# shichaoy/pop_up_slam

Hardware: AMD Instinct MI355X
Metric: graph-solve iters/sec + final chi2, 1k-pose/5k-edge plane graph (higher is better)
Workload: dtype f64; 1 GPU; C2 synthetic corridor: 1000 SE3 poses, 200 planes, 5000 plane edges, 999 odometry edges (BASELINE.json configs[1], seed 42); jacobian_mode=numeric, total_lm_solves=812

## Files before the change

### include/pps.h

```cpp
#ifndef PPS_H
#define PPS_H

#include <stddef.h>
#include <stdint.h>

#ifdef __cplusplus
extern "C" {
#endif

#define PPS_VERSION 304

typedef struct pps_graph pps_graph;

enum pps_status {
  PPS_OK = 0,
  PPS_EINVAL = 1,
  PPS_ENOTPD = 2,
  PPS_EHIP = 3,
  PPS_ENOMEM = 4,
  PPS_ESTATE = 5
};

enum pps_jacobian_mode {
  PPS_JAC_NUMERIC = 0,
// ... 26 lines not shown

int pps_add_pose_prior(pps_graph* g, int pose, const double meas6[6], const double sqrtinf_ut[21], int* fid);
int pps_add_odometry(pps_graph* g, int pose1, int pose2, const double meas6[6], const double sqrtinf_ut[21], int* fid);
int pps_add_plane_obs(pps_graph* g, int pose, int plane, const double meas4[4], const double sqrtinf_ut[6], int* fid);
int pps_add_plane_obs2(pps_graph* g, int pose_id, int plane_id, const double meas4[4], const double ray6[6],
                       const double sqrtinf_ut[6], int* fid);
int pps_edge_ray(const float invK[9], const float seg2d[4], double ray6[6]);
int pps_add_plane_prior(pps_graph* g, int plane, const double meas4[4], const double sqrtinf_ut[6], int* fid);

int pps_set_measurement(pps_graph* g, int fid, const double meas4[4]);
int pps_set_measurements(pps_graph* g, int n, const int* fids, const double* meas4 );

int pps_remove_factor(pps_graph* g, int fid);
int pps_remove_node(pps_graph* g, int nid);

int pps_update(pps_graph* g);
int pps_batch_optimize(pps_graph* g, int* iterations);
int pps_chi2(pps_graph* g, double* chi2);

int pps_cov_recover(pps_graph* g);
int pps_cov_marginals(pps_graph* g, int n, const int* ids, double* out, int64_t* offsets);
int pps_cov_access(pps_graph* g, int n, const int* rows, const int* cols, double* out, int64_t* offsets, int* in_pattern);
int pps_cov_joint(pps_graph* g, int n, const int* ids, double* out);
int pps_cov_last_times(const pps_graph* g, double sec[2]);
int pps_cov_block(pps_graph* g, int nr, const int* rows, int nc, const int* cols, double* out);
int pps_cov_block_last(const pps_graph* g, double* kernel_sec, int* launches);

typedef struct pps_multi pps_multi;
int pps_multi_create(int n, pps_graph* const* graphs, pps_multi** out);
int pps_multi_destroy(pps_multi* m);
const char* pps_multi_last_error(const pps_multi* m);
int pps_multi_optimize(pps_multi* m, int* iterations, int* status);
int pps_multi_rounds(const pps_multi* m, int* rounds);
int pps_multi_save_state(pps_multi* m);
int pps_multi_restore_state(pps_multi* m);
int pps_multi_set_profiling(pps_multi* m, int level);
int pps_multi_phase_times(const pps_multi* m, double sec[5], long long counts[4]);

int pps_num_nodes(const pps_graph* g, int* n);
int pps_num_factors(const pps_graph* g, int* n);
int pps_get_pose(pps_graph* g, int id, double tq[7]);
int pps_get_plane(pps_graph* g, int id, double abcd[4]);
int pps_set_pose(pps_graph* g, int id, const double tq[7]);
int pps_set_plane(pps_graph* g, int id, const double abcd[4]);
int pps_get_poses(pps_graph* g, int n, const int* ids, double* out);
int pps_get_planes(pps_graph* g, int n, const int* ids, double* out);
int pps_save_state(pps_graph* g);
int pps_restore_state(pps_graph* g);

typedef struct pps_stats {
  int    n_poses, n_planes, n_factors;
  int    dim_nodes, dim_measure;
  int    n_fronts, n_levels, max_front;
  int64_t nnz_L;
  int    lm_iterations;
  int    lm_trials_accepted, lm_trials_rejected;
  double chi2_initial, chi2_final, lambda_final;
  double last_delta_norm;
  double t_total, t_analysis, t_upload;
  double t_linearize, t_assemble, t_factor, t_backsolve, t_retract_chi2;
  int    n_linearize, n_factorize;
  int    lm_trials_notpd;
  int    n_launches;
} pps_stats;
int pps_get_stats(const pps_graph* g, pps_stats* out);
int pps_get_trace(const pps_graph* g, int cap, double* lambda, double* chi2, int* accepted, int* n);
int pps_set_profiling(pps_graph* g, int level);

int pps_factor_shape(const pps_graph* g, int fid, int* dim, int* cols);
int pps_eval_factor(pps_graph* g, int fid, int mode , double* J, double* r);

int pps_analyze(pps_graph* g);
int pps_analysis_reuse(const pps_graph* g, int* fronts_kept, int* fronts_total);
int pps_analysis_kept(const pps_graph* g, int kept[6]);
int pps_analysis_dump(pps_graph* g, int64_t cap, int32_t* out, int64_t* needed);

int pps_time_linearize(pps_graph* g, int mode, int iters, double* sec_per_launch);
int pps_bench_sweep(pps_graph* g, int mode, int replicas, int iters, double sec_per_sweep[3],
                    int64_t* n_plane_edges, int64_t* n_odo_edges);

int pps_debug_front_factor(int tiles, int strip, int p, int b, const double* A, double* L, double* U, double* not_pd);

int pps_debug_exmap(int kind, int n, const double* x, const double* delta, double* out);

int pps_popup_planes(int device, const float* seg2d, int n, const float invK[9], const float T_wc[16],
                     float* planes_out);

typedef struct pps_point { float x, y, z; uint32_t rgba; } pps_point;

typedef struct pps_popup pps_popup;
int pps_popup_create(int device, int width, int height, const float invK[9], pps_popup** out);
int pps_popup_destroy(pps_popup* p);
const char* pps_popup_last_error(const pps_popup* p);
int pps_popup_set_image(pps_popup* p, const unsigned char* bgr);
int pps_popup_run(pps_popup* p, const float* seg2d, int n, const float T_wc[16], const float* polys,
                  const int* poly_off, int nplanes, int step, float depth_thre, float ceiling_thre, int* n_valid);
int pps_popup_run_async(pps_popup* p, const float* seg2d, int n, const float T_wc[16], const float* polys,
                        const int* poly_off, int nplanes, int step, float depth_thre, float ceiling_thre);
int pps_popup_planes_wait(pps_popup* p, float* planes);
int pps_popup_wait(pps_popup* p, int* n_valid);
int pps_popup_download(pps_popup* p, float* planes, pps_point* cloud, float* depth, int32_t* plane_id);
int pps_popup_set_outputs(pps_popup* p, int want_depth, int want_plane_id);
int pps_popup_plane_info(pps_popup* p, float plane_cam_dist_thre, const int* actual_plane_indices, int n_actual,
                         float* dist_to_cam, int32_t* good);
int pps_popup_fill_depth(pps_popup* p);
int pps_popup_download_segments3d(pps_popup* p, float* seg3d_world);
int pps_popup_last_kernel_time(const pps_popup* p, double* sec);
int pps_popup_polygons_simple(const float K[9], const float invK[9], const float T_wc[16], int width, int height, const float* seg2d, int n,
                              float* verts, int cap_verts, int* poly_off, int* n_verts);
int pps_popup_mask_host(const float* polys, const int* poly_off, int nplanes, int width, int height, int step, int32_t* plane_id);

int pps_frames_set_calibration(pps_graph* g, const float invK[9]);
int pps_frames_add(pps_graph* g, int pose_id, int n_seg, const float* seg2d, const int* fids, int* frame_id);
int pps_refresh_measurements(pps_graph* g);
int pps_get_measurement(pps_graph* g, int fid, double meas4[4]);

typedef struct pps_assoc_params {
  double edge_asso_2ddist;
  double edge_asso_planedist;
  double edge_asso_proj;
  double edge_asso_angle;
  int assoc_near_frames;
} pps_assoc_params;
void pps_assoc_default_params(pps_assoc_params* p);
int pps_landmark_update(pps_graph* g, int plane_id, int frame_plane_indice, int frame_seq_id, const float seg2d[4],
                        const float seg3d_xy[4]);
int pps_landmark_set_merged(pps_graph* g, int plane_id);
int pps_find_closest_planes(pps_graph* g, const double est_pose[7], int frame_seq_id, int n, const double* planes_local,
                            const int* frame_plane_indice, const float* seg2d, const float* seg3d_xy,
                            const pps_assoc_params* prm, int* best_plane_id, double* best_err);

int pps_graph_save(pps_graph* g, const char* path, int precision);
int pps_graph_load(const char* path, const pps_props* props, pps_graph** out);

int pps_reproject_points(pps_graph* g, int n, const int* plane_ids, const float* pts_xyz, float* out_xyz);

typedef struct pps_edge_params {
  int downsample_contour;
  int dilation_distance, erosion_distance;
  double pre_vertical_thre, pre_minium_len, pre_contour_close_thre, interval_overlap_thre, post_short_thre,
         post_bind_dist_thre, post_merge_dist_thre, post_merge_angle_thre, post_extend_thre;
  double pre_boundary_thre, pre_merge_angle_thre, pre_merge_dist_thre, pre_proj_angle_thre, pre_proj_cover_thre,
         pre_proj_cover_large_thre, pre_proj_dist_thre;
} pps_edge_params;
void pps_edge_default_params(pps_edge_params* p);

typedef struct pps_edges pps_edges;
int pps_edges_create(int device, int width, int height, pps_edges** out);
int pps_edges_destroy(pps_edges* e);
const char* pps_edges_last_error(const pps_edges* e);
int pps_edges_select(pps_edges* e, const unsigned char* label_map, int label_on_device, const float* lsd_lines,
                     int n_lines, const pps_edge_params* prm, float* open_segs, int* n_open, float* closed_segs,
                     int* n_closed, float* open_in_closed);
int pps_edges_download_label(pps_edges* e, unsigned char* out, int* w, int* h);
int pps_edges_contour(pps_edges* e, float* xy, int cap, int* n, int* n_contours, int* n_points);
int pps_edges_last_kernel_time(const pps_edges* e, double* sec);
int pps_edges_host_contour(const int16_t* cell_segs, int n, float scale, float* xy, int cap, int* n_xy, int* n_contours,
                           int* n_points);
int pps_edges_host_select(const float* contour_xy, int n_contour, int width, int height, const float* lsd_lines, int n_lines,
                          const pps_edge_params* prm, float* open_segs, int* n_open, float* closed_segs, int* n_closed,
                          float* open_in_closed);

#ifdef __cplusplus
}
#endif
#endif
// ... 1 lines not shown
```

### pop_up_slam_amd/__init__.py

```python
from __future__ import annotations

import ctypes as C
import os

import numpy as np

_HERE = os.path.dirname(os.path.abspath(__file__))
LIB_PATH = os.environ.get("PPS_LIB") or os.path.join(_HERE, "libpps.so")

PPS_OK, PPS_EINVAL, PPS_ENOTPD, PPS_EHIP, PPS_ENOMEM, PPS_ESTATE = range(6)
JAC_NUMERIC, JAC_ANALYTIC = 0, 1

_dp = C.POINTER(C.c_double)
_fp = C.POINTER(C.c_float)
_ip = C.POINTER(C.c_int)


PPS_VERSION = 304


class PpsProps(C.Structure):
    _fields_ = [
        ("epsilon2", C.c_double), ("epsilon_abs", C.c_double), ("epsilon_rel", C.c_double),
        ("max_iterations", C.c_int), ("lm_lambda0", C.c_double), ("lm_lambda_factor", C.c_double),
        ("jacobian_mode", C.c_int), ("device", C.c_int), ("verbose", C.c_int),
    ]


class PpsStats(C.Structure):
    _fields_ = [
        ("n_poses", C.c_int), ("n_planes", C.c_int), ("n_factors", C.c_int),
        ("dim_nodes", C.c_int), ("dim_measure", C.c_int),
        ("n_fronts", C.c_int), ("n_levels", C.c_int), ("max_front", C.c_int),
        ("nnz_L", C.c_int64),
        ("lm_iterations", C.c_int), ("lm_trials_accepted", C.c_int), ("lm_trials_rejected", C.c_int),
        ("chi2_initial", C.c_double), ("chi2_final", C.c_double), ("lambda_final", C.c_double),
        ("last_delta_norm", C.c_double),
        ("t_total", C.c_double), ("t_analysis", C.c_double), ("t_upload", C.c_double),
        ("t_linearize", C.c_double), ("t_assemble", C.c_double), ("t_factor", C.c_double),
        ("t_backsolve", C.c_double), ("t_retract_chi2", C.c_double),
        ("n_linearize", C.c_int), ("n_factorize", C.c_int), ("lm_trials_notpd", C.c_int), ("n_launches", C.c_int),
    ]

    def asdict(self):
        return {k: getattr(self, k) for k, _ in self._fields_}


class PpsError(RuntimeError):
    def __init__(self, code, msg):
        super().__init__(f"pps error {code}: {msg}")
        self.code = code


_LIB = None

def edge_ray(invK, seg2d):
    k = np.ascontiguousarray(invK, dtype=np.float32).reshape(9); sg = np.ascontiguousarray(seg2d, dtype=np.float32).reshape(4)
    out = np.zeros(6)
    rc = lib().pps_edge_ray(k.ctypes.data_as(_fp), sg.ctypes.data_as(_fp), out.ctypes.data_as(_dp))
    if rc != PPS_OK:
        raise PpsError(rc, "pps_edge_ray")
    return out


class PpsEdgeParams(C.Structure):
    _fields_ = [("downsample_contour", C.c_int), ("dilation_distance", C.c_int), ("erosion_distance", C.c_int)] + [
        (k, C.c_double) for k in ("pre_vertical_thre", "pre_minium_len", "pre_contour_close_thre", "interval_overlap_thre",
                                  "post_short_thre", "post_bind_dist_thre", "post_merge_dist_thre", "post_merge_angle_thre",
                                  "post_extend_thre", "pre_boundary_thre", "pre_merge_angle_thre", "pre_merge_dist_thre",
                                  "pre_proj_angle_thre", "pre_proj_cover_thre", "pre_proj_cover_large_thre",
                                  "pre_proj_dist_thre")]


class PpsAssocParams(C.Structure):
    _fields_ = [("edge_asso_2ddist", C.c_double), ("edge_asso_planedist", C.c_double), ("edge_asso_proj", C.c_double),
                ("edge_asso_angle", C.c_double), ("assoc_near_frames", C.c_int)]


SYMBOLS = [
    "pps_default_props", "pps_version", "pps_last_error", "pps_graph_create", "pps_graph_destroy",
    "pps_get_props", "pps_set_props", "pps_add_pose", "pps_add_plane", "pps_add_pose_prior",
    "pps_add_odometry", "pps_add_plane_obs", "pps_add_plane_prior", "pps_set_measurement",
    "pps_set_measurements", "pps_remove_factor", "pps_remove_node", "pps_update", "pps_batch_optimize",
    "pps_chi2", "pps_num_nodes", "pps_num_factors", "pps_get_pose", "pps_get_plane", "pps_set_pose",
    "pps_set_plane", "pps_get_poses", "pps_get_planes", "pps_get_stats", "pps_get_trace",
    "pps_set_profiling", "pps_factor_shape", "pps_eval_factor", "pps_analyze", "pps_analysis_dump",
    "pps_bench_sweep", "pps_save_state", "pps_restore_state",
    "pps_popup_planes", "pps_popup_create", "pps_popup_destroy", "pps_popup_last_error", "pps_popup_set_image",
    "pps_popup_run", "pps_popup_run_async", "pps_popup_planes_wait", "pps_popup_wait", "pps_popup_download", "pps_popup_last_kernel_time",
    "pps_frames_set_calibration", "pps_frames_add", "pps_refresh_measurements", "pps_get_measurement",
    "pps_popup_download_segments3d", "pps_assoc_default_params", "pps_landmark_update", "pps_landmark_set_merged",
    "pps_find_closest_planes", "pps_graph_save", "pps_graph_load", "pps_add_plane_obs2", "pps_edge_ray",
    "pps_time_linearize", "pps_debug_front_factor", "pps_debug_exmap", "pps_reproject_points", "pps_popup_set_outputs",
    "pps_edge_default_params", "pps_edges_create", "pps_edges_destroy", "pps_edges_last_error", "pps_edges_select",
    "pps_edges_download_label", "pps_edges_contour", "pps_edges_last_kernel_time", "pps_edges_host_contour",
    "pps_edges_host_select", "pps_popup_fill_depth", "pps_popup_plane_info", "pps_popup_mask_host",
    "pps_multi_create", "pps_multi_destroy", "pps_multi_last_error", "pps_multi_optimize", "pps_multi_rounds", "pps_multi_save_state", "pps_multi_restore_state", "pps_multi_set_profiling", "pps_multi_phase_times", "pps_popup_polygons_simple", "pps_analysis_reuse", "pps_analysis_kept",
    "pps_cov_recover", "pps_cov_marginals", "pps_cov_access", "pps_cov_joint", "pps_cov_last_times",
    "pps_cov_block", "pps_cov_block_last",
]


def lib():
    global _LIB
    if _LIB is None:
        if not os.path.exists(LIB_PATH):
            raise ImportError(
                f"{LIB_PATH} not found: build it with `python -c 'import __graft_entry__ as g; g.build()'` "
                "(or make -C pop_up_slam_amd/csrc).  There is no CPU fallback.")
        L = C.CDLL(LIB_PATH)
        L.pps_version.restype = C.c_int
        if L.pps_version() != PPS_VERSION:
            raise ImportError(f"{LIB_PATH} reports PPS_VERSION {L.pps_version()}, this binding mirrors {PPS_VERSION}: rebuild the library")
        L.pps_last_error.restype = C.c_char_p
        L.pps_last_error.argtypes = [C.c_void_p]
        L.pps_default_props.argtypes = [C.POINTER(PpsProps)]
        L.pps_default_props.restype = None
        L.pps_graph_create.argtypes = [C.POINTER(PpsProps), C.POINTER(C.c_void_p)]
        L.pps_graph_destroy.argtypes = [C.c_void_p]
        L.pps_get_props.argtypes = [C.c_void_p, C.POINTER(PpsProps)]
        L.pps_set_props.argtypes = [C.c_void_p, C.POINTER(PpsProps)]
        L.pps_add_pose.argtypes = [C.c_void_p, _dp, _ip]
        L.pps_add_plane.argtypes = [C.c_void_p, _dp, _ip]
        L.pps_add_pose_prior.argtypes = [C.c_void_p, C.c_int, _dp, _dp, _ip]
        L.pps_add_odometry.argtypes = [C.c_void_p, C.c_int, C.c_int, _dp, _dp, _ip]
        L.pps_add_plane_obs.argtypes = [C.c_void_p, C.c_int, C.c_int, _dp, _dp, _ip]
        L.pps_add_plane_prior.argtypes = [C.c_void_p, C.c_int, _dp, _dp, _ip]
        L.pps_set_measurement.argtypes = [C.c_void_p, C.c_int, _dp]
        L.pps_set_measurements.argtypes = [C.c_void_p, C.c_int, _ip, _dp]
        L.pps_remove_factor.argtypes = [C.c_void_p, C.c_int]
        L.pps_remove_node.argtypes = [C.c_void_p, C.c_int]
        L.pps_update.argtypes = [C.c_void_p]
        L.pps_batch_optimize.argtypes = [C.c_void_p, _ip]
        L.pps_chi2.argtypes = [C.c_void_p, _dp]
        L.pps_num_nodes.argtypes = [C.c_void_p, _ip]
        L.pps_num_factors.argtypes = [C.c_void_p, _ip]
        L.pps_get_pose.argtypes = [C.c_void_p, C.c_int, _dp]
        L.pps_get_plane.argtypes = [C.c_void_p, C.c_int, _dp]
        L.pps_set_pose.argtypes = [C.c_void_p, C.c_int, _dp]
        L.pps_set_plane.argtypes = [C.c_void_p, C.c_int, _dp]
        L.pps_get_poses.argtypes = [C.c_void_p, C.c_int, _ip, _dp]
        L.pps_get_planes.argtypes = [C.c_void_p, C.c_int, _ip, _dp]
        L.pps_save_state.argtypes = [C.c_void_p]
        L.pps_restore_state.argtypes = [C.c_void_p]
        L.pps_get_stats.argtypes = [C.c_void_p, C.POINTER(PpsStats)]
        L.pps_get_trace.argtypes = [C.c_void_p, C.c_int, _dp, _dp, _ip, _ip]
        L.pps_set_profiling.argtypes = [C.c_void_p, C.c_int]
        L.pps_factor_shape.argtypes = [C.c_void_p, C.c_int, _ip, _ip]
        L.pps_eval_factor.argtypes = [C.c_void_p, C.c_int, C.c_int, _dp, _dp]
        L.pps_analyze.argtypes = [C.c_void_p]
        L.pps_analysis_dump.argtypes = [C.c_void_p, C.c_int64, C.POINTER(C.c_int32), C.POINTER(C.c_int64)]
        L.pps_bench_sweep.argtypes = [C.c_void_p, C.c_int, C.c_int, C.c_int, _dp, C.POINTER(C.c_int64),
                                      C.POINTER(C.c_int64)]
        _u8 = C.POINTER(C.c_ubyte)
        L.pps_popup_planes.argtypes = [C.c_int, _fp, C.c_int, _fp, _fp, _fp]
        L.pps_popup_create.argtypes = [C.c_int, C.c_int, C.c_int, _fp, C.POINTER(C.c_void_p)]
        L.pps_popup_destroy.argtypes = [C.c_void_p]
        L.pps_popup_last_error.argtypes = [C.c_void_p]
        L.pps_popup_last_error.restype = C.c_char_p
        L.pps_popup_set_image.argtypes = [C.c_void_p, _u8]
        L.pps_popup_run.argtypes = [C.c_void_p, _fp, C.c_int, _fp, _fp, _ip, C.c_int, C.c_int, C.c_float, C.c_float, _ip]
        L.pps_popup_run_async.argtypes = L.pps_popup_run.argtypes[:-1]
        L.pps_popup_planes_wait.argtypes = [C.c_void_p, _fp]
        L.pps_popup_wait.argtypes = [C.c_void_p, C.POINTER(C.c_int)]
        L.pps_popup_download.argtypes = [C.c_void_p, _fp, C.c_void_p, _fp, C.POINTER(C.c_int32)]
        L.pps_popup_last_kernel_time.argtypes = [C.c_void_p, _dp]
        L.pps_popup_mask_host.argtypes = [_fp, _ip, C.c_int, C.c_int, C.c_int, C.c_int, C.POINTER(C.c_int32)]
        L.pps_popup_polygons_simple.argtypes = [_fp, _fp, _fp, C.c_int, C.c_int, _fp, C.c_int, _fp, C.c_int, _ip, _ip]
        L.pps_multi_create.argtypes = [C.c_int, C.POINTER(C.c_void_p), C.POINTER(C.c_void_p)]
        L.pps_multi_destroy.argtypes = [C.c_void_p]
        L.pps_multi_last_error.argtypes = [C.c_void_p]
        L.pps_multi_last_error.restype = C.c_char_p
        L.pps_multi_optimize.argtypes = [C.c_void_p, _ip, _ip]
        L.pps_multi_rounds.argtypes = [C.c_void_p, _ip]
        L.pps_multi_save_state.argtypes = [C.c_void_p]; L.pps_multi_restore_state.argtypes = [C.c_void_p]
        L.pps_multi_set_profiling.argtypes = [C.c_void_p, C.c_int]
        L.pps_multi_phase_times.argtypes = [C.c_void_p, _dp, C.POINTER(C.c_longlong)]
        L.pps_popup_fill_depth.argtypes = [C.c_void_p]
        L.pps_popup_plane_info.argtypes = [C.c_void_p, C.c_float, _ip, C.c_int, _fp, _ip]
        L.pps_frames_set_calibration.argtypes = [C.c_void_p, _fp]
        L.pps_frames_add.argtypes = [C.c_void_p, C.c_int, C.c_int, _fp, _ip, _ip]
        L.pps_refresh_measurements.argtypes = [C.c_void_p]
# ... 237 lines not shown
        out = np.zeros((n, 7)); self._ck(self.L.pps_get_poses(self.h, n, ptr, out.ctypes.data_as(_dp))); return out

    def get_planes(self, ids=None, n=None):
        if ids is not None:
            i = np.ascontiguousarray(ids, dtype=np.int32); n = len(i); ptr = i.ctypes.data_as(_ip)
        else:
            ptr = None
            if n is None:
                n = self.stats()["n_planes"]
        out = np.zeros((n, 4)); self._ck(self.L.pps_get_planes(self.h, n, ptr, out.ctypes.data_as(_dp))); return out

    def frames_set_calibration(self, invK):
        k = np.ascontiguousarray(invK, dtype=np.float32).reshape(9)
        self._ck(self.L.pps_frames_set_calibration(self.h, k.ctypes.data_as(_fp)))

    def frames_add(self, pose_id, seg2d, fids):
        seg = np.ascontiguousarray(seg2d, dtype=np.float32).reshape(-1, 4)
        f = np.ascontiguousarray(fids, dtype=np.int32)
        assert len(f) == len(seg) + 1
        out = C.c_int()
        self._ck(self.L.pps_frames_add(self.h, pose_id, len(seg), seg.ctypes.data_as(_fp), f.ctypes.data_as(_ip), C.byref(out)))
        return out.value

    def refresh_measurements(self):
        self._ck(self.L.pps_refresh_measurements(self.h))

    def get_measurement(self, fid):
        out = np.zeros(4); self._ck(self.L.pps_get_measurement(self.h, fid, out.ctypes.data_as(_dp))); return out

    def landmark_update(self, plane_id, frame_plane_indice, frame_seq_id, seg2d=None, seg3d_xy=None):
        s2 = None if seg2d is None else np.ascontiguousarray(seg2d, dtype=np.float32).reshape(4)
        s3 = None if seg3d_xy is None else np.ascontiguousarray(seg3d_xy, dtype=np.float32).reshape(4)
        self._ck(self.L.pps_landmark_update(self.h, int(plane_id), int(frame_plane_indice), int(frame_seq_id),
                                            None if s2 is None else s2.ctypes.data_as(_fp),
                                            None if s3 is None else s3.ctypes.data_as(_fp)))

    def landmark_set_merged(self, plane_id):
        self._ck(self.L.pps_landmark_set_merged(self.h, int(plane_id)))

    def find_closest_planes(self, est_pose, frame_seq_id, planes_local, frame_plane_indice, seg2d, seg3d_xy, **params):
        prm = PpsAssocParams(); self.L.pps_assoc_default_params(C.byref(prm))
        for k, v in params.items():
            setattr(prm, k, v)
        pl = np.ascontiguousarray(planes_local, dtype=np.float64).reshape(-1, 4); n = len(pl)
        fpi = np.ascontiguousarray(frame_plane_indice, dtype=np.int32).reshape(n)
        s2 = np.ascontiguousarray(seg2d, dtype=np.float32).reshape(n, 4)
        s3 = np.ascontiguousarray(seg3d_xy, dtype=np.float32).reshape(n, 4)
        pose = np.ascontiguousarray(est_pose, dtype=np.float64).reshape(7)
        best = np.full(n, -1, dtype=np.int32); err = np.full(n, -1.0)
        self._ck(self.L.pps_find_closest_planes(self.h, pose.ctypes.data_as(_dp), int(frame_seq_id), n, pl.ctypes.data_as(_dp),
                                                fpi.ctypes.data_as(_ip), s2.ctypes.data_as(_fp), s3.ctypes.data_as(_fp),
                                                C.byref(prm), best.ctypes.data_as(_ip), err.ctypes.data_as(_dp)))
        return best, err

    def time_linearize(self, mode=JAC_NUMERIC, iters=200):
        s = C.c_double(); self._ck(self.L.pps_time_linearize(self.h, int(mode), int(iters), C.byref(s))); return s.value

    def reproject_points(self, plane_ids, pts):
        ids = np.ascontiguousarray(plane_ids, dtype=np.int32); p = np.ascontiguousarray(pts, dtype=np.float32).reshape(-1, 3)
        assert len(ids) == len(p)
        out = np.zeros_like(p)
        self._ck(self.L.pps_reproject_points(self.h, len(ids), ids.ctypes.data_as(_ip), p.ctypes.data_as(_fp), out.ctypes.data_as(_fp)))
        return out

    def save_state(self):
        self._ck(self.L.pps_save_state(self.h))

    def restore_state(self):
        self._ck(self.L.pps_restore_state(self.h))

    def stats(self):
        s = PpsStats(); self._ck(self.L.pps_get_stats(self.h, C.byref(s))); return s.asdict()

    def trace(self):
        n = C.c_int(); self._ck(self.L.pps_get_trace(self.h, 0, None, None, None, C.byref(n)))
        lam = np.zeros(n.value); chi = np.zeros(n.value); acc = np.zeros(n.value, dtype=np.int32)
        self._ck(self.L.pps_get_trace(self.h, n.value, lam.ctypes.data_as(_dp), chi.ctypes.data_as(_dp),
                                      acc.ctypes.data_as(_ip), C.byref(n)))
        return [(float(l), float(c), bool(a)) for l, c, a in zip(lam, chi, acc)]

    def set_profiling(self, level=2):
        self._ck(self.L.pps_set_profiling(self.h, int(level)))

    def eval_factor(self, fid, mode=JAC_NUMERIC):
        m, c = C.c_int(), C.c_int(); self._ck(self.L.pps_factor_shape(self.h, fid, C.byref(m), C.byref(c)))
        J = np.zeros((m.value, c.value)); r = np.zeros(m.value)
        self._ck(self.L.pps_eval_factor(self.h, fid, mode, J.ctypes.data_as(_dp), r.ctypes.data_as(_dp)))
        return J, r

    def analysis_reuse(self):
        a, b = C.c_int(), C.c_int()
        self._ck(self.L.pps_analysis_reuse(self.h, C.byref(a), C.byref(b)))
        return a.value, b.value

    def analysis_kept(self):
        k = (C.c_int * 6)()
        self._ck(self.L.pps_analysis_kept(self.h, k))
        return dict(zip(("fronts", "fronts_lists", "blocks", "segs", "contribs", "nd_segs"), [int(x) for x in k]))

    def analyze(self):
        self._ck(self.L.pps_analyze(self.h))

    def analysis_dump(self):
        need = C.c_int64(); self._ck(self.L.pps_analysis_dump(self.h, 0, None, C.byref(need)))
        buf = np.zeros(need.value, dtype=np.int32)
        self._ck(self.L.pps_analysis_dump(self.h, need.value, buf.ctypes.data_as(C.POINTER(C.c_int32)), C.byref(need)))
        return parse_analysis_dump(buf)

    def bench_sweep(self, mode=JAC_NUMERIC, replicas=1, iters=10):
        sec = (C.c_double * 3)(); npl = C.c_int64(); nod = C.c_int64()
        self._ck(self.L.pps_bench_sweep(self.h, mode, replicas, iters, sec, C.byref(npl), C.byref(nod)))
        return tuple(sec), npl.value, nod.value


_DUMP_SCALARS = ["n_nodes", "n_scalars", "n_fronts", "n_levels", "max_front", "n_blocks", "n_segs", "L_size",
                 "U_size", "H_size", "J_size"]
_DUMP_VECTORS = ["node_pos", "node_voff", "order", "f_p", "f_b", "f_poff", "f_parent", "f_level", "f_Loff", "f_Uoff",
                 "f_bidx_off", "bidx", "f_child_off", "child", "f_cmap_off", "cmap", "level_off", "level_fronts",
                 "f_asm_off", "asm_blk", "asm_lrow", "asm_lcol", "blk_rows", "blk_cols", "blk_size", "blk_nseg",
                 "blk_hoff", "seg_blk", "seg_c0", "seg_cnt", "seg_hoff", "contrib", "node_compact", "factor_joff"]


def parse_analysis_dump(buf):
    out = {}
    k = 0
    for name in _DUMP_SCALARS:
        out[name] = int(buf[k]); k += 1
    def vec():
        nonlocal k
        n = int(buf[k]); k += 1
        v = np.array(buf[k:k + n], dtype=np.int64); k += n
        return v
    for name in _DUMP_VECTORS[:-2]:
        out[name] = vec()
    for name in ("n_stages", "n_groups", "n_glevels"):
        out[name] = int(buf[k]); k += 1
    for name in ("stage_grp_off", "grp_lvl_off", "glvl_front_off", "glvl_fronts", "stage_max_front", "stage_max_width",
                 "f_el_off", "el_src", "el_tgt", "f_ea_off", "ea_tgt", "blk_doff", "blk_dst", "frec", "crec", "srec",
                 "pidx", "obs_dir", "nd_segs"):
        out[name] = vec()
    for name in _DUMP_VECTORS[-2:]:
        out[name] = vec()
    out["factor_poff"] = vec()
    out["P_size"] = int(buf[k]); k += 1
    assert k == len(buf), (k, len(buf))
    return out


POINT_DTYPE = np.dtype([("x", "<f4"), ("y", "<f4"), ("z", "<f4"), ("rgba", "<u4")])


def popup_planes(seg2d, invK, T_wc, device=0):
    seg = np.ascontiguousarray(seg2d, dtype=np.float32).reshape(-1, 4)
    k = np.ascontiguousarray(invK, dtype=np.float32).reshape(9)
    t = np.ascontiguousarray(T_wc, dtype=np.float32).reshape(16)
    out = np.zeros((len(seg) + 1, 4), dtype=np.float32)
    rc = lib().pps_popup_planes(device, seg.ctypes.data_as(_fp), len(seg), k.ctypes.data_as(_fp), t.ctypes.data_as(_fp),
                                out.ctypes.data_as(_fp))
    if rc != PPS_OK:
        raise PpsError(rc, "pps_popup_planes failed")
    return out


class Popup:

    def __init__(self, width, height, invK, device=0):
# ... 300 lines not shown
```

### pop_up_slam_amd/csrc/pps_api.cpp

```cpp
#include "pps_graph.h"

using namespace pps;
using namespace pps_impl;

namespace pps {
Switches read_switches() {
  auto on = [](const char* k) { return getenv(k) != nullptr; };
  auto num = [](const char* k, long long dflt) { const char* e = getenv(k); return e && *e ? atoll(e) : dflt; };
  Switches s;
  s.k1_thread_form = on("PPS_K1_THREAD_FORM");
  {
    long long plain = num("PPS_PLAIN_SCHEDULE", 0);
    if (on("PPS_PLAIN_SCHEDULE") && plain <= 0) plain = 15;
    s.no_preassemble = (plain & 1) != 0; s.no_solve_flow = (plain & 2) != 0; s.no_root_fuse = (plain & 4) != 0; s.split_expand = (plain & 8) != 0;
  }
  s.no_spec_lin = on("PPS_NO_SPEC_LIN");
  s.no_dual = on("PPS_NO_DUAL");
  s.no_strip = on("PPS_NO_STRIP");
  s.no_incremental = on("PPS_NO_INCREMENTAL");
  s.no_incr_compact = on("PPS_NO_INCR_COMPACT");
  s.verify_upload = on("PPS_DEBUG_VERIFY_UPLOAD");
  s.multi_levels = on("PPS_MULTI_LEVELS");
  s.multi_thread_form = on("PPS_MULTI_THREAD_FORM");
  s.debug_drop_flag = (int)num("PPS_DEBUG_DROP_FLAG", 0);
  if (on("PPS_DEBUG_DROP_FLAG") && s.debug_drop_flag < 1) s.debug_drop_flag = 1;
  s.trace = (int)num("PPS_TRACE", 0);
  if (on("PPS_TRACE") && s.trace < 1) s.trace = 1;
  {
    long long tm = num("PPS_TIMING", 0);
    if (on("PPS_TIMING") && tm <= 0) tm = 7;
    s.analysis_timing = (tm & 1) != 0; s.upload_timing = (tm & 2) != 0; s.multi_timing = (tm & 8) ? 2 : ((tm & 4) ? 1 : 0);
  }
  s.multi_split = (int)num("PPS_MULTI_SPLIT", 0);
  s.multi_thread_factors = num("PPS_MULTI_THREAD_FACTORS", 120000);
  return s;
}
}

namespace pps_impl {
void report_front_trace(pps_graph* g) {
  const Analysis& A = g->an;
  std::vector<long long> tr((size_t)A.n_fronts * 8);
  (void)hipMemcpy(tr.data(), g->dev.trace, tr.size() * 8, hipMemcpyDeviceToHost);
  if (g->dev.trace_solve) {
    for (int l = A.n_levels - 1; l >= 0; l--) {
      double ph[5] = {0, 0, 0, 0, 0}, gap = 0; int n = 0, ng = 0;
      for (int s2 = 0; s2 < A.n_fronts; s2++) {
        if (A.f_level[s2] != l) continue;
        n++;
        for (int k = 0; k < 5; k++) ph[k] += (double)(tr[(size_t)s2 * 8 + k + 1] - tr[(size_t)s2 * 8 + k]);
        const int par = A.f_parent[s2];
        if (par >= 0) { gap += (double)(tr[(size_t)s2 * 8] - tr[(size_t)par * 8 + 5]); ng++; }
      }
      if (!n) continue;
      fprintf(stderr, "  solve level %d (%d fronts): panel load %.0f boundary values %.0f y - L_B^T x_b %.0f back-substitution %.0f store %.0f | start after parent's end %.0f\n",
              l, n, ph[0] / n, ph[1] / n, ph[2] / n, ph[3] / n, ph[4] / n, ng ? gap / ng : 0.0);
    }
  } else {
    double acc[5] = {0, 0, 0, 0, 0};
    std::vector<double> lvl_tot(A.n_levels, 0.0); std::vector<int> lvl_n(A.n_levels, 0);
    for (int s2 = 0; s2 < A.n_fronts; s2++) {
      for (int k = 0; k < 5; k++) acc[k] += (double)(tr[(size_t)s2 * 8 + k + 1] - tr[(size_t)s2 * 8 + k]);
      lvl_tot[A.f_level[s2]] += (double)(tr[(size_t)s2 * 8 + 5] - tr[(size_t)s2 * 8]); lvl_n[A.f_level[s2]]++;
    }
    { double pn = 0, tr2 = 0; for (int s2 = 0; s2 < A.n_fronts; s2++) { pn += (double)tr[(size_t)s2 * 8 + 6]; tr2 += (double)tr[(size_t)s2 * 8 + 7]; }
      fprintf(stderr, "PPS_TRACE elimination split: panel %.0f trailing %.0f cycles per front\n", pn / A.n_fronts, tr2 / A.n_fronts); }
    fprintf(stderr, "PPS_TRACE mean cycles per front: zero %.0f gather %.0f extend-add %.0f eliminate %.0f store %.0f\n",
            acc[0] / A.n_fronts, acc[1] / A.n_fronts, acc[2] / A.n_fronts, acc[3] / A.n_fronts, acc[4] / A.n_fronts);
    for (int l = 0; l < A.n_levels; l++) fprintf(stderr, "  level %d: %d fronts, mean total %.0f cycles\n", l, lvl_n[l], lvl_tot[l] / std::max(1, lvl_n[l]));
    {
      std::vector<long long> last_child_end(A.n_fronts, 0);
      for (int s2 = 0; s2 < A.n_fronts; s2++) if (A.f_parent[s2] >= 0) last_child_end[A.f_parent[s2]] = std::max(last_child_end[A.f_parent[s2]], tr[(size_t)s2 * 8 + 5]);
      for (int l = 0; l < A.n_levels; l++) {
        double ph[7] = {0, 0, 0, 0, 0, 0, 0}, gap = 0; int n = 0, ng = 0;
        for (int s2 = 0; s2 < A.n_fronts; s2++) {
          if (A.f_level[s2] != l) continue;
          n++;
          for (int k = 0; k < 5; k++) ph[k] += (double)(tr[(size_t)s2 * 8 + k + 1] - tr[(size_t)s2 * 8 + k]);
          ph[5] += (double)tr[(size_t)s2 * 8 + 6]; ph[6] += (double)tr[(size_t)s2 * 8 + 7];
          if (last_child_end[s2] > 0) { gap += (double)(tr[(size_t)s2 * 8] - last_child_end[s2]); ng++; }
        }
        if (!n) continue;
        fprintf(stderr, "  level %d: zero %.0f gather %.0f extend-add %.0f eliminate %.0f (panel %.0f trailing %.0f) store %.0f | start after last child's end %.0f\n", l,
                ph[0] / n, ph[1] / n, ph[2] / n, ph[3] / n, ph[5] / n, ph[6] / n, ph[4] / n, ng ? gap / ng : 0.0);
      }
    }
    {
      double w[8] = {0, 0, 0, 0, 0, 0, 0, 0}; int nw2 = 0;
      for (int s2 = 0; s2 < A.n_fronts; s2++) {
        if (A.f_p[s2] + A.f_b[s2] + 1 <= 64) continue;
        nw2++;
        for (int k = 0; k < 5; k++) w[k] += (double)(tr[(size_t)s2 * 8 + k + 1] - tr[(size_t)s2 * 8 + k]);
        w[5] += (double)tr[(size_t)s2 * 8 + 6]; w[6] += (double)tr[(size_t)s2 * 8 + 7];
      }
      if (nw2) fprintf(stderr, "  fronts beyond 64 rows (%d): zero %.0f gather %.0f extend-add %.0f eliminate %.0f (panel %.0f trailing %.0f) store %.0f cycles\n", nw2,
                       w[0] / nw2, w[1] / nw2, w[2] / nw2, w[3] / nw2, w[5] / nw2, w[6] / nw2, w[4] / nw2);
    }
    long long tmin = tr[0], tmax = tr[5];
    for (int s2 = 0; s2 < A.n_fronts; s2++) { tmin = std::min(tmin, tr[(size_t)s2 * 8]); tmax = std::max(tmax, tr[(size_t)s2 * 8 + 5]); }
    fprintf(stderr, "  first start -> last end: %lld cycles\n", tmax - tmin);
// ... 315 lines not shown
int pps_set_profiling(pps_graph* g, int level) { if (!g) return PPS_EINVAL; g->profiling = level < 0 ? 0 : level; return PPS_OK; }

int pps_factor_shape(const pps_graph* g, int fid, int* dim, int* cols) {
  if (!g) return PPS_EINVAL;
  if (fid < 0 || fid >= (int)g->factors.size() || g->factors[fid].deleted) return PPS_EINVAL;
  const HostFactor& f = g->factors[fid];
  if (dim) *dim = kFDim[f.type];
  if (cols) *cols = (g->nodes[f.a].type == NODE_POSE ? 6 : 3) + (f.b >= 0 ? (g->nodes[f.b].type == NODE_POSE ? 6 : 3) : 0);
  return PPS_OK;
}

int pps_eval_factor(pps_graph* g, int fid, int mode, double* J, double* r) {
  if (!g || !J || !r) return PPS_EINVAL;
  if (fid < 0 || fid >= (int)g->factors.size() || g->factors[fid].deleted) return fail(g, PPS_EINVAL, "eval_factor: unknown id");
  int rc = prepare_solve(g);
  if (rc != PPS_OK) return rc;
  rc = linpoint_from_estimate(g); if (rc != PPS_OK) return rc;
  HIP_TRY(g, launch_linearize(g->dev, mode, true, g->stream));
  const HostFactor& f = g->factors[fid];
  const int m = kFDim[f.type];
  const int da = g->nodes[f.a].type == NODE_POSE ? 6 : 3;
  const int db = f.b >= 0 ? (g->nodes[f.b].type == NODE_POSE ? 6 : 3) : 0;
  const int64_t base[4] = {g->dev.joff_pp, g->dev.joff_odo, g->dev.joff_obs, g->dev.joff_lp};
  std::vector<double> buf(kJSize[f.type]);
  HIP_TRY(g, hipMemcpyAsync(buf.data(), g->dev.J + base[f.type] + (int64_t)f.slot * kJSize[f.type], buf.size() * 8,
                            hipMemcpyDeviceToHost, g->stream));
  HIP_TRY(g, hipStreamSynchronize(g->stream));
  const int cols = da + db;
  for (int i = 0; i < m; i++) {
    for (int j = 0; j < da; j++) J[i * cols + j] = buf[i * da + j];
    for (int j = 0; j < db; j++) J[i * cols + da + j] = buf[m * da + i * db + j];
    r[i] = buf[m * (da + db) + i];
  }
  return PPS_OK;
}

int pps_analyze(pps_graph* g) {
  if (!g) return PPS_EINVAL;
  if (g->n_live_nodes == 0) return fail(g, PPS_ESTATE, "empty graph");
  if (g->dev_ready) {
    int rc = download_state(g); if (rc != PPS_OK) return rc;
    rc = download_measurements(g); if (rc != PPS_OK) return rc;
    g->topo_dirty = true;
  }
  return run_analysis(g);
}

int pps_analysis_reuse(const pps_graph* g, int* fronts_kept, int* fronts_total) {
  if (!g) return PPS_EINVAL;
  analysis_cache_stats(g->acache, fronts_kept, fronts_total);
  return PPS_OK;
}

int pps_analysis_kept(const pps_graph* g, int kept[6]) {
  if (!g || !kept) return PPS_EINVAL;
  const Analysis::Kept& k = g->an.kept;
  kept[0] = k.fronts; kept[1] = k.fronts_lists; kept[2] = k.blocks; kept[3] = k.segs; kept[4] = k.contribs; kept[5] = k.nd_segs;
  return PPS_OK;
}

int pps_analysis_dump(pps_graph* g, int64_t cap, int32_t* out, int64_t* needed) {
  if (!g || !needed) return PPS_EINVAL;
  if (!g->analyzed || g->analysis_stale) { int rc = pps_analyze(g); if (rc != PPS_OK) return rc; }
  std::vector<int32_t> v;
  dump_analysis(g->an, v);
  v.push_back((int32_t)g->nodes.size());
  for (const auto& n : g->nodes) v.push_back(n.deleted ? -1 : n.compact);
  int64_t base[4]; j_bases(g, base, nullptr);
  v.push_back((int32_t)g->factors.size());
  for (const auto& f : g->factors) v.push_back(f.deleted ? -1 : (int32_t)(base[f.type] + (int64_t)f.slot * kJSize[f.type]));
  int64_t pbase[4]; p_bases(g, pbase, nullptr);
  v.push_back((int32_t)g->factors.size());
  for (const auto& f : g->factors) v.push_back(f.deleted ? -1 : (int32_t)(pbase[f.type] + (int64_t)f.slot * kPSize[f.type]));
  v.push_back((int32_t)g->an.P_size);
  *needed = (int64_t)v.size();
  if (out && cap >= (int64_t)v.size()) memcpy(out, v.data(), v.size() * sizeof(int32_t));
  return PPS_OK;
}

int pps_debug_front_factor(int tiles, int strip, int p, int b, const double* A, double* L, double* U, double* not_pd) {
  if (!A || !L || !U) return PPS_EINVAL;
  const int rc = pps::debug_front_factor(tiles, strip, p, b, A, L, U, not_pd);
  return rc == 0 ? PPS_OK : (rc < 0 ? PPS_EINVAL : PPS_EHIP);
}

int pps_debug_exmap(int kind, int n, const double* x, const double* delta, double* out) {
  if (!x || !delta || !out) return PPS_EINVAL;
  const int rc = pps::debug_exmap(kind, n, x, delta, out);
  return rc == 0 ? PPS_OK : (rc < 0 ? PPS_EINVAL : PPS_EHIP);
}

int pps_time_linearize(pps_graph* g, int mode, int iters, double* sec_per_launch) {
  if (!g || iters < 1 || !sec_per_launch) return PPS_EINVAL;
  int rc = prepare_solve(g);
  if (rc != PPS_OK) return rc;
  rc = linpoint_from_estimate(g); if (rc != PPS_OK) return rc;
  for (int k = 0; k < 3; k++) HIP_TRY(g, launch_linearize(g->dev, mode, false, g->stream));
  HIP_TRY(g, hipEventRecord(g->ev[0], g->stream));
  for (int k = 0; k < iters; k++) HIP_TRY(g, launch_linearize(g->dev, mode, false, g->stream));
  HIP_TRY(g, hipEventRecord(g->ev[1], g->stream));
  HIP_TRY(g, hipEventSynchronize(g->ev[1]));
  float ms = 0;
  HIP_TRY(g, hipEventElapsedTime(&ms, g->ev[0], g->ev[1]));
  *sec_per_launch = 1e-3 * ms / iters;
  return PPS_OK;
}

int pps_bench_sweep(pps_graph* g, int mode, int replicas, int iters, double* sec_per_sweep, int64_t* n_plane_edges,
                    int64_t* n_odo_edges) {
  if (!g || replicas < 1 || iters < 1 || !sec_per_sweep) return PPS_EINVAL;
  int rc = prepare_solve(g);
  if (rc != PPS_OK) return rc;
  rc = linpoint_from_estimate(g); if (rc != PPS_OK) return rc;
  if (g->dev.n_obs_fixed != g->dev.n_obs) return fail(g, PPS_ESTATE, "bench_sweep: graph holds re-popping plane edges (Factor2)");
  DevGraph d = g->dev;
  std::vector<void*> tmp;
  auto rep = [&](auto** ptr, size_t count_per) -> int {
    using T = std::remove_pointer_t<std::remove_pointer_t<decltype(ptr)>>;
    if (count_per == 0) return PPS_OK;
    void* p = nullptr;
    hipError_t e = hipMalloc(&p, count_per * sizeof(T) * (size_t)replicas);
    if (e != hipSuccess) return hip_fail(g, e, "hipMalloc(bench)");
    tmp.push_back(p);
    for (int r = 0; r < replicas; r++) {
      e = hipMemcpyAsync(static_cast<char*>(p) + (size_t)r * count_per * sizeof(T), *ptr, count_per * sizeof(T),
                         hipMemcpyDeviceToDevice, g->stream);
      if (e != hipSuccess) return hip_fail(g, e, "hipMemcpyAsync(bench)");
    }
    *ptr = static_cast<T*>(p);
    return PPS_OK;
  };
  auto cleanup = [&]() { (void)hipStreamSynchronize(g->stream); for (void* p : tmp) (void)hipFree(p); };
#define BT(x) do { rc = (x); if (rc != PPS_OK) { cleanup(); return rc; } } while (0)
  BT(rep(&d.obs_pose, (size_t)d.n_obs)); BT(rep(&d.obs_plane, (size_t)d.n_obs));
  BT(rep(&d.obs_meas, (size_t)4 * d.obs_ld)); BT(rep(&d.obs_w, (size_t)6 * d.obs_ld));
  BT(rep(&d.odo_a, (size_t)d.n_odo)); BT(rep(&d.odo_b, (size_t)d.n_odo));
  BT(rep(&d.odo_meas, (size_t)6 * d.odo_ld)); BT(rep(&d.odo_w, (size_t)21 * d.odo_ld));
#undef BT
  const size_t slab = (size_t)d.n_obs * 30 + (size_t)d.n_odo * 78;
  double* Jbig = nullptr;
  hipError_t e = hipMalloc(reinterpret_cast<void**>(&Jbig), slab * sizeof(double) * (size_t)replicas);
  if (e != hipSuccess) { cleanup(); return hip_fail(g, e, "hipMalloc(Jbig)"); }
  tmp.push_back(Jbig);
  e = launch_sweep_bench(d, mode, replicas, Jbig, -1, g->stream);
  if (e == hipSuccess) e = hipStreamSynchronize(g->stream);
  float total_ms = 0, part_ms[2] = {0, 0};
  for (int it = 0; it < iters && e == hipSuccess; it++) {
    (void)hipEventRecord(g->ev[0], g->stream);
    e = launch_sweep_bench(d, mode, replicas, Jbig, -1, g->stream);
    (void)hipEventRecord(g->ev[1], g->stream);
    if (e == hipSuccess) e = hipEventSynchronize(g->ev[1]);
    float ms = 0;
    (void)hipEventElapsedTime(&ms, g->ev[0], g->ev[1]);
    total_ms += ms;
    for (int part = 0; part < 2 && e == hipSuccess; part++) {
      (void)hipEventRecord(g->ev[0], g->stream);
      e = launch_sweep_bench(d, mode, replicas, Jbig, part, g->stream);
      (void)hipEventRecord(g->ev[1], g->stream);
      if (e == hipSuccess) e = hipEventSynchronize(g->ev[1]);
      (void)hipEventElapsedTime(&ms, g->ev[0], g->ev[1]);
      part_ms[part] += ms;
    }
  }
  cleanup();
  if (e != hipSuccess) return hip_fail(g, e, "sweep bench");
  sec_per_sweep[1] = 1e-3 * part_ms[0] / iters;
// ... 9 lines not shown
```

### pop_up_slam_amd/csrc/pps_device.h

```cpp
#pragma once

#include <hip/hip_runtime.h>

#include <cstdint>

namespace pps {

struct DevGraph {
  int n_pose = 0, n_plane = 0, pose_ld = 0, plane_ld = 0;
  double *pose_est = nullptr, *pose_lin = nullptr;
  double *plane_est = nullptr, *plane_lin = nullptr;
  int *pose_voff = nullptr, *plane_voff = nullptr;
  int n_obs = 0, n_odo = 0, n_pp = 0, n_lp = 0;
  int obs_ld = 0, odo_ld = 0, pp_ld = 0, lp_ld = 0;
  int *obs_pose = nullptr, *obs_plane = nullptr; double *obs_meas = nullptr, *obs_w = nullptr;
  int n_obs_fixed = 0; double* obs_ray = nullptr;
  int *odo_a = nullptr, *odo_b = nullptr;         double *odo_meas = nullptr, *odo_w = nullptr;
  int *pp_pose = nullptr;                          double *pp_meas = nullptr, *pp_w = nullptr;
  int *lp_plane = nullptr;                         double *lp_meas = nullptr, *lp_w = nullptr;
  double* J = nullptr;
  int64_t joff_obs = 0, joff_odo = 0, joff_pp = 0, joff_lp = 0;
  double* P = nullptr;
  int64_t poff_obs = 0;
  double* H = nullptr;
  double* L = nullptr;
  double* U = nullptr;
  double* delta = nullptr;
  int n_scalars = 0;
  int n_fronts = 0, n_levels = 0, max_front = 0, n_segs = 0, n_blocks = 0;
  int *f_p = nullptr, *f_b = nullptr, *f_poff = nullptr;
  int* pidx = nullptr;
  int64_t *f_Loff = nullptr, *f_Uoff = nullptr;
  int *f_bidx_off = nullptr, *bidx = nullptr;
  int *f_child_off = nullptr, *child = nullptr;
  int *f_cmap_off = nullptr, *cmap = nullptr;
  int *level_fronts = nullptr;
  int *f_asm_off = nullptr, *asm_blk = nullptr, *asm_lrow = nullptr, *asm_lcol = nullptr;
  int *asm_el0 = nullptr, *asm_fsz = nullptr;
  int *blk_rows = nullptr, *blk_cols = nullptr, *blk_size = nullptr, *blk_nseg = nullptr;
  int64_t* blk_hoff = nullptr;
  int *seg_blk = nullptr, *seg_c0 = nullptr, *seg_cnt = nullptr;
  int64_t* seg_hoff = nullptr;
  int* contrib = nullptr;
  int n_mseg = 0; int* mseg_blk = nullptr;
  int *f_el_off = nullptr, *el_src = nullptr, *el_tgt = nullptr;
  int *blk_doff = nullptr, *blk_dst = nullptr;
  double* Hf = nullptr;
  int64_t* f_ea_off = nullptr; int* ea_tgt = nullptr;
  int *grp_lvl_off = nullptr, *glvl_front_off = nullptr, *glvl_fronts = nullptr;
  int* grp_span = nullptr;
  int *frec = nullptr, *crec = nullptr, *srec = nullptr;
  int* obs_dir = nullptr;
  int* k3_flag = nullptr;
  int* nd_segs = nullptr; int n_nd_segs = 0;
  int* k2_single = nullptr; int n_k2_single = 0;
  int* k2_multi = nullptr; int n_k2_multi = 0;
  int* k2_finish = nullptr; int n_k2_finish = 0;
  int* k2t = nullptr; int n_k2t_big = 0, n_k2t_small = 0, n_k2t_spec = 0;
  int *cls_off = nullptr, *cls_fronts = nullptr;
  double* chi2_partials = nullptr;
  int chi2_blocks = 0;
  double* dn_partials = nullptr;
  unsigned int* ticket = nullptr;
  double* result_dev = nullptr;
  long long* trace = nullptr;
  int trace_solve = 0;
  int no_strip = 0;
  unsigned sw = 0;
  double step_ac[4] = {0, 0, 0, 0};
  double* gwork = nullptr;
  int64_t gwork_stride = 0;
};

constexpr double kStatusInternal = 64.0;
enum : unsigned { SW_K1_THREAD_FORM = 1u, SW_NO_SOLVE_FLOW = 2u, SW_NO_ROOT_FUSE = 4u, SW_DEBUG_DROP_FLAG = 8u, SW_DEBUG_DROP_XFLAG = 16u };
struct Switches {
  bool k1_thread_form = false;
  bool no_preassemble = false;
  bool no_solve_flow = false;
  bool no_root_fuse = false;
  bool split_expand = false;
  bool no_spec_lin = false;
  bool no_dual = false;
  bool no_strip = false;
  bool no_incremental = false;
  bool no_incr_compact = false;
  bool verify_upload = false;
  bool multi_levels = false, multi_thread_form = false;
  int debug_drop_flag = 0;
  int trace = 0;
  bool analysis_timing = false, upload_timing = false;
  int multi_timing = 0;
  int multi_split = 0;
  long long multi_thread_factors = 120000;
  unsigned dev_bits() const {
    return (k1_thread_form ? SW_K1_THREAD_FORM : 0u) | (no_solve_flow ? SW_NO_SOLVE_FLOW : 0u) | (no_root_fuse ? SW_NO_ROOT_FUSE : 0u) |
           (debug_drop_flag == 1 ? SW_DEBUG_DROP_FLAG : 0u) | (debug_drop_flag == 2 ? SW_DEBUG_DROP_XFLAG : 0u);
  }
};
Switches read_switches();

struct LinGuard {
  const double* chi[2];
  const double* pose[2];
  const double* plane[2];
  double error;
  int on, single;
  int want = -1;
};

struct SpecLin {
  double *J, *P, *H, *Hf;
  int which;
};

unsigned long long launch_count();
void count_launch();
#define PPS_LAUNCH(...) do { ::pps::count_launch(); hipLaunchKernelGGL(__VA_ARGS__); } while (0)
#define PPS_LAUNCH_EV(ev0, ev1, kernel, grid, block, lds, st, ...)                                                     \
  do {                                                                                                                 \
    ::pps::count_launch();                                                                                             \
    if (ev0) hipExtLaunchKernelGGL(kernel, grid, block, lds, st, ev0, ev1, 0, __VA_ARGS__);                            \
    else hipLaunchKernelGGL(kernel, grid, block, lds, st, __VA_ARGS__);                                                \
  } while (0)

hipError_t step_constants(double ac[4]);
hipError_t launch_linearize(const DevGraph& d, int mode, bool at_estimate, hipStream_t st, const LinGuard* guard = nullptr, hipEvent_t ev0 = nullptr,
                            hipEvent_t ev1 = nullptr);
hipError_t launch_hblocks(const DevGraph& d, hipStream_t st, const LinGuard* guard = nullptr, bool products = true);
bool k1_lane_form(const DevGraph& d, int mode);
bool k1_products(const DevGraph& d, int mode);
hipError_t launch_factor_level(const DevGraph& d, int level_begin, int level_count, int level_max_front, double lambda,
                               hipStream_t st);
hipError_t launch_backsolve_level(const DevGraph& d, int level_begin, int level_count, hipStream_t st);
struct DualAlt {
  double *L, *U, *delta, *result_dev, *chi2_partials, *dn_partials;
  unsigned int* ticket;
  double lambda;
};
hipError_t launch_band_all(const DevGraph& d, const DualAlt* alt, int n_groups, int nwaves_factor, int nwaves_solve, int max_front, int max_panel,
                           int max_group_fronts, double lambda, int epoch, hipStream_t st, hipEvent_t ev0 = nullptr, hipEvent_t ev1 = nullptr);
int band_all_solve_waves(int max_panel, int max_group_fronts);
hipError_t launch_band_factor(const DevGraph& d, int grp_begin, int grp_count, int nwaves, int max_front, double lambda, hipStream_t st,
                              hipEvent_t ev0 = nullptr, hipEvent_t ev1 = nullptr, bool pre = false);
hipError_t launch_band_solve(const DevGraph& d, int grp_begin, int grp_count, int nwaves, int max_panel, int max_group_fronts, hipStream_t st,
                             const DualAlt* alt = nullptr);
hipError_t launch_band_factor_dual(const DevGraph& d, const DualAlt& alt, int grp_begin, int grp_count, int nwaves, int max_front, double lambda,
                                   hipStream_t st, hipEvent_t ev0 = nullptr, hipEvent_t ev1 = nullptr, bool pre = false);
bool band_root_fusable(const DevGraph& d, int grp_count, int max_front);
hipError_t launch_band_root(const DevGraph& d, const DualAlt* alt, int grp, int nwaves_factor, int nwaves_solve, int max_front, int max_panel,
                            int max_group_fronts, double lambda, hipStream_t st, hipEvent_t ev0 = nullptr, hipEvent_t ev1 = nullptr,
                            bool pre = false);
hipError_t launch_trial_dual(const DevGraph& d, const DualAlt& alt, const double* base_pose, const double* base_plane, double* out_pose0,
                             double* out_plane0, double* out_pose1, double* out_plane1, double* host_result0, double seq0, double* host_result1,
                             double seq1, hipStream_t st, int n_trials = 2);
hipError_t launch_trial_lin(const DevGraph& d, const DualAlt& alt, const SpecLin& sl, const double* base_pose, const double* base_plane, double* out_pose0,
                            double* out_plane0, double* out_pose1, double* out_plane1, double* host_result0, double seq0, double* host_result1,
                            double seq1, hipStream_t st, hipEvent_t ev0 = nullptr, hipEvent_t ev1 = nullptr);
int trial_lin_waves(const DevGraph& d);
bool trial_lin_ok(const DevGraph& d, int mode);
hipError_t launch_hblocks_spec(const DevGraph& d, const SpecLin& sl, hipStream_t st, const LinGuard* guard = nullptr);
hipError_t launch_expand_ea(const DevGraph& d, int n_fronts, double* zero, size_t n_zero, int* ones, size_t n_ones, hipStream_t st);
hipError_t launch_expand_el(const DevGraph& d, int n_asm, hipStream_t st);
hipError_t launch_expand_lists(const DevGraph& d, int n_fronts, int n_asm, double* zero, size_t n_zero, hipStream_t st);
int band_max_rows();
bool band_level_solve_direct_ok(int p, int b);
size_t band_solve_lds_bytes(int max_panel);
int band_front_limit();
int debug_front_factor(int tiles, int strip, int p, int b, const double* A_host, double* L_host, double* U_host, double* not_pd);
int debug_exmap(int kind, int n, const double* x_host, const double* delta_host, double* out_host);
int band_reg_rows();
size_t band_lds_bytes(int max_front, bool reg_only_kernel = false);
hipError_t launch_retract_trial(const DevGraph& d, hipStream_t st);
hipError_t launch_retract_apply(const DevGraph& d, hipStream_t st);
hipError_t launch_chi2(const DevGraph& d, bool at_estimate, double* host_result, double seq, hipStream_t st);
hipError_t launch_clear_status(const DevGraph& d, hipStream_t st);
hipError_t launch_chi2_trial(const DevGraph& d, double* host_result, double seq, hipStream_t st);

int dense_front_max_pivots();
hipError_t launch_dense_hpush(const DevGraph& d, int max_el_per_front, double lambda, hipStream_t st);
hipError_t launch_dense_factor_level(const DevGraph& d, int level_begin, int level_count, const int* off_asm, int n_asm,
                                     const int* off_pan, int n_pan, const int* off_trl, int n_trl, hipStream_t st);
hipError_t launch_dense_solve_level(const DevGraph& d, int level_begin, int level_count, int level_max_b, hipStream_t st);

constexpr int kBatchMax = 128;
enum { BF_ACTIVE = 1,
       BF_RELIN = 2 };
struct BatchStage { int grp_begin, grp_count; };
struct BatchAlt {
  double *L, *U, *delta, *result_dev, *chi2_partials, *dn_partials;
  unsigned int* ticket;
  double* pose[3];
  double* plane[3];
};
struct BatchArgs {
  const DevGraph* gs;
  const BatchStage* stage_tab;
  double* results;
  int n_total, b0, n;
  int no_products;
  double seq;
  double lambda[kBatchMax];
  unsigned char flags[kBatchMax];
  const BatchAlt* alt;
  int rstride, lin_apply;
  double lambda2[kBatchMax];
  unsigned char xsel[kBatchMax];
};
struct BatchGeom {
  int lin_blocks = 0, lin_obs_blocks = 0, lin_rest_blocks = 0, repop_blocks = 0;
  int hblocks = 0, k2t_blocks = 0, k2tg_blocks = 0, hreduce = 0, retract = 0, chi2 = 0;
  int k2_blocks = 0, k2_finish = 0;
  long long n_factors_total = 0;
  bool lin_thread_form = false;
  int n_stages = 0;
  int stage_groups[32] = {0}, stage_nw_factor[32] = {0}, stage_nw_solve[32] = {0};
  int stage_per_wave_factor[32] = {0}, stage_per_wave_solve[32] = {0}, stage_grp_fronts[32] = {0};
  bool stage_reg_only[32] = {false};
  bool stage_pre[32] = {false};
  int stage_nw_flow[32] = {0};
  bool level_form = false;
  int n_levels = 0;
  int lvl_cls_blocks[64][3] = {{0}};
  int lvl_blocks[64] = {0};
  int lvl_direct_pp[64] = {0};
  int lvl_max_panel[64] = {0};
  int solve_per_wave_all = 0;
  int stage_max_front[32] = {0};
};
hipError_t launch_batch_linearize(const BatchArgs& a, const BatchGeom& g, int mode, hipStream_t st);
hipError_t launch_batch_hblocks(const BatchArgs& a, const BatchGeom& g, hipStream_t st, bool products);
hipError_t launch_batch_chi2(const BatchArgs& a, const BatchGeom& g, int slot, hipStream_t st);
hipError_t launch_batch_solve(const BatchArgs& a, const BatchGeom& g, hipStream_t st, hipEvent_t after_factor = nullptr);
struct RestoreRec { double* dst; const double* src; long long n; };
hipError_t launch_batch_restore(const RestoreRec* tab, int n, hipStream_t st);
hipError_t launch_batch_begin_dual(const BatchArgs& a, const BatchGeom& g, hipStream_t st);
hipError_t launch_batch_trial_dual(const BatchArgs& a, const BatchGeom& g, hipStream_t st);

hipError_t launch_scatter_patches(const char* table, const char* src_base, int n_patches, char* arena, hipStream_t st);

int lds_front_limit();
// ... 5 lines not shown
```

### pop_up_slam_amd/csrc/pps_graph.h

```cpp
#pragma once
#include <hip/hip_runtime.h>

#include <algorithm>
#include <charconv>
#include <chrono>
#include <cmath>
#include <cstdio>
#include <cstdlib>
#include <cstring>
#include <mutex>
#include <new>
#include <string>
#include <unordered_map>
#include <vector>

#include "../../include/pps.h"
#include "pps_device.h"
#include "pps_geom.h"
#include "pps_lm.h"
#include "pps_popup_dev.h"
#include "pps_symbolic.h"

namespace pps_impl {

// ... 11 lines not shown
  double w[21];
  bool deleted;
  int slot;
  int repop;
  double ray[6];
};

inline double now_s() {
  using namespace std::chrono;
  return duration_cast<duration<double>>(steady_clock::now().time_since_epoch()).count();
}

}

struct pps_graph {
  pps_props props;
  std::string err;
  std::vector<pps_impl::HostNode> nodes;
  std::vector<pps_impl::HostFactor> factors;
  int n_live_nodes = 0, n_live_factors = 0, dim_nodes = 0, dim_measure = 0;
  int n_live_type[4] = {0, 0, 0, 0}, n_live_repop = 0;
  bool topo_dirty = true;
  bool analysis_stale = true;
  bool host_values_newer = true;
  bool dev_values_newer = false;
  bool meas_dirty = false;
  bool analyzed = false;
  int n_analyses = 0;
  std::vector<pps::SymNode> sym_nodes; std::vector<pps::SymFactor> sym_factors;
  size_t cmp_nodes = 0, cmp_factors = 0; int64_t cmp_base[4] = {0, 0, 0, 0}; bool cmp_valid = false, cmp_has_repop = false;
  bool grown_only = true;
  bool grown_only_upload = false;
  pps::Analysis an;
  pps::AnalysisParams aprm;
  pps::Switches sw;
  pps::AnalysisCache* acache = nullptr;
  std::vector<int> pose_ids, plane_ids;
  std::vector<int> fslot_ids[4];
  std::vector<int> level_max_front;
  bool use_band = false;
  bool use_dense = false;
  std::vector<int> level_max_b;
  int max_el_per_front = 0;
  std::vector<int> dw_asm, dw_pan, dw_trl;
  int *d_dw_asm = nullptr, *d_dw_pan = nullptr, *d_dw_trl = nullptr;
  std::vector<int> stage_max_piv, stage_nw_factor, stage_nw_solve, stage_max_grp_fronts, stage_max_panel;
  std::vector<char> stage_pre;
  bool dev_ready = false;
  hipStream_t stream = nullptr;
  pps::DevGraph dev;
  std::vector<void*> allocs;
  struct Arena { char* base = nullptr; size_t cap = 0, off = 0, spill = 0; };
  Arena up, scr;
  char* stage = nullptr;
  size_t stage_cap = 0;
  size_t stage_lo = 0, stage_hi = 0;
  struct UpSlot { size_t off, cap; };
  std::vector<UpSlot> up_slots;
  size_t up_cursor = 0, up_high = 0;
  bool up_unknown = true;
  long an_seq = 0, an_base_seq = -1, up_an_seq = -1;
  bool hint_violation = false;
  bool verify_hints = false;
  bool up_unknown_meas = false;
  size_t slot_obs_meas = (size_t)-1;
  size_t slot_lp_meas = (size_t)-1;
  std::vector<int> pk_obs_a, pk_obs_b, pk_odo_a, pk_odo_b, pk_obs_ids, pk_odo_ids;
  std::vector<double> pk_obs_m, pk_obs_w, pk_odo_m, pk_odo_w;
  size_t pk_n_obs = 0, pk_n_odo = 0, pk_ld_obs = 0, pk_ld_odo = 0;
  bool pk_meas_ok = false;
  bool status_clean = false;
  bool up_inflight = false;
  double* state_pin = nullptr; size_t state_pin_cap = 0;
  bool pin_holds_est = false;
  std::unordered_map<std::string, double> up_laps;
  struct UpPatch { size_t off, len; bool exact8 = false; };
  std::vector<UpPatch> up_patches;
  char* patch_host = nullptr; size_t patch_cap = 0;
  size_t up_bytes_sent = 0, up_bytes_total = 0;
  double* host_result = nullptr;
  double seq = 0.0;
  double *spec_pose = nullptr, *spec_plane = nullptr, *spec_chi2_partials = nullptr, *spec_dn_partials = nullptr;
  unsigned int* spec_ticket = nullptr;
  double seq2 = 0.0;
  double *spec_L = nullptr, *spec_U = nullptr, *spec_delta = nullptr;
  double* spec_result = nullptr;
  double *spec_J = nullptr, *spec_P = nullptr, *spec_H = nullptr, *spec_Hf = nullptr;
  bool k3_all = false;
  int k3_nw_factor = 0, k3_nw_solve = 0, k3_max_front = 0, k3_max_panel = 0, k3_max_grp = 0, k3_epoch = 0;
  double *snap_pose = nullptr, *snap_plane = nullptr;
  int snap_version = -1, upload_version = 0;
  int k2t_version = -1;
  int profiling = 0;
  hipEvent_t ev[2] = {nullptr, nullptr};
  unsigned long long launches0 = 0;
  std::vector<char> k1_skip;
  std::vector<hipEvent_t> k1_events;
  std::vector<hipEvent_t> fk_events;
  int fk_used = 0;
  int k1_used = 0;
  float frames_invK[9] = {1, 0, 0, 0, 1, 0, 0, 0, 1};
  std::vector<int> fr_pose;
  std::vector<int> fr_seg_off{0};
  std::vector<float> fr_seg;
  std::vector<int> fr_item_frame, fr_item_plane, fr_item_fid;
  bool frames_dirty = true;
  std::vector<int> fr_slot, fr_pslot;
  long n_removals = 0, fr_cache_removals = -1;
  int fr_hint_version = -2; size_t fr_hint_cursor = 0, fr_hint_items = 0, fr_hint_frames = 0;
  int frames_version = -1;
  int *d_item_frame = nullptr, *d_item_plane = nullptr, *d_item_slot = nullptr, *d_frame_pose_slot = nullptr, *d_frame_seg_off = nullptr;
  float* d_fr_seg = nullptr;
  bool dev_meas_newer = false;
  int n_obs_fixed = 0;
  struct Landmark { int plane_id, fpi, seq, deleted; float seg2d[4], seg3d[4]; };
  std::vector<Landmark> lms;
  std::unordered_map<int, int> lm_of_plane;
  bool lms_dirty = true;
  int lms_upload_version = -1;
  pps::AssocLandmark* d_lms = nullptr; size_t d_lms_cap = 0;
  pps::AssocLandmark* h_lms = nullptr;
  pps::AssocQuery* d_queries = nullptr; pps::AssocResult* d_results = nullptr; size_t d_q_cap = 0;
  double* d_lm_planes = nullptr; size_t d_lm_planes_cap = 0;
  char* rp_pin = nullptr; size_t rp_cap = 0;
  bool cov_valid = false;
  int cov_version = -1;
  double* cov_S = nullptr; size_t cov_S_cap = 0;
  int* cov_parent = nullptr; size_t cov_parent_cap = 0; int cov_parent_version = -1;
  char* cov_req = nullptr; size_t cov_req_cap = 0;
  double* cov_out = nullptr; size_t cov_out_cap = 0;
  std::vector<int> cov_epos, cov_front_of;
  hipEvent_t cov_ev[3] = {nullptr, nullptr, nullptr};
  double cov_sec[2] = {0, 0};
  std::vector<int> cov_rootlen; int cov_max_p = 0, cov_max_rows = 0;
  char* cov_breq = nullptr; size_t cov_breq_cap = 0;
  double* cov_strip = nullptr; size_t cov_strip_cap = 0;
  double* cov_bout = nullptr; size_t cov_bout_cap = 0; bool cov_bout_clean = false;
  hipEvent_t cov_bev[2] = {nullptr, nullptr};
  double cov_block_sec = 0; int cov_block_launches = 0;
  pps_stats stats{};
  std::vector<double> tr_lambda, tr_chi2;
  std::vector<int> tr_acc;
};

namespace pps_impl {
using namespace pps;

inline int fail(pps_graph* g, int code, const std::string& msg) {
  if (g) g->err = msg;
  return code;
}
inline int hip_fail(pps_graph* g, hipError_t e, const char* what) {
  return fail(g, PPS_EHIP, std::string(what) + ": " + hipGetErrorString(e));
}
#define HIP_TRY(g, expr)                                   \
  do {                                                     \
    hipError_t _e = (expr);                                \
    if (_e != hipSuccess) return hip_fail(g, _e, #expr);   \
  } while (0)


inline bool live_node(const pps_graph* g, int id, int type) {
  return id >= 0 && id < (int)g->nodes.size() && !g->nodes[id].deleted && g->nodes[id].type == type;
}

void free_device(pps_graph* g);
// ... 119 lines not shown
```

### pop_up_slam_amd/csrc/pps_k1.hip

```cpp
#include <atomic>
#include <cstdlib>
#include <mutex>

#include <hip/hip_ext.h>

#include "pps_k1_body.h"

namespace pps {

hipError_t launch_linearize_lanes(const DevGraph& d, const double* pose, const double* plane, const LinGuard& gd, hipStream_t st, hipEvent_t ev0, hipEvent_t ev1);
hipError_t launch_sweep_bench_lanes(const DevGraph& d, int replicas, double* Jbig, int part, hipStream_t st);
hipError_t launch_batch_linearize_lanes(const BatchArgs& a, const BatchGeom& g, hipStream_t st);

constexpr int kObsNumericWaves = 2;

template <int MODE, int PART>
__global__ __launch_bounds__(kLinBlock) void k_linearize(DevGraph d, const double* __restrict__ pose,
                                                          const double* __restrict__ plane, int nb_obs, int nb_odo,
                                                          int nb_pp, LinGuard gd) {
  extern __shared__ double lin_lds[];
  if (!lin_guard(gd, pose, plane)) return;
  body_linearize<MODE, PART, PART == 0>(d, pose, plane, nb_obs, nb_odo, nb_pp, blockIdx.x, lin_lds);
}

__global__ __launch_bounds__(kLinBlock) __attribute__((amdgpu_waves_per_eu(kObsNumericWaves, kObsNumericWaves)))
void k_linearize_obs_numeric(DevGraph d, const double* __restrict__ pose, const double* __restrict__ plane, int nb_obs, int nb_odo, int nb_pp, LinGuard gd) {
  extern __shared__ double lin_lds[];
  if (!lin_guard(gd, pose, plane)) return;
  body_linearize<0, 0, true>(d, pose, plane, nb_obs, nb_odo, nb_pp, blockIdx.x, lin_lds);
}

__global__ void k_step_constants(double* out, double eps) {
  double ac[2];
  rot_step_quat(ac, eps); out[0] = ac[0]; out[1] = ac[1];
  plane_step_quat(ac, eps); out[2] = ac[0]; out[3] = ac[1];
}
static std::atomic<int> g_step_state[64];
static double g_step_ac[64][4];
static std::mutex g_step_mutex;
hipError_t step_constants(double ac[4]) {
  int dev = 0;
  (void)hipGetDevice(&dev);
  dev &= 63;
  if (g_step_state[dev].load(std::memory_order_acquire) != 2) {
    std::lock_guard<std::mutex> lk(g_step_mutex);
    if (g_step_state[dev].load(std::memory_order_acquire) != 2) {
      double* o = nullptr;
      hipError_t e = hipMalloc(&o, 4 * sizeof(double));
      if (e != hipSuccess) return e;
      hipLaunchKernelGGL(k_step_constants, dim3(1), dim3(1), 0, 0, o, kNumDiffEps);
      e = hipGetLastError();
      if (e == hipSuccess) e = hipMemcpy(g_step_ac[dev], o, 4 * sizeof(double), hipMemcpyDeviceToHost);
      (void)hipFree(o);
      if (e != hipSuccess) return e;
      g_step_state[dev].store(2, std::memory_order_release);
    }
  }
  for (int k = 0; k < 4; k++) ac[k] = g_step_ac[dev][k];
  return hipSuccess;
}

static thread_local unsigned long long t_launches = 0;
unsigned long long launch_count() { return t_launches; }
void count_launch() { ++t_launches; }

__global__ __launch_bounds__(64) void k_linearize_repop(DevGraph d, const double* __restrict__ pose,
                                                        const double* __restrict__ plane, LinGuard gd) {
  __shared__ double repop_lds[64 * 31];
  if (!lin_guard(gd, pose, plane)) return;
  body_linearize_repop(d, pose, plane, blockIdx.x, repop_lds);
}

bool k1_lane_form(const DevGraph& d, int mode) {
  return mode == 0 && d.n_obs + d.n_odo + d.n_pp + d.n_lp <= kLaneParallelMaxFactors && !(d.sw & SW_K1_THREAD_FORM);
}

bool k1_products(const DevGraph& d, int mode) { (void)mode; return !(d.sw & SW_K1_THREAD_FORM); }

hipError_t launch_linearize(const DevGraph& d, int mode, bool at_estimate, hipStream_t st, const LinGuard* guard, hipEvent_t ev0, hipEvent_t ev1) {
  const LinGuard gd = guard ? *guard : LinGuard{};
  if (d.n_obs > d.n_obs_fixed) {
    PPS_LAUNCH(k_linearize_repop, dim3(cdiv(d.n_obs - d.n_obs_fixed, 64)), dim3(64), 0, st, d,
                       at_estimate ? d.pose_est : d.pose_lin, at_estimate ? d.plane_est : d.plane_lin, gd);
  }
  const int nb_obs = cdiv(d.n_obs_fixed, kLinBlock), nb_odo = cdiv(d.n_odo, kLinBlock), nb_pp = cdiv(d.n_pp, kLinBlock),
            nb_lp = cdiv(d.n_lp, kLinBlock);
  const int nb = nb_obs + nb_odo + nb_pp + nb_lp;
  if (nb == 0) return hipSuccess;
  const double* pose = at_estimate ? d.pose_est : d.pose_lin;
  const double* plane = at_estimate ? d.plane_est : d.plane_lin;
  if (k1_lane_form(d, mode)) return launch_linearize_lanes(d, pose, plane, gd, st, ev0, ev1);
  if (ev0) { const hipError_t e = hipEventRecord(ev0, st); if (e != hipSuccess) return e; }
  const size_t lds0 = (size_t)(kLinBlock / 64) * 64 * 31 * sizeof(double), lds1 = (size_t)(kLinBlock / 64) * 64 * 79 * sizeof(double);
  const int nb_rest = nb - nb_obs;
  DevGraph dn = d;
  if (!k1_products(d, mode)) dn.P = nullptr;
  if (mode == 1) {
    if (nb_obs) PPS_LAUNCH((k_linearize<1, 0>), dim3(nb_obs), dim3(kLinBlock), lds0, st, dn, pose, plane, nb_obs, nb_odo, nb_pp, gd);
    if (nb_rest) PPS_LAUNCH((k_linearize<1, 1>), dim3(nb_rest), dim3(kLinBlock), lds1, st, dn, pose, plane, nb_obs, nb_odo, nb_pp, gd);
  } else {
    if (nb_obs) PPS_LAUNCH(k_linearize_obs_numeric, dim3(nb_obs), dim3(kLinBlock), lds0, st, dn, pose, plane, nb_obs, nb_odo, nb_pp, gd);
    if (nb_rest) PPS_LAUNCH((k_linearize<0, 1>), dim3(nb_rest), dim3(kLinBlock), lds1, st, dn, pose, plane, nb_obs, nb_odo, nb_pp, gd);
  }
  if (ev1) { const hipError_t e = hipEventRecord(ev1, st); if (e != hipSuccess) return e; }
  return hipGetLastError();
}

template <int MODE, int PART>
__device__ __forceinline__ void body_sweep_bench(const DevGraph& d, double* __restrict__ Jbig, int nb_obs_per, int nb_odo_per, int replicas) {
  const int per = PART == 0 ? nb_obs_per : nb_odo_per;
  const int rep = blockIdx.x / per;
  int b = blockIdx.x % per + (PART == 0 ? 0 : nb_obs_per);
  const size_t slab = (size_t)d.n_obs * 30 + (size_t)d.n_odo * 78;
  double* Jr = Jbig + (size_t)rep * slab;
  const double* obs_meas = d.obs_meas + (size_t)rep * 4 * d.obs_ld;
  const double* obs_w = d.obs_w + (size_t)rep * 6 * d.obs_ld;
  const int* obs_pose = d.obs_pose + (size_t)rep * d.n_obs;
  const int* obs_plane = d.obs_plane + (size_t)rep * d.n_obs;
  const double* odo_meas = d.odo_meas + (size_t)rep * 6 * d.odo_ld;
  const double* odo_w = d.odo_w + (size_t)rep * 21 * d.odo_ld;
  const int* odo_a = d.odo_a + (size_t)rep * d.n_odo;
  const int* odo_b = d.odo_b + (size_t)rep * d.n_odo;
  extern __shared__ double lin_lds[];
  double* lds_wave = lin_lds + (size_t)(threadIdx.x >> 6) * 64 * (PART == 0 ? 31 : 79);
  if (b < nb_obs_per) {
    const int i0 = b * kLinBlock + (threadIdx.x & ~63);
    const int i = min(b * kLinBlock + (int)threadIdx.x, d.n_obs - 1);
    double pz[7], pl[4], ms[4], w[6], out[30];
    load_pose(d.pose_lin, d.pose_ld, obs_pose[i], pz);
    load_plane(d.plane_lin, d.plane_ld, obs_plane[i], pl);
    load_soa<4>(obs_meas, d.obs_ld, i, ms);
    load_soa<6>(obs_w, d.obs_ld, i, w);
    lin_plane_obs<MODE>(pz, pl, ms, w, out);
    if (i0 < d.n_obs) store_records_coalesced<30>(out, Jr + (size_t)i0 * 30, min(64, d.n_obs - i0), lds_wave);
    return;
  }
  if (PART == 0) return;
  b -= nb_obs_per;
  const int i0 = b * kLinBlock + (threadIdx.x & ~63);
  const int i = min(b * kLinBlock + (int)threadIdx.x, d.n_odo - 1);
  double p1[7], p2[7], ms[6], w[21];
  load_pose(d.pose_lin, d.pose_ld, odo_a[i], p1);
  load_pose(d.pose_lin, d.pose_ld, odo_b[i], p2);
  load_soa<6>(odo_meas, d.odo_ld, i, ms);
  load_soa<21>(odo_w, d.odo_ld, i, w);
  if (MODE == 1) {
    double out[78];
    lin_odometry<MODE>(p1, p2, ms, w, out);
    if (i0 < d.n_odo) store_records_coalesced<78>(out, Jr + (size_t)d.n_obs * 30 + (size_t)i0 * 78, min(64, d.n_odo - i0), lds_wave);
  } else {
    lin_odometry<MODE>(p1, p2, ms, w, lds_wave + (threadIdx.x & 63) * 79);
    if (i0 < d.n_odo) flush_records_coalesced<78>(Jr + (size_t)d.n_obs * 30 + (size_t)i0 * 78, min(64, d.n_odo - i0), lds_wave);
  }
}

template <int MODE, int PART>
__global__ __launch_bounds__(kLinBlock) void k_sweep_bench(DevGraph d, double* __restrict__ Jbig, int nb_obs_per, int nb_odo_per, int replicas) {
  body_sweep_bench<MODE, PART>(d, Jbig, nb_obs_per, nb_odo_per, replicas);
}
__global__ __launch_bounds__(kLinBlock) __attribute__((amdgpu_waves_per_eu(kObsNumericWaves, kObsNumericWaves)))
void k_sweep_bench_obs_numeric(DevGraph d, double* __restrict__ Jbig, int nb_obs_per, int nb_odo_per, int replicas) {
  body_sweep_bench<0, 0>(d, Jbig, nb_obs_per, nb_odo_per, replicas);
}

hipError_t launch_sweep_bench(const DevGraph& d, int mode, int replicas, double* Jbig, int part, hipStream_t st) {
  if (mode == 2) return launch_sweep_bench_lanes(d, replicas, Jbig, part, st);
  const int nb_obs = cdiv(d.n_obs, kLinBlock), nb_odo = cdiv(d.n_odo, kLinBlock);
  const size_t lds0 = (size_t)(kLinBlock / 64) * 64 * 31 * sizeof(double), lds1 = (size_t)(kLinBlock / 64) * 64 * 79 * sizeof(double);
  if (nb_obs + nb_odo == 0) return hipSuccess;
  if (mode == 1) {
    if (nb_obs && part != 1) PPS_LAUNCH((k_sweep_bench<1, 0>), dim3(nb_obs * replicas), dim3(kLinBlock), lds0, st, d, Jbig, nb_obs, nb_odo, replicas);
    if (nb_odo && part != 0) PPS_LAUNCH((k_sweep_bench<1, 1>), dim3(nb_odo * replicas), dim3(kLinBlock), lds1, st, d, Jbig, nb_obs, nb_odo, replicas);
  } else {
    if (nb_obs && part != 1) PPS_LAUNCH(k_sweep_bench_obs_numeric, dim3(nb_obs * replicas), dim3(kLinBlock), lds0, st, d, Jbig, nb_obs, nb_odo, replicas);
// ... 45 lines not shown
```

### pop_up_slam_amd/csrc/pps_k1_lanes.hip

```cpp
#include <hip/hip_ext.h>

#include "pps_k1_body.h"

namespace pps {

__global__ __launch_bounds__(kLanesPerBlock) void k_linearize_lanes(DevGraph d, const double* __restrict__ pose,
                                                                    const double* __restrict__ plane, int nb_obs, int nb_odo,
                                                                    int nb_pp, LinGuard gd, int apply) {
  if (!lin_guard(gd, pose, plane)) return;
  body_linearize_lanes(d, pose, plane, nb_obs, nb_odo, nb_pp, blockIdx.x, apply != 0);
}


hipError_t launch_linearize_lanes(const DevGraph& d, const double* pose, const double* plane, const LinGuard& gd, hipStream_t st, hipEvent_t ev0, hipEvent_t ev1) {
  const int lb_obs = cdiv(d.n_obs_fixed, kObsPerBlock), lb_odo = cdiv(d.n_odo, kFactorsPerBlock), lb_pp = cdiv(d.n_pp, kFactorsPerBlock),
            lb_lp = cdiv(d.n_lp, kFactorsPerBlock);
  PPS_LAUNCH_EV(ev0, ev1, k_linearize_lanes, dim3(lb_obs + lb_odo + lb_pp + lb_lp), dim3(kLanesPerBlock), 0, st, d, pose, plane, lb_obs, lb_odo, lb_pp, gd, 0);
  return hipGetLastError();
}

template <int PART>
__global__ __launch_bounds__(kLanesPerBlock) void k_sweep_bench_lanes(DevGraph d, double* __restrict__ Jbig, int lb_obs_per, int lb_odo_per, int apply) {
  const int per = PART == 0 ? lb_obs_per : lb_odo_per;
  const int rep = blockIdx.x / per;
  const int b = blockIdx.x % per + (PART == 0 ? 0 : lb_obs_per);
  const size_t slab = (size_t)d.n_obs * 30 + (size_t)d.n_odo * 78;
  DevGraph r = d;
  r.J = Jbig + (size_t)rep * slab; r.joff_obs = 0; r.joff_odo = (int64_t)d.n_obs * 30;
  r.obs_meas = d.obs_meas + (size_t)rep * 4 * d.obs_ld; r.obs_w = d.obs_w + (size_t)rep * 6 * d.obs_ld;
  r.obs_pose = d.obs_pose + (size_t)rep * d.n_obs; r.obs_plane = d.obs_plane + (size_t)rep * d.n_obs;
  r.odo_meas = d.odo_meas + (size_t)rep * 6 * d.odo_ld; r.odo_w = d.odo_w + (size_t)rep * 21 * d.odo_ld;
  r.odo_a = d.odo_a + (size_t)rep * d.n_odo; r.odo_b = d.odo_b + (size_t)rep * d.n_odo;
  r.n_obs_fixed = d.n_obs;
  r.obs_dir = nullptr; r.P = nullptr;
  body_linearize_lanes(r, d.pose_lin, d.plane_lin, lb_obs_per, lb_odo_per, 0, b, apply != 0);
}


hipError_t launch_sweep_bench_lanes(const DevGraph& d, int replicas, double* Jbig, int part, hipStream_t st) {
  const int lb_obs = cdiv(d.n_obs, kObsPerBlock), lb_odo = cdiv(d.n_odo, kFactorsPerBlock);
  if (lb_obs && part != 1) PPS_LAUNCH(k_sweep_bench_lanes<0>, dim3(lb_obs * replicas), dim3(kLanesPerBlock), 0, st, d, Jbig, lb_obs, lb_odo, 0);
  if (lb_odo && part != 0) PPS_LAUNCH(k_sweep_bench_lanes<1>, dim3(lb_odo * replicas), dim3(kLanesPerBlock), 0, st, d, Jbig, lb_obs, lb_odo, 0);
  return hipGetLastError();
}

__global__ __launch_bounds__(kLanesPerBlock) void kb_linearize_lanes(BatchArgs a) {
  PPS_BATCH_PROLOGUE(BF_ACTIVE | BF_RELIN)
  const int nb_obs = dcdiv(d.n_obs_fixed, kObsPerBlock), nb_odo = dcdiv(d.n_odo, kFactorsPerBlock),
            nb_pp = dcdiv(d.n_pp, kFactorsPerBlock), nb_lp = dcdiv(d.n_lp, kFactorsPerBlock);
  if ((int)blockIdx.x >= nb_obs + nb_odo + nb_pp + nb_lp) return;
  body_linearize_lanes(d, pose_lin, plane_lin, nb_obs, nb_odo, nb_pp, blockIdx.x, a.lin_apply != 0);
}


hipError_t launch_batch_linearize_lanes(const BatchArgs& a, const BatchGeom& g, hipStream_t st) {
  PPS_LAUNCH(kb_linearize_lanes, dim3(g.lin_blocks, a.n), dim3(kLanesPerBlock), 0, st, a);
  return hipGetLastError();
}

}
```

### pop_up_slam_amd/csrc/pps_k2.hip

```cpp
#include <cstdlib>

#include "pps_kcommon.h"
#include "pps_symbolic.h"

namespace pps {

constexpr int kK2Waves = 16;

__device__ __forceinline__ double wave_segment_sum(const DevGraph& d, int rec, int4 mine, int lane, int* __restrict__ plist) {
  const int rows = __builtin_amdgcn_readlane(rec, 0), cols = __builtin_amdgcn_readlane(rec, 1), size = __builtin_amdgcn_readlane(rec, 2);
  const int cnt = __builtin_amdgcn_readlane(rec, 4);
  const int rc = rows * cols;
  const bool act = lane < size;
  const bool is_g = lane >= rc;
  const int cdiv_ = cols > 0 ? cols : 1;
  const int i = is_g ? lane - rc : lane / cdiv_;
  const int j = is_g ? 0 : lane - (lane / cdiv_) * cdiv_;
  const bool isp = lane < cnt && mine.w >= kProductFlag;
  const unsigned long long pmask = __ballot(isp);
  unsigned long long jmask = __ballot(lane < cnt && !isp);
  const double* __restrict__ J = d.J;
  const double* __restrict__ P = d.P;
  double acc = 0.0;
  const int np = __builtin_popcountll(pmask);
  const int S = size <= 12 ? 5 : (size <= 21 ? 3 : (size <= 32 ? 2 : 1));
  const int sl = lane / (size > 0 ? size : 1), en = lane - sl * size;
  const bool live = sl < S && size > 0;
  const int enc = live ? en : 0;
  double v0[16];
  if (np > 0) {
    const int rank = __builtin_popcountll(pmask & ((1ull << lane) - 1ull));
    if (isp) plist[rank] = mine.y;
    __builtin_amdgcn_wave_barrier();
#pragma unroll
    for (int u = 0; u < 16; u++) { const int k = sl + S * u; v0[u] = P[plist[k < np ? k : np - 1] + enc]; }
  }
  while (jmask) {
    const int c0 = __builtin_ctzll(jmask);
    jmask &= jmask - 1;
    const bool two = jmask != 0;
    const int c1 = two ? __builtin_ctzll(jmask) : c0;
    jmask &= jmask - 1;
    double a[2][6], bb[2][6];
#pragma unroll
    for (int u = 0; u < 2; u++) {
      const int cc = u ? c1 : c0;
      const int jv = __builtin_amdgcn_readlane(mine.x, cc), ju = __builtin_amdgcn_readlane(mine.y, cc);
      const int ro = __builtin_amdgcn_readlane(mine.z, cc), mm = __builtin_amdgcn_readlane(mine.w, cc);
      const double* pa = J + jv + i;
      const double* pb = is_g ? J + ro : J + ju + j;
      const int sb = is_g ? 1 : cols;
#pragma unroll
      for (int k = 0; k < 6; k++) {
        const bool ok = act && k < mm && (u == 0 || two);
        a[u][k] = ok ? pa[k * rows] : 0.0;
        bb[u][k] = ok ? pb[k * sb] : 0.0;
      }
    }
#pragma unroll
    for (int u = 0; u < 2; u++)
#pragma unroll
      for (int k = 0; k < 6; k++) acc = PPS_MAC(acc, a[u][k], bb[u][k]);
  }
  if (is_g) acc = -acc;
  if (!act) acc = 0.0;
  if (np > 0) {
    double pacc = 0.0;
#pragma unroll
    for (int u = 0; u < 16; u++) pacc += (live && sl + S * u < np) ? v0[u] : 0.0;
    for (int k0 = 16 * S; k0 < np; k0 += 16 * S) {
      double v[16];
#pragma unroll
      for (int u = 0; u < 16; u++) { const int k = k0 + sl + S * u; v[u] = P[plist[k < np ? k : np - 1] + enc]; }
#pragma unroll
      for (int u = 0; u < 16; u++) pacc += (live && k0 + sl + S * u < np) ? v[u] : 0.0;
    }
    __builtin_amdgcn_wave_barrier();
    double tot = pacc;
    for (int sg = 1; sg < S; sg++) tot += __shfl(pacc, lane + sg * size, 64);
    acc += act ? tot : 0.0;
  }
  return acc;
}

__device__ __forceinline__ void seg_header(const DevGraph& d, int seg, int lane, int& rec, int4& mine) {
  rec = d.srec[(size_t)seg * 8 + (lane & 7)];
  const int c0 = __builtin_amdgcn_readlane(rec, 3), cnt = __builtin_amdgcn_readlane(rec, 4);
  mine = make_int4(0, 0, 0, 0);
  if (lane < cnt) mine = reinterpret_cast<const int4*>(d.contrib)[c0 + lane];
  if (!d.P && mine.w >= kProductFlag) { mine.w -= kProductFlag; mine.y = mine.x; }
}

__device__ __forceinline__ void body_hblocks2(const DevGraph& d, int bx) {
  __shared__ double part[kK2Waves][64];
  __shared__ int plist_lds[kK2Waves][64];
  const int wave = uni(threadIdx.x >> 6), lane = threadIdx.x & 63;
  int* const plist = plist_lds[wave];
  const int nbs = (d.n_k2_single + kK2Waves - 1) / kK2Waves;
  if (bx < nbs) {
    const int slot = bx * kK2Waves + wave;
    if (slot >= d.n_k2_single) return;
    int rec; int4 mine;
    seg_header(d, uni(d.k2_single[slot]), lane, rec, mine);
    const int size = __builtin_amdgcn_readlane(rec, 2), hoff = __builtin_amdgcn_readlane(rec, 5), doff = __builtin_amdgcn_readlane(rec, 6);
    const int dst = lane < size ? d.blk_dst[doff + lane] : -1;
    const double acc = wave_segment_sum(d, rec, mine, lane, plist);
    if (lane >= size) return;
    d.H[hoff + lane] = acc;
    if (dst >= 0) d.Hf[dst] = acc;
    return;
  }
  const int b = bx - nbs;
  if (b >= d.n_k2_multi) return;
  const int seg0 = uni(d.k2_multi[2 * b]), info = uni(d.k2_multi[2 * b + 1]);
  const int nsc = info & 0xffff;
  const bool fin = (info >> 16) != 0;
  int rec0; int4 mine0;
  seg_header(d, seg0, lane, rec0, mine0);
  const int size = __builtin_amdgcn_readlane(rec0, 2), hoff = __builtin_amdgcn_readlane(rec0, 5), doff = __builtin_amdgcn_readlane(rec0, 6);
  const int dst = (fin && wave == 0 && lane < size) ? d.blk_dst[doff + lane] : -1;
  double acc = 0.0;
  for (int sgi = wave; sgi < nsc; sgi += kK2Waves) {
    int rec; int4 mine;
    if (sgi == 0) { rec = rec0; mine = mine0; } else seg_header(d, seg0 + sgi, lane, rec, mine);
    acc += wave_segment_sum(d, rec, mine, lane, plist);
  }
  part[wave][lane] = acc;
  __syncthreads();
  if (wave != 0 || lane >= size) return;
  const int nw = nsc < kK2Waves ? nsc : kK2Waves;
  double q[4] = {0.0, 0.0, 0.0, 0.0};
#pragma unroll
  for (int w = 0; w < 4; w++)
    for (int v = w; v < nw; v += 4) q[w] += part[v][lane];
  const double tot = (q[0] + q[1]) + (q[2] + q[3]);
  d.H[hoff + lane] = tot;
  if (dst >= 0) d.Hf[dst] = tot;
}

constexpr int kK2Chunk = 16;
__device__ __forceinline__ void body_hfinish(const DevGraph& d, int bx) {
  const int lane = threadIdx.x & 63;
  const int seg0 = uni(d.k2_finish[bx]);
  const int rec = d.srec[(size_t)seg0 * 8 + (lane & 7)];
  const int size = __builtin_amdgcn_readlane(rec, 2), hoff = __builtin_amdgcn_readlane(rec, 5), doff = __builtin_amdgcn_readlane(rec, 6);
  const int nseg = __builtin_amdgcn_readlane(rec, 7);
  const int nch = (nseg + kK2Chunk - 1) / kK2Chunk;
  const int ln = lane < size ? lane : 0;
  const int dst = lane < size ? d.blk_dst[doff + lane] : -1;
  double* __restrict__ h = d.H + hoff;
  double tot = 0.0;
  for (int c0 = 0; c0 < nch; c0 += 16) {
    double v[16];
#pragma unroll
    for (int u = 0; u < 16; u++) { const int c = c0 + u; v[u] = h[(size_t)(c < nch ? c : 0) * kK2Chunk * size + ln]; }
#pragma unroll
    for (int u = 0; u < 16; u++) tot += c0 + u < nch ? v[u] : 0.0;
  }
  if (lane >= size) return;
  h[lane] = tot;
  if (dst >= 0) d.Hf[dst] = tot;
}
__global__ __launch_bounds__(64) void k_hfinish(DevGraph d, LinGuard gd) { if (!lin_guard(gd)) return; body_hfinish(d, blockIdx.x); }

__global__ __launch_bounds__(64 * kK2Waves) void k_hblocks2(DevGraph d, LinGuard gd) { if (!lin_guard(gd)) return; body_hblocks2(d, blockIdx.x); }

hipError_t launch_hblocks_spec(const DevGraph& d_in, const SpecLin& sl, hipStream_t st, const LinGuard* guard) {
  DevGraph d = d_in;
  d.J = sl.J; d.P = sl.P; d.H = sl.H; d.Hf = sl.Hf;
  return launch_hblocks(d, st, guard, true);
}

hipError_t launch_hblocks(const DevGraph& d_in, hipStream_t st, const LinGuard* guard, bool products) {
  const int nb = (d_in.n_k2_single + kK2Waves - 1) / kK2Waves + d_in.n_k2_multi;
  if (nb == 0) return hipSuccess;
  const LinGuard gd = guard ? *guard : LinGuard{};
  DevGraph d = d_in;
  if (!products) d.P = nullptr;
  PPS_LAUNCH(k_hblocks2, dim3(nb), dim3(64 * kK2Waves), 0, st, d, gd);
  if (d.n_k2_finish > 0) PPS_LAUNCH(k_hfinish, dim3(d.n_k2_finish), dim3(64), 0, st, d, gd);
  return hipGetLastError();
}

constexpr int kH2Slots = 8;
constexpr int kH2Stride = 80;
constexpr int kH2WaveDoubles = kH2Slots * kH2Stride;

struct SegHdr { int rec; int4 mine; int dst; };
__device__ __forceinline__ void seg_fetch_record(const DevGraph& d, int seg, int lane, SegHdr& h) {
  h.rec = seg >= 0 ? d.srec[(size_t)seg * 8 + (lane & 7)] : 0;
}
__device__ __forceinline__ void seg_fetch_contrib(const DevGraph& d, int lane, SegHdr& h) {
  const int size = __builtin_amdgcn_readlane(h.rec, 2), c0 = __builtin_amdgcn_readlane(h.rec, 3), cnt = __builtin_amdgcn_readlane(h.rec, 4);
  const int doff = __builtin_amdgcn_readlane(h.rec, 6), nsegb = __builtin_amdgcn_readlane(h.rec, 7);
  h.mine = make_int4(0, 0, 0, 0);
  if (lane < cnt) h.mine = reinterpret_cast<const int4*>(d.contrib)[c0 + lane];
  if (h.mine.w >= kProductFlag) { h.mine.w -= kProductFlag; h.mine.y = h.mine.x; }
  h.dst = (lane < size && nsegb == 1) ? d.blk_dst[doff + lane] : -1;
}

__device__ __forceinline__ void wave_hblock_segment(const DevGraph& d, const SegHdr& h, double* __restrict__ S) {
  const int lane = threadIdx.x & 63;
  const int rec = h.rec;
  const int4 mine = h.mine;
  const int dst = h.dst;
  const int rows = __builtin_amdgcn_readlane(rec, 0), cols = __builtin_amdgcn_readlane(rec, 1), size = __builtin_amdgcn_readlane(rec, 2);
  const int cnt = __builtin_amdgcn_readlane(rec, 4);
  const int hoff = __builtin_amdgcn_readlane(rec, 5);
  if (size == 0) return;
  const int rc = rows * cols;
  const bool act = lane < size;
  const bool is_g = lane >= rc;
  const int cdiv_ = cols > 0 ? cols : 1;
  const int i = is_g ? lane - rc : lane / cdiv_;
  const int j = is_g ? 0 : lane - (lane / cdiv_) * cdiv_;
  const double* __restrict__ J = d.J;
  double acc = 0.0;
  for (int cb = 0; cb < cnt; cb += kH2Slots) {
    const int nc = cnt - cb < kH2Slots ? cnt - cb : kH2Slots;
    if (nc == 1) {
      const int jv = __builtin_amdgcn_readlane(mine.x, cb), ju = __builtin_amdgcn_readlane(mine.y, cb);
// ... 300 lines not shown
```

### pop_up_slam_amd/csrc/pps_k4.hip

```cpp
#include <algorithm>
#include <cstdlib>

#include <hip/hip_ext.h>

#include "pps_geom.h"
#include "pps_kcommon.h"
#include "pps_k1_body.h"

namespace pps {

template <bool TRIAL>
__device__ __forceinline__ void body_retract(const DevGraph& d, double* __restrict__ pose_lin, double* __restrict__ pose_est,
                                             double* __restrict__ plane_lin, double* __restrict__ plane_est, int bx, double* red) {
  const int i = bx * blockDim.x + threadIdx.x;
  double dn = 0.0;
  if (i < d.n_pose) {
    double p[7], o[7], dl[6];
    load_pose(pose_lin, d.pose_ld, i, p);
    const int off = d.pose_voff[i];
#pragma unroll
    for (int k = 0; k < 6; k++) { dl[k] = d.delta[off + k]; dn += dl[k] * dl[k]; }
    pose_exmap(p, dl, o);
    if (TRIAL) {
#pragma unroll
      for (int k = 0; k < 7; k++) { pose_est[(size_t)k * d.pose_ld + i] = p[k]; pose_lin[(size_t)k * d.pose_ld + i] = o[k]; }
    } else {
#pragma unroll
      for (int k = 0; k < 7; k++) pose_est[(size_t)k * d.pose_ld + i] = o[k];
    }
  } else if (i < d.n_pose + d.n_plane) {
    const int l = i - d.n_pose;
    double p[4], o[4], dl[3];
    load_plane(plane_lin, d.plane_ld, l, p);
    const int off = d.plane_voff[l];
#pragma unroll
    for (int k = 0; k < 3; k++) { dl[k] = d.delta[off + k]; dn += dl[k] * dl[k]; }
    plane_exmap(p, dl, o);
    if (TRIAL) {
#pragma unroll
      for (int k = 0; k < 4; k++) { plane_est[(size_t)k * d.plane_ld + l] = p[k]; plane_lin[(size_t)k * d.plane_ld + l] = o[k]; }
    } else {
#pragma unroll
      for (int k = 0; k < 4; k++) plane_est[(size_t)k * d.plane_ld + l] = o[k];
    }
  }
#pragma unroll
  for (int o2 = 32; o2 > 0; o2 >>= 1) dn += __shfl_down(dn, o2, 64);
  if ((threadIdx.x & 63) == 0) red[threadIdx.x >> 6] = dn;
  __syncthreads();
  if (threadIdx.x == 0) d.dn_partials[bx] = red[0] + red[1] + red[2] + red[3];
}

template <bool TRIAL>
__global__ __launch_bounds__(256) void k_retract(DevGraph d) {
  __shared__ double red[4];
  body_retract<TRIAL>(d, d.pose_lin, d.pose_est, d.plane_lin, d.plane_est, blockIdx.x, red);
}

hipError_t launch_retract_trial(const DevGraph& d, hipStream_t st) {
  const int n = d.n_pose + d.n_plane;
  if (n == 0) return hipSuccess;
  PPS_LAUNCH(k_retract<true>, dim3(cdiv(n, 256)), dim3(256), 0, st, d);
  return hipGetLastError();
}
hipError_t launch_retract_apply(const DevGraph& d, hipStream_t st) {
  const int n = d.n_pose + d.n_plane;
  if (n == 0) return hipSuccess;
  PPS_LAUNCH(k_retract<false>, dim3(cdiv(n, 256)), dim3(256), 0, st, d);
  return hipGetLastError();
}

constexpr int kChiBlock = 256;

__device__ __forceinline__ void chi2_finish(const DevGraph& d, int nb, int n_dn, double* __restrict__ out, double seq) {
  double cs = 0.0, dn = 0.0;
  for (int i = threadIdx.x; i < nb; i += kChiBlock) cs += __hip_atomic_load(&d.chi2_partials[i], __ATOMIC_RELAXED, __HIP_MEMORY_SCOPE_AGENT);
  for (int i = threadIdx.x; i < n_dn; i += kChiBlock) dn += __hip_atomic_load(&d.dn_partials[i], __ATOMIC_RELAXED, __HIP_MEMORY_SCOPE_AGENT);
#pragma unroll
  for (int o = 32; o > 0; o >>= 1) { cs += __shfl_down(cs, o, 64); dn += __shfl_down(dn, o, 64); }
  __shared__ double red2[2][kChiBlock / 64];
  if ((threadIdx.x & 63) == 0) { red2[0][threadIdx.x >> 6] = cs; red2[1][threadIdx.x >> 6] = dn; }
  __syncthreads();
  if (threadIdx.x == 0) {
    double a = 0.0, b2 = 0.0;
    for (int k = 0; k < kChiBlock / 64; k++) { a += red2[0][k]; b2 += red2[1][k]; }
    const double npd = __hip_atomic_load(&d.result_dev[2], __ATOMIC_RELAXED, __HIP_MEMORY_SCOPE_AGENT);
    d.result_dev[0] = a; d.result_dev[1] = b2; d.result_dev[2] = 0.0;
    out[0] = a; out[1] = b2; out[2] = npd;
    __hip_atomic_store(&out[3], seq, __ATOMIC_RELEASE, __HIP_MEMORY_SCOPE_SYSTEM);
  }
}

template <bool TICKET = true, bool APPLY = false>
__device__ __forceinline__ void body_chi2(const DevGraph& d, const double* __restrict__ pose,
                                          const double* __restrict__ plane, int nb_obs, int nb_odo, int nb_pp,
                                          int n_dn, double* __restrict__ out, double seq, int bx, int nb, int total_blocks = 0) {
  __shared__ double red[kChiBlock / 64];
  int b = bx;
  double s = 0.0;
  if (b < nb_obs) {
    const int i = b * kChiBlock + threadIdx.x;
    if (i < d.n_obs) {
      double pz[7], pl[4], ms[4], w[6], e[3], r[3];
      fetch_pose<APPLY>(d, pose, d.obs_pose[i], pz);
      fetch_plane<APPLY>(d, plane, d.obs_plane[i], pl);
      if (i < d.n_obs_fixed) load_soa<4>(d.obs_meas, d.obs_ld, i, ms);
      else {
        double ray[6];
        load_soa<6>(d.obs_ray, d.n_obs - d.n_obs_fixed, i - d.n_obs_fixed, ray);
        repop_wall_plane(pz, ray, ms);
      }
      load_soa<6>(d.obs_w, d.obs_ld, i, w);
      res_plane_obs(pz, pl, ms, e);
      whiten<3>(w, e, r);
      s = r[0] * r[0] + r[1] * r[1] + r[2] * r[2];
    }
  } else if ((b -= nb_obs) < nb_odo) {
    const int i = b * kChiBlock + threadIdx.x;
    if (i < d.n_odo) {
      double p1[7], p2[7], ms[6], w[21], e[6], r[6];
      fetch_pose<APPLY>(d, pose, d.odo_a[i], p1);
      fetch_pose<APPLY>(d, pose, d.odo_b[i], p2);
      load_soa<6>(d.odo_meas, d.odo_ld, i, ms);
      load_soa<21>(d.odo_w, d.odo_ld, i, w);
      res_odometry(p1, p2, ms, e);
      whiten<6>(w, e, r);
#pragma unroll
      for (int k = 0; k < 6; k++) s += r[k] * r[k];
    }
  } else if ((b -= nb_odo) < nb_pp) {
    const int i = b * kChiBlock + threadIdx.x;
    if (i < d.n_pp) {
      double pz[7], ms[6], w[21], e[6], r[6];
      fetch_pose<APPLY>(d, pose, d.pp_pose[i], pz);
      load_soa<6>(d.pp_meas, d.pp_ld, i, ms);
      load_soa<21>(d.pp_w, d.pp_ld, i, w);
      res_pose_prior(pz, ms, e);
      whiten<6>(w, e, r);
#pragma unroll
      for (int k = 0; k < 6; k++) s += r[k] * r[k];
    }
  } else {
    b -= nb_pp;
    const int i = b * kChiBlock + threadIdx.x;
    if (i < d.n_lp) {
      double pl[4], ms[4], w[6], e[3], r[3];
      fetch_plane<APPLY>(d, plane, d.lp_plane[i], pl);
      load_soa<4>(d.lp_meas, d.lp_ld, i, ms);
      load_soa<6>(d.lp_w, d.lp_ld, i, w);
      res_plane_prior(pl, ms, e);
      whiten<3>(w, e, r);
      s = r[0] * r[0] + r[1] * r[1] + r[2] * r[2];
    }
  }
#pragma unroll
  for (int o = 32; o > 0; o >>= 1) s += __shfl_down(s, o, 64);
  if ((threadIdx.x & 63) == 0) red[threadIdx.x >> 6] = s;
  __syncthreads();
  if (!TICKET) {
    if (threadIdx.x == 0) { double t = 0.0; for (int k = 0; k < kChiBlock / 64; k++) t += red[k]; d.chi2_partials[bx] = t; }
    return;
  }
  __shared__ bool last;
  if (threadIdx.x == 0) {
    double t = 0.0;
    for (int k = 0; k < kChiBlock / 64; k++) t += red[k];
    d.chi2_partials[bx] = t;
    __builtin_amdgcn_fence(__ATOMIC_RELEASE, "agent");
    asm volatile("s_waitcnt vmcnt(0)" ::: "memory");
    last = atomicAdd(d.ticket, 1u) == (unsigned int)((total_blocks > 0 ? total_blocks : nb) - 1);
  }
  __syncthreads();
  if (!last) return;
  if (threadIdx.x == 0) __builtin_amdgcn_fence(__ATOMIC_ACQUIRE, "agent");
  __syncthreads();
  chi2_finish(d, nb, n_dn, out, seq);
  if (threadIdx.x == 0) *d.ticket = 0u;
}

__global__ __launch_bounds__(kChiBlock) void k_chi2(DevGraph d, const double* __restrict__ pose,
                                                    const double* __restrict__ plane, int nb_obs, int nb_odo, int nb_pp,
                                                    int n_dn, double* __restrict__ out, double seq) {
  body_chi2(d, pose, plane, nb_obs, nb_odo, nb_pp, n_dn, out, seq, blockIdx.x, gridDim.x);
}

__device__ __forceinline__ void body_retract_to(const DevGraph& d, const double* __restrict__ base_pose, const double* __restrict__ base_plane,
                                                double* __restrict__ out_pose, double* __restrict__ out_plane, int bx, double* red) {
  const int i = bx * blockDim.x + threadIdx.x;
  double dn = 0.0;
  if (i < d.n_pose) {
    double p[7], o[7], dl[6];
    load_pose(base_pose, d.pose_ld, i, p);
    const int off = d.pose_voff[i];
#pragma unroll
    for (int k = 0; k < 6; k++) { dl[k] = d.delta[off + k]; dn += dl[k] * dl[k]; }
    pose_exmap(p, dl, o);
#pragma unroll
    for (int k = 0; k < 7; k++) out_pose[(size_t)k * d.pose_ld + i] = o[k];
  } else if (i < d.n_pose + d.n_plane) {
    const int l = i - d.n_pose;
    double p[4], o[4], dl[3];
    load_plane(base_plane, d.plane_ld, l, p);
    const int off = d.plane_voff[l];
#pragma unroll
    for (int k = 0; k < 3; k++) { dl[k] = d.delta[off + k]; dn += dl[k] * dl[k]; }
    plane_exmap(p, dl, o);
#pragma unroll
    for (int k = 0; k < 4; k++) out_plane[(size_t)k * d.plane_ld + l] = o[k];
  }
#pragma unroll
  for (int o2 = 32; o2 > 0; o2 >>= 1) dn += __shfl_down(dn, o2, 64);
  if ((threadIdx.x & 63) == 0) red[threadIdx.x >> 6] = dn;
  __syncthreads();
  if (threadIdx.x == 0) d.dn_partials[bx] = red[0] + red[1] + red[2] + red[3];
}

__global__ __launch_bounds__(kChiBlock) void k_trial_dual(DevGraph d, DualAlt alt, const double* __restrict__ base_pose, const double* __restrict__ base_plane,
                                                          double* __restrict__ out_pose, double* __restrict__ out_plane, double* __restrict__ out_pose1,
                                                          double* __restrict__ out_plane1, int nb_ret, int nb_obs, int nb_odo, int nb_pp, int nb_chi,
                                                          double* __restrict__ out, double seq, double* __restrict__ out1, double seq1) {
  if (blockIdx.y) {
    d.delta = alt.delta; d.chi2_partials = alt.chi2_partials; d.dn_partials = alt.dn_partials; d.ticket = alt.ticket; d.result_dev = alt.result_dev;
    out_pose = out_pose1; out_plane = out_plane1; out = out1; seq = seq1;
  }
  const int total = nb_ret + nb_chi;
  if ((int)blockIdx.x >= nb_ret) {
    body_chi2<true, true>(d, base_pose, base_plane, nb_obs, nb_odo, nb_pp, nb_ret, out, seq, (int)blockIdx.x - nb_ret, nb_chi, total);
    return;
  }
  __shared__ double red[4];
  body_retract_to(d, base_pose, base_plane, out_pose, out_plane, blockIdx.x, red);
  __shared__ bool last;
  if (threadIdx.x == 0) {
    __builtin_amdgcn_fence(__ATOMIC_RELEASE, "agent");
    asm volatile("s_waitcnt vmcnt(0)" ::: "memory");
    last = atomicAdd(d.ticket, 1u) == (unsigned int)(total - 1);
  }
  __syncthreads();
  if (!last) return;
  if (threadIdx.x == 0) __builtin_amdgcn_fence(__ATOMIC_ACQUIRE, "agent");
  __syncthreads();
  chi2_finish(d, nb_chi, nb_ret, out, seq);
  if (threadIdx.x == 0) *d.ticket = 0u;
}

hipError_t launch_trial_dual(const DevGraph& d, const DualAlt& alt, const double* base_pose, const double* base_plane, double* out_pose0,
                             double* out_plane0, double* out_pose1, double* out_plane1, double* host_result0, double seq0, double* host_result1,
                             double seq1, hipStream_t st, int n_trials) {
  const int n = d.n_pose + d.n_plane;
  const int nb_obs = cdiv(d.n_obs, kChiBlock), nb_odo = cdiv(d.n_odo, kChiBlock), nb_pp = cdiv(d.n_pp, kChiBlock), nb_lp = cdiv(d.n_lp, kChiBlock);
  const int nb = nb_obs + nb_odo + nb_pp + nb_lp;
  if (nb == 0 || n == 0) return hipErrorInvalidValue;
  const int nb_ret = cdiv(n, 256);
  PPS_LAUNCH(k_trial_dual, dim3(nb_ret + nb, n_trials), dim3(kChiBlock), 0, st, d, alt, base_pose, base_plane, out_pose0, out_plane0, out_pose1, out_plane1, nb_ret,
             nb_obs, nb_odo, nb_pp, nb, host_result0, seq0, host_result1, seq1);
  return hipGetLastError();
}

__global__ __launch_bounds__(kChiBlock) void k_trial_lin(DevGraph d, DualAlt alt, SpecLin sl, const double* __restrict__ base_pose, const double* __restrict__ base_plane,
                                                         double* __restrict__ out_pose, double* __restrict__ out_plane, double* __restrict__ out_pose1,
                                                         double* __restrict__ out_plane1, int nb_ret, int nb_obs, int nb_odo, int nb_pp, int nb_chi,
                                                         double* __restrict__ out, double seq, double* __restrict__ out1, double seq1, int lb_obs, int lb_odo, int lb_pp, int apply) {
  static_assert(kChiBlock == kLanesPerBlock, "one block size for the trial blocks and the lane-form sweep");
  const int total = nb_ret + nb_chi;
  const bool sweep = (int)blockIdx.x >= 2 * total;
  const int y = sweep ? sl.which : ((int)blockIdx.x >= total ? 1 : 0);
  const int bx0 = sweep ? (int)blockIdx.x - 2 * total : (int)blockIdx.x - y * total;
  if (y) {
    d.delta = alt.delta; d.chi2_partials = alt.chi2_partials; d.dn_partials = alt.dn_partials; d.ticket = alt.ticket; d.result_dev = alt.result_dev;
    out_pose = out_pose1; out_plane = out_plane1; out = out1; seq = seq1;
  }
  if (sweep) {
    d.J = sl.J; d.P = sl.P; d.H = sl.H; d.Hf = sl.Hf;
    body_linearize_lanes(d, base_pose, base_plane, lb_obs, lb_odo, lb_pp, bx0, apply != 0);
    return;
  }
  if (bx0 >= nb_ret) {
    body_chi2<true, true>(d, base_pose, base_plane, nb_obs, nb_odo, nb_pp, nb_ret, out, seq, bx0 - nb_ret, nb_chi, total);
    return;
  }
  __shared__ double red[4];
  body_retract_to(d, base_pose, base_plane, out_pose, out_plane, bx0, red);
  __shared__ bool last;
  if (threadIdx.x == 0) {
    __builtin_amdgcn_fence(__ATOMIC_RELEASE, "agent");
    asm volatile("s_waitcnt vmcnt(0)" ::: "memory");
    last = atomicAdd(d.ticket, 1u) == (unsigned int)(total - 1);
  }
  __syncthreads();
  if (!last) return;
  if (threadIdx.x == 0) __builtin_amdgcn_fence(__ATOMIC_ACQUIRE, "agent");
  __syncthreads();
  chi2_finish(d, nb_chi, nb_ret, out, seq);
  if (threadIdx.x == 0) *d.ticket = 0u;
}

int trial_lin_waves(const DevGraph& d) {
  const int nb = cdiv(d.n_obs, kChiBlock) + cdiv(d.n_odo, kChiBlock) + cdiv(d.n_pp, kChiBlock) + cdiv(d.n_lp, kChiBlock) + cdiv(d.n_pose + d.n_plane, 256);
  const int lb = cdiv(d.n_obs_fixed, kObsPerBlock) + cdiv(d.n_odo, kFactorsPerBlock) + cdiv(d.n_pp, kFactorsPerBlock) + cdiv(d.n_lp, kFactorsPerBlock);
  return (2 * nb + lb) * (kChiBlock / 64);
}
bool trial_lin_ok(const DevGraph& d, int mode) { return k1_lane_form(d, mode) && d.n_obs == d.n_obs_fixed && d.P != nullptr; }

hipError_t launch_trial_lin(const DevGraph& d, const DualAlt& alt, const SpecLin& sl, const double* base_pose, const double* base_plane, double* out_pose0,
                            double* out_plane0, double* out_pose1, double* out_plane1, double* host_result0, double seq0, double* host_result1,
                            double seq1, hipStream_t st, hipEvent_t ev0, hipEvent_t ev1) {
  const int n = d.n_pose + d.n_plane;
  const int nb_obs = cdiv(d.n_obs, kChiBlock), nb_odo = cdiv(d.n_odo, kChiBlock), nb_pp = cdiv(d.n_pp, kChiBlock), nb_lp = cdiv(d.n_lp, kChiBlock);
  const int nb = nb_obs + nb_odo + nb_pp + nb_lp;
  if (nb == 0 || n == 0) return hipErrorInvalidValue;
  const int nb_ret = cdiv(n, 256);
  const int lb_obs = cdiv(d.n_obs_fixed, kObsPerBlock), lb_odo = cdiv(d.n_odo, kFactorsPerBlock), lb_pp = cdiv(d.n_pp, kFactorsPerBlock),
            lb_lp = cdiv(d.n_lp, kFactorsPerBlock);
  const int lb_all = lb_obs + lb_odo + lb_pp + lb_lp;
  PPS_LAUNCH_EV(ev0, ev1, k_trial_lin, dim3(2 * (nb_ret + nb) + lb_all), dim3(kChiBlock), 0, st, d, alt, sl, base_pose, base_plane, out_pose0,
                out_plane0, out_pose1, out_plane1, nb_ret, nb_obs, nb_odo, nb_pp, nb, host_result0, seq0, host_result1, seq1, lb_obs, lb_odo, lb_pp, 1);
  return hipGetLastError();
}

hipError_t launch_chi2(const DevGraph& d, bool at_estimate, double* host_result, double seq, hipStream_t st) {
  const int nb_obs = cdiv(d.n_obs, kChiBlock), nb_odo = cdiv(d.n_odo, kChiBlock), nb_pp = cdiv(d.n_pp, kChiBlock),
            nb_lp = cdiv(d.n_lp, kChiBlock);
  const int nb = nb_obs + nb_odo + nb_pp + nb_lp;
  const double* pose = at_estimate ? d.pose_est : d.pose_lin;
  const double* plane = at_estimate ? d.plane_est : d.plane_lin;
  if (nb == 0) return hipErrorInvalidValue;
  const int n_dn = cdiv(d.n_pose + d.n_plane, 256);
  PPS_LAUNCH(k_chi2, dim3(nb), dim3(kChiBlock), 0, st, d, pose, plane, nb_obs, nb_odo, nb_pp, n_dn, host_result, seq);
  return hipGetLastError();
}

__global__ __launch_bounds__(kChiBlock) void k_chi2_trial(DevGraph d, int nb_obs, int nb_odo, int nb_pp, int n_dn, double* __restrict__ out, double seq) {
  body_chi2<true, true>(d, d.pose_est, d.plane_est, nb_obs, nb_odo, nb_pp, n_dn, out, seq, blockIdx.x, gridDim.x);
}

hipError_t launch_chi2_trial(const DevGraph& d, double* host_result, double seq, hipStream_t st) {
  const int nb_obs = cdiv(d.n_obs, kChiBlock), nb_odo = cdiv(d.n_odo, kChiBlock), nb_pp = cdiv(d.n_pp, kChiBlock),
            nb_lp = cdiv(d.n_lp, kChiBlock);
  const int nb = nb_obs + nb_odo + nb_pp + nb_lp;
  if (nb == 0) return hipErrorInvalidValue;
  PPS_LAUNCH(k_chi2_trial, dim3(nb), dim3(kChiBlock), 0, st, d, nb_obs, nb_odo, nb_pp, cdiv(d.n_pose + d.n_plane, 256), host_result, seq);
  return hipGetLastError();
}

__global__ __launch_bounds__(kChiBlock) void kb_chi2(BatchArgs a, int slot) {
  PPS_BATCH_PROLOGUE(BF_ACTIVE)
  const int nb_obs = dcdiv(d.n_obs, kChiBlock), nb_odo = dcdiv(d.n_odo, kChiBlock), nb_pp = dcdiv(d.n_pp, kChiBlock),
            nb_lp = dcdiv(d.n_lp, kChiBlock);
  const int nb = nb_obs + nb_odo + nb_pp + nb_lp;
  if ((int)blockIdx.x >= nb) return;
  body_chi2<false>(d, pose_lin, plane_lin, nb_obs, nb_odo, nb_pp, dcdiv(d.n_pose + d.n_plane, 256),
                   a.results + (size_t)(a.alt ? 12 : 8) * (size_t)(a.b0 + b) + 4 * slot, a.seq, blockIdx.x, nb);
}

__global__ __launch_bounds__(kChiBlock) void kb_chi2_finish(BatchArgs a, int slot, int dual) {
  PPS_BATCH_PROLOGUE(BF_ACTIVE)
  const int nb = dcdiv(d.n_obs, kChiBlock) + dcdiv(d.n_odo, kChiBlock) + dcdiv(d.n_pp, kChiBlock) + dcdiv(d.n_lp, kChiBlock);
  const int n_dn = dcdiv(d.n_pose + d.n_plane, 256);
  if (!dual) { chi2_finish(d, nb, n_dn, a.results + (size_t)(a.alt ? 12 : 8) * (size_t)(a.b0 + b) + 4 * slot, a.seq); return; }
  DevGraph d2 = d;
  if (blockIdx.z) {
    const BatchAlt al = load_alt(a.alt + a.b0 + b);
    d2.chi2_partials = al.chi2_partials; d2.dn_partials = al.dn_partials; d2.result_dev = al.result_dev;
  }
  chi2_finish(d2, nb, n_dn, a.results + 12 * (size_t)(a.b0 + b) + 4 * (1 + blockIdx.z), a.seq);
}

hipError_t launch_batch_chi2(const BatchArgs& a, const BatchGeom& g, int slot, hipStream_t st) {
  if (g.chi2 <= 0) return hipErrorInvalidValue;
  PPS_LAUNCH(kb_chi2, dim3(g.chi2, a.n), dim3(kChiBlock), 0, st, a, slot);
  PPS_LAUNCH(kb_chi2_finish, dim3(1, a.n), dim3(kChiBlock), 0, st, a, slot, 0);
  return hipGetLastError();
}

__global__ __launch_bounds__(64) void kb_begin_dual(BatchArgs a) {
  PPS_BATCH_PROLOGUE(BF_ACTIVE)
  const BatchAlt al = load_alt(a.alt + a.b0 + b);
  if (threadIdx.x < 4) { d.result_dev[threadIdx.x] = 0.0; al.result_dev[threadIdx.x] = 0.0; }
}

__global__ __launch_bounds__(kChiBlock) void kb_trial_dual(BatchArgs a, int nb_ret) {
  __shared__ double red[4];
  PPS_BATCH_PROLOGUE(BF_ACTIVE)
  const BatchAlt al = load_alt(a.alt + a.b0 + b);
  const int xs = a.xsel[b], z = blockIdx.z;
  const int ts = (xs + 1 + z) % 3;
  DevGraph d2 = d;
  if (z) { d2.delta = al.delta; d2.chi2_partials = al.chi2_partials; d2.dn_partials = al.dn_partials; d2.ticket = al.ticket; d2.result_dev = al.result_dev; }
  if ((int)blockIdx.x < nb_ret) {
    if ((int)blockIdx.x * 256 >= d.n_pose + d.n_plane) return;
    body_retract_to(d2, pose_lin, plane_lin, sel3(al.pose, ts), sel3(al.plane, ts), blockIdx.x, red);
    return;
  }
  const int nb_obs = dcdiv(d.n_obs, kChiBlock), nb_odo = dcdiv(d.n_odo, kChiBlock), nb_pp = dcdiv(d.n_pp, kChiBlock),
            nb_lp = dcdiv(d.n_lp, kChiBlock);
  const int nb = nb_obs + nb_odo + nb_pp + nb_lp;
  const int bx = (int)blockIdx.x - nb_ret;
  if (bx >= nb) return;
  body_chi2<false, true>(d2, pose_lin, plane_lin, nb_obs, nb_odo, nb_pp, dcdiv(d.n_pose + d.n_plane, 256),
// ... 89 lines not shown
```

### pop_up_slam_amd/csrc/pps_solve.cpp

```cpp
#include "pps_graph.h"

using namespace pps;
using namespace pps_impl;

namespace pps_impl {

struct PhaseTimer {
  pps_graph* g; double* acc; bool on;
  PhaseTimer(pps_graph* g_, double* a) : g(g_), acc(a), on(g_->profiling >= 2) { if (on) (void)hipEventRecord(g->ev[0], g->stream); }
  ~PhaseTimer() {
    if (!on) return;
    (void)hipEventRecord(g->ev[1], g->stream);
    (void)hipEventSynchronize(g->ev[1]);
    float ms = 0;
    (void)hipEventElapsedTime(&ms, g->ev[0], g->ev[1]);
    *acc += 1e-3 * ms;
  }
};

int do_linearize(pps_graph* g, const LinGuard* guard = nullptr) {
  if (g->profiling == 1) {
    if (g->k1_used + 2 > (int)g->k1_events.size()) {
      for (int k = 0; k < 2; k++) { hipEvent_t e; HIP_TRY(g, hipEventCreate(&e)); g->k1_events.push_back(e); }
    }
    g->k1_skip.resize(g->k1_events.size() / 2, 0);
    g->k1_skip[g->k1_used / 2] = 0;
    HIP_TRY(g, launch_linearize(g->dev, g->props.jacobian_mode, false, g->stream, guard, g->k1_events[g->k1_used], g->k1_events[g->k1_used + 1]));
    g->k1_used += 2;
  } else
  { PhaseTimer t(g, &g->stats.t_linearize); HIP_TRY(g, launch_linearize(g->dev, g->props.jacobian_mode, false, g->stream, guard)); }
  { PhaseTimer t(g, &g->stats.t_assemble); HIP_TRY(g, launch_hblocks(g->dev, g->stream, guard, k1_products(g->dev, g->props.jacobian_mode))); }
  if (!guard) g->stats.n_linearize++;
  return PPS_OK;
}

static int enqueue_factor_solve(pps_graph* g, const DevGraph& dv, const DualAlt* alt, double lambda, hipStream_t st_, bool events) {
  const Analysis& A = g->an;
  if (g->k3_all) {
    hipEvent_t e0 = nullptr, e1 = nullptr;
    if (events) {
      if (g->fk_used + 2 > (int)g->fk_events.size()) for (int k = 0; k < 2; k++) { hipEvent_t e; HIP_TRY(g, hipEventCreate(&e)); g->fk_events.push_back(e); }
      e0 = g->fk_events[g->fk_used]; e1 = g->fk_events[g->fk_used + 1]; g->fk_used += 2;
    }
    g->k3_epoch = g->k3_epoch >= (1 << 30) ? 1 : g->k3_epoch + 1;
    HIP_TRY(g, launch_band_all(dv, alt, A.n_groups, g->k3_nw_factor, g->k3_nw_solve, g->k3_max_front, g->k3_max_panel, g->k3_max_grp, lambda, g->k3_epoch, st_, e0, e1));
    return PPS_OK;
  }
  const int top = A.n_stages - 1;
  const bool fuse = top >= 0 && band_root_fusable(dv, A.stage_grp_off[top + 1] - A.stage_grp_off[top], A.stage_max_front[top]);
  for (int st = 0; st < A.n_stages; st++) {
    hipEvent_t e0 = nullptr, e1 = nullptr;
    if (events) {
      if (g->fk_used + 2 > (int)g->fk_events.size()) for (int k = 0; k < 2; k++) { hipEvent_t e; HIP_TRY(g, hipEventCreate(&e)); g->fk_events.push_back(e); }
      e0 = g->fk_events[g->fk_used]; e1 = g->fk_events[g->fk_used + 1]; g->fk_used += 2;
    }
    const int g0 = A.stage_grp_off[st], ng = A.stage_grp_off[st + 1] - g0;
    const bool pre = st < (int)g->stage_pre.size() && g->stage_pre[st] != 0;
    if (fuse && st == top)
      HIP_TRY(g, launch_band_root(dv, alt, g0, g->stage_nw_factor[st], g->stage_nw_solve[st], A.stage_max_front[st], g->stage_max_panel[st],
                                  g->stage_max_grp_fronts[st], lambda, st_, e0, e1, pre));
    else if (alt) HIP_TRY(g, launch_band_factor_dual(dv, *alt, g0, ng, g->stage_nw_factor[st], A.stage_max_front[st], lambda, st_, e0, e1, pre));
    else HIP_TRY(g, launch_band_factor(dv, g0, ng, g->stage_nw_factor[st], A.stage_max_front[st], lambda, st_, e0, e1, pre));
  }
  for (int st = fuse ? top - 1 : top; st >= 0; st--)
    HIP_TRY(g, launch_band_solve(dv, A.stage_grp_off[st], A.stage_grp_off[st + 1] - A.stage_grp_off[st], g->stage_nw_solve[st],
                                 g->stage_max_panel[st], g->stage_max_grp_fronts[st], st_, alt));
  return PPS_OK;
}

int do_solve_on(pps_graph* g, const DevGraph& dv, double lambda, hipStream_t st_) { return enqueue_factor_solve(g, dv, nullptr, lambda, st_, false); }

int do_solve(pps_graph* g, double lambda) {
  const Analysis& A = g->an;
  if (g->use_band) {
    if (g->profiling < 2) {
      int rc = do_solve_on(g, g->dev, lambda, g->stream);
      if (rc != PPS_OK) return rc;
      g->stats.n_factorize++;
      return PPS_OK;
    }
    {
      PhaseTimer t(g, &g->stats.t_factor);
      for (int st = 0; st < A.n_stages; st++)
        HIP_TRY(g, launch_band_factor(g->dev, A.stage_grp_off[st], A.stage_grp_off[st + 1] - A.stage_grp_off[st], g->stage_nw_factor[st],
                                      A.stage_max_front[st], lambda, g->stream));
    }
    {
      PhaseTimer t(g, &g->stats.t_backsolve);
      for (int st = A.n_stages - 1; st >= 0; st--)
        HIP_TRY(g, launch_band_solve(g->dev, A.stage_grp_off[st], A.stage_grp_off[st + 1] - A.stage_grp_off[st], g->stage_nw_solve[st],
                                     g->stage_max_panel[st], g->stage_max_grp_fronts[st], g->stream));
    }
    g->stats.n_factorize++;
    return PPS_OK;
  }
  if (g->use_dense) {
    {
      PhaseTimer t(g, &g->stats.t_factor);
      HIP_TRY(g, hipMemsetAsync(g->dev.L, 0, (size_t)A.L_size * 8, g->stream));
      HIP_TRY(g, launch_dense_hpush(g->dev, g->max_el_per_front, lambda, g->stream));
      for (int l = 0; l < A.n_levels; l++) {
        const int base = A.level_off[l] + l, cnt = A.level_off[l + 1] - A.level_off[l];
        HIP_TRY(g, launch_dense_factor_level(g->dev, A.level_off[l], cnt, g->d_dw_asm + base, g->dw_asm[base + cnt], g->d_dw_pan + base,
                                             g->dw_pan[base + cnt], g->d_dw_trl + base, g->dw_trl[base + cnt], g->stream));
      }
    }
    {
      PhaseTimer t(g, &g->stats.t_backsolve);
      for (int l = A.n_levels - 1; l >= 0; l--)
        HIP_TRY(g, launch_dense_solve_level(g->dev, A.level_off[l], A.level_off[l + 1] - A.level_off[l], g->level_max_b[l], g->stream));
    }
    g->stats.n_factorize++;
    return PPS_OK;
  }
// ... 118 lines not shown
    if (g->spec_result) HIP_TRY(g, hipMemsetAsync(g->spec_result, 0, 4 * sizeof(double), g->stream));
  }
  g->status_clean = false;
  rc = copy_state(g, true); if (rc != PPS_OK) return rc;
  rc = do_linearize(g); if (rc != PPS_OK) return rc;
  rc = do_solve(g, 0.0); if (rc != PPS_OK) return rc;
  double chi2 = 0.0, dn = 0.0; bool notpd = false;
  if (g->n_live_factors > 0 && g->dev.n_pose + g->dev.n_plane > 0) {
    const DevGraph& d = g->dev;
    { PhaseTimer t(g, &g->stats.t_retract_chi2);
      HIP_TRY(g, launch_trial_dual(d, DualAlt{}, d.pose_lin, d.plane_lin, d.pose_est, d.plane_est, nullptr, nullptr, g->host_result, 0.0, nullptr, 0.0, g->stream, 1)); }
    rc = enqueue_state_download(g); if (rc != PPS_OK) return rc;
    HIP_TRY(g, hipStreamSynchronize(g->stream));
    chi2 = g->host_result[0]; dn = std::sqrt(g->host_result[1]); notpd = g->host_result[2] != 0.0;
    if (g->host_result[2] >= kStatusInternal) return fail(g, PPS_EHIP, "internal error: a hand-over flag between the waves or workgroups of a K3 launch never arrived (the step was discarded)");
  } else {
    { PhaseTimer t(g, &g->stats.t_retract_chi2); HIP_TRY(g, launch_retract_apply(g->dev, g->stream)); }
    rc = enqueue_state_download(g); if (rc != PPS_OK) return rc;
    rc = read_result(g, true, &chi2, &dn, &notpd); if (rc != PPS_OK) return rc;
  }
  resolve_k1_events(g);
  if (notpd) {
    rc = copy_state(g, false); if (rc != PPS_OK) return rc;
    HIP_TRY(g, hipStreamSynchronize(g->stream));
    g->stats.t_total = now_s() - t0; g->stats.n_launches = (int)(launch_count() - g->launches0);
    return fail(g, PPS_ENOTPD, "normal equations not positive definite");
  }
  g->dev_values_newer = true;
  state_download_arrived(g);
  g->status_clean = true;
  g->stats.chi2_final = chi2; g->stats.last_delta_norm = dn; g->stats.lambda_final = 0;
  g->stats.t_total = now_s() - t0; g->stats.n_launches = (int)(launch_count() - g->launches0);
  return PPS_OK;
}

static int lm_solve(pps_graph* g, int* iterations);

int pps_batch_optimize(pps_graph* g, int* iterations) {
  if (!g) return PPS_EINVAL;
  cov_invalidate(g);
  if (g->n_live_nodes > 0 && g->n_live_factors == 0) {
    begin_solve(g);
    if (iterations) *iterations = 0;
    return PPS_OK;
  }
  const int rc = lm_solve(g, iterations);
  if (rc != PPS_OK && rc != PPS_ENOTPD) abandon_device_copy(g);
  return rc;
}

static int end_lm_solve(pps_graph* g, const LmControl& lm, const LmSink& sink, int* iterations, double t0) {
  { const int rc2 = enqueue_state_download(g); if (rc2 != PPS_OK) return rc2; }
  HIP_TRY(g, hipStreamSynchronize(g->stream));
  g->dev_values_newer = true;
  state_download_arrived(g);
  g->status_clean = true;
  resolve_k1_events(g);
  g->stats.t_total = now_s() - t0; g->stats.n_launches = (int)(launch_count() - g->launches0);
  if (g->dev.trace) report_front_trace(g);
  if (lm.finish(sink, iterations) != PPS_OK) return fail(g, PPS_ENOTPD, kLmNotPdMessage);
  return PPS_OK;
}

static int lm_solve_dual(pps_graph* g, int* iterations, double t0) {
  const pps_props& prop = g->props;
  const Analysis& A = g->an;
  if (!g->status_clean) {
    HIP_TRY(g, launch_clear_status(g->dev, g->stream));
    HIP_TRY(g, hipMemsetAsync(g->spec_result, 0, 4 * sizeof(double), g->stream));
  }
  g->status_clean = false;
  LmControl lm(prop);
  const LmSink sink = lm_sink(g, prop.verbose != 0);
  double* slot0 = g->host_result;
  double* slot[2] = {g->host_result + 4, g->host_result + 8};
  DevGraph& d = g->dev;
  int rc = copy_state(g, true); if (rc != PPS_OK) return rc;
  double *t_pose[2] = {d.pose_est, g->spec_pose}, *t_plane[2] = {d.plane_est, g->spec_plane};
  double seqs[2] = {0, 0};
  const bool adaptive = A.n_fronts >= 2048;
  bool use_alt = !adaptive;
  bool have_next = true;
  const bool fuse_lin = !g->sw.no_spec_lin && g->spec_J != nullptr && trial_lin_ok(d, prop.jacobian_mode) && trial_lin_waves(d) <= 3072;
  int fused_pair = -1;
  int pred = 0, pred_launched = 0;
  bool error_known = false;
  auto enqueue_trial_lin = [&](const DualAlt& alt, double s0, double s1) -> int {
    pred_launched = use_alt ? pred : 0;
    const SpecLin sl{g->spec_J, g->spec_P, g->spec_H, g->spec_Hf, pred_launched};
    hipEvent_t e0 = nullptr, e1 = nullptr;
    fused_pair = -1;
    if (g->profiling == 1) {
      if (g->k1_used + 2 > (int)g->k1_events.size()) for (int k = 0; k < 2; k++) { hipEvent_t e; HIP_TRY(g, hipEventCreate(&e)); g->k1_events.push_back(e); }
      g->k1_skip.resize(g->k1_events.size() / 2, 0);
      fused_pair = g->k1_used / 2;
      g->k1_skip[fused_pair] = 1;
      e0 = g->k1_events[g->k1_used]; e1 = g->k1_events[g->k1_used + 1]; g->k1_used += 2;
    }
    HIP_TRY(g, launch_trial_lin(d, alt, sl, d.pose_lin, d.plane_lin, t_pose[0], t_plane[0], t_pose[1], t_plane[1], slot[0], s0, slot[1], s1, g->stream, e0, e1));
    const LinGuard gd{{d.result_dev, g->spec_result}, {nullptr, nullptr}, {nullptr, nullptr}, lm.error, error_known ? 1 : 0, use_alt ? 0 : 1, pred_launched};
    HIP_TRY(g, launch_hblocks_spec(d, sl, g->stream, &gd));
    return PPS_OK;
  };
  auto enqueue_dual = [&](double lam) -> int {
    DualAlt alt{g->spec_L, g->spec_U, g->spec_delta, g->spec_result, g->spec_chi2_partials, g->spec_dn_partials, g->spec_ticket,
                lam * prop.lm_lambda_factor};
    have_next = use_alt;
    const int n_trials = use_alt ? 2 : 1;
    { const int rc2 = enqueue_factor_solve(g, d, use_alt ? &alt : nullptr, lam, g->stream, g->profiling == 1); if (rc2 != PPS_OK) return rc2; }
    g->stats.n_factorize += n_trials;
    g->seq += 1.0; seqs[0] = g->seq;
    g->seq2 += 1.0; seqs[1] = g->seq2;
    if (fuse_lin) return enqueue_trial_lin(alt, seqs[0], seqs[1]);
    HIP_TRY(g, launch_trial_dual(d, alt, d.pose_lin, d.plane_lin, t_pose[0], t_plane[0], t_pose[1], t_plane[1], slot[0], seqs[0], slot[1], seqs[1],
                                 g->stream, n_trials));
    return PPS_OK;
  };
  rc = do_linearize(g); if (rc != PPS_OK) return rc;
  g->seq += 1.0;
  const double seq0 = g->seq;
  HIP_TRY(g, launch_chi2(d, false, slot0, seq0, g->stream));
  const bool spec_lin = !g->sw.no_spec_lin && !fuse_lin && !adaptive;
  int spec_pair = -1;
  auto enqueue_spec_lin = [&](double err) -> int {
    if (!spec_lin) return PPS_OK;
    LinGuard gd{{d.result_dev, g->spec_result}, {t_pose[0], t_pose[1]}, {t_plane[0], t_plane[1]}, err, 1, have_next ? 0 : 1};
    spec_pair = g->profiling == 1 ? g->k1_used / 2 : -1;
    return do_linearize(g, &gd);
  };
  auto drop_spec_lin = [&]() { if (spec_pair >= 0 && (size_t)spec_pair < g->k1_skip.size()) g->k1_skip[spec_pair] = 1; spec_pair = -1; };
  rc = enqueue_dual(lm.lambda); if (rc != PPS_OK) return rc;
  rc = wait_result(g, slot0, seq0); if (rc != PPS_OK) return rc;
  lm.error = slot0[0]; error_known = true;
  g->stats.chi2_initial = lm.error;
  rc = enqueue_spec_lin(lm.error); if (rc != PPS_OK) return rc;
  rc = wait_result(g, slot[0], seqs[0]); if (rc != PPS_OK) return rc;
  int cur = 0;
  lm.take_step(slot[0]);
  bool trial_taken = false;
  while (lm.running(prop)) {
    const LmVerdict v = lm.judge(sink, slot[cur][0]);
    if (v == LmVerdict::Converged) { trial_taken = true; break; }
    if (v == LmVerdict::Accepted) {
      if (adaptive) use_alt = cur != 0;
      pred = cur;
      std::swap(d.pose_lin, t_pose[cur]); std::swap(d.plane_lin, t_plane[cur]);
      if (fuse_lin && cur == pred_launched) {
        std::swap(d.J, g->spec_J); std::swap(d.P, g->spec_P); std::swap(d.H, g->spec_H); std::swap(d.Hf, g->spec_Hf);
        g->stats.n_linearize++;
        if (fused_pair >= 0 && (size_t)fused_pair < g->k1_skip.size()) g->k1_skip[fused_pair] = 0;
      }
      else if (fuse_lin) { rc = do_linearize(g); if (rc != PPS_OK) return rc; }
      else if (spec_lin) { g->stats.n_linearize++; spec_pair = -1; }
      else { rc = do_linearize(g); if (rc != PPS_OK) return rc; }
      rc = enqueue_dual(lm.lambda); if (rc != PPS_OK) return rc;
      rc = enqueue_spec_lin(lm.error); if (rc != PPS_OK) return rc;
      cur = 0;
      rc = wait_result(g, slot[0], seqs[0]); if (rc != PPS_OK) return rc;
    } else {
      if (have_next) {
        cur = 1; have_next = false;
        rc = wait_result(g, slot[1], seqs[1]); if (rc != PPS_OK) return rc;
      } else {
        drop_spec_lin();
        if (adaptive) use_alt = true;
        rc = enqueue_dual(lm.lambda); if (rc != PPS_OK) return rc;
        rc = enqueue_spec_lin(lm.error); if (rc != PPS_OK) return rc;
        cur = 0;
        rc = wait_result(g, slot[0], seqs[0]); if (rc != PPS_OK) return rc;
      }
    }
    lm.take_step(slot[cur]);
  }
  drop_spec_lin();
  if (trial_taken) { std::swap(d.pose_lin, t_pose[cur]); std::swap(d.plane_lin, t_plane[cur]); }
  d.pose_est = d.pose_lin; d.plane_est = d.plane_lin;
  d.pose_lin = t_pose[0]; d.plane_lin = t_plane[0];
  g->spec_pose = t_pose[1]; g->spec_plane = t_plane[1];
  return end_lm_solve(g, lm, sink, iterations, t0);
}

static int lm_solve(pps_graph* g, int* iterations) {
  const double t0 = now_s();
  begin_solve(g);
// ... 54 lines not shown
```

### pop_up_slam_amd/csrc/pps_upload.cpp

```cpp
#include "pps_graph.h"

using namespace pps;
using namespace pps_impl;

namespace pps_impl {

void free_device(pps_graph* g) {
  for (void* p : g->allocs) (void)hipFree(p);
  g->allocs.clear();
  for (pps_graph::Arena* a : {&g->up, &g->scr}) {
    const size_t want = (a == &g->up ? std::max(a->off, g->up_high) : a->off) + a->spill;
    if (a->spill > 0 || a->base == nullptr) {
      if (a->base) (void)hipFree(a->base);
      a->cap = std::max<size_t>(size_t(1) << 20, 2 * want);
      if (hipMalloc(reinterpret_cast<void**>(&a->base), a->cap) != hipSuccess) { a->base = nullptr; a->cap = 0; }
      if (a == &g->up) { g->up_slots.clear(); g->up_high = 0; g->up_unknown = true; }
    }
    a->off = 0; a->spill = 0;
  }
  g->up_cursor = 0; g->up_patches.clear();
  if (g->stage_cap < g->up.cap) {
    if (g->stage) (void)hipHostFree(g->stage);
    g->stage = nullptr; g->stage_cap = 0;
    if (hipHostMalloc(reinterpret_cast<void**>(&g->stage), g->up.cap, hipHostMallocDefault) == hipSuccess) g->stage_cap = g->up.cap;
// ... 382 lines not shown
  if (sync) HIP_TRY(g, hipStreamSynchronize(g->stream));
  else g->up_inflight = true;
  g->host_values_newer = false;
  return PPS_OK;
}

template <int K>
void pack_soa(const pps_graph* g, int type, const double HostFactor::*dummy, bool weights, std::vector<double>& out, size_t ld) {
  (void)dummy;
  const std::vector<int>& ids = g->fslot_ids[type];
  const size_t n = ids.size();
  out.assign((size_t)K * ld, 0.0);
  for (size_t s = 0; s < n; s++) {
    const HostFactor& f = g->factors[ids[s]];
    const double* src = weights ? f.w : f.meas;
    for (int k = 0; k < K; k++) out[(size_t)k * ld + s] = src[k];
  }
}

int download_measurements(pps_graph* g) {
  if (!g->dev_meas_newer) return PPS_OK;
  HIP_TRY(g, hipSetDevice(g->props.device));
  const DevGraph& d = g->dev;
  const size_t n = g->fslot_ids[F_PLANE_OBS].size(), ld = (size_t)d.obs_ld;
  std::vector<double> m((size_t)4 * ld);
  if (n) HIP_TRY(g, hipMemcpyAsync(m.data(), d.obs_meas, m.size() * 8, hipMemcpyDeviceToHost, g->stream));
  HIP_TRY(g, hipStreamSynchronize(g->stream));
  for (size_t s2 = 0; s2 < n && s2 < (size_t)d.n_obs; s2++) {
    HostFactor& f = g->factors[g->fslot_ids[F_PLANE_OBS][s2]];
    for (int k = 0; k < 4; k++) f.meas[k] = m[(size_t)k * ld + s2];
  }
  g->dev_meas_newer = false;
  g->pk_meas_ok = false;
  return PPS_OK;
}

int upload_measurements(pps_graph* g) {
  DevGraph& d = g->dev;
  std::vector<double> m;
  pack_soa<4>(g, F_PLANE_OBS, nullptr, false, m, (size_t)d.obs_ld);
  if (d.n_obs) HIP_TRY(g, hipMemcpyAsync(d.obs_meas, m.data(), m.size() * 8, hipMemcpyHostToDevice, g->stream));
  std::vector<double> m2;
  pack_soa<4>(g, F_PLANE_PRIOR, nullptr, false, m2, (size_t)d.lp_ld);
  if (d.n_lp) HIP_TRY(g, hipMemcpyAsync(d.lp_meas, m2.data(), m2.size() * 8, hipMemcpyHostToDevice, g->stream));
  g->up_unknown_meas = true;
  HIP_TRY(g, hipStreamSynchronize(g->stream));
  g->meas_dirty = false;
  return PPS_OK;
}

int upload_all(pps_graph* g) {
  const double t0 = now_s();
  const bool was_grown_only = g->grown_only_upload;
  const bool tm = g->sw.upload_timing;
  g->verify_hints = g->sw.verify_upload;
  double tl = t0;
  auto lap = [&](const char* what) { if (!tm) return; const double t = now_s(); g->up_laps[what] += t - tl; tl = t; };
  int rc = ensure_device(g);
  if (rc != PPS_OK) return rc;
  lap("0 ensure_device");
  if (g->dev_values_newer) { rc = download_state(g); if (rc != PPS_OK) return rc; }
  lap("1a state download");
  bool keep_meas = false;
  const size_t n_obs_on_device = (size_t)g->dev.n_obs;
  if (g->dev_meas_newer) {
    const size_t n_obs_new = (size_t)g->n_live_type[F_PLANE_OBS], n_lp_new = (size_t)g->n_live_type[F_PLANE_PRIOR];
    const bool any_repop = g->n_live_repop > 0;
    keep_meas = g->grown_only_upload && !g->up_unknown && !g->up_unknown_meas && g->up.spill == 0 && !any_repop && g->dev.n_obs == g->dev.n_obs_fixed &&
                j_capacity((int64_t)n_obs_new) == g->dev.obs_ld && j_capacity((int64_t)n_lp_new) == g->dev.lp_ld && g->slot_obs_meas < g->up_slots.size() &&
                true;
    if (!keep_meas) {
      if (tm) g->up_laps["(measurement downloads, count)"] += 1e-3;
      rc = download_measurements(g); if (rc != PPS_OK) return rc;
    }
  }
  lap("1b measurements");
  if (!g->analyzed || g->analysis_stale) { rc = run_analysis(g); if (rc != PPS_OK) return rc; }
  lap("3 analysis");
  HIP_TRY(g, hipStreamSynchronize(g->stream));
  g->up_inflight = false;
  lap("1c opening stream sync");
  free_device(g);
  g->spec_L = g->spec_U = g->spec_delta = nullptr; g->spec_result = nullptr;
  g->spec_pose = g->spec_plane = g->spec_chi2_partials = g->spec_dn_partials = nullptr; g->spec_ticket = nullptr;
  g->spec_J = g->spec_P = g->spec_H = g->spec_Hf = nullptr;
  g->d_item_frame = g->d_item_plane = g->d_item_slot = g->d_frame_pose_slot = g->d_frame_seg_off = nullptr; g->d_fr_seg = nullptr;
  g->frames_dirty = true;
  g->snap_pose = g->snap_plane = nullptr; g->upload_version++;
  lap("2 free_device");
  const Analysis& A = g->an;
  DevGraph& d = g->dev;
  const bool hints = was_grown_only && !g->up_unknown && g->up_an_seq >= 0 && g->an_base_seq == g->up_an_seq;
  const Analysis::Kept K = hints ? A.kept : Analysis::Kept();
  const size_t kF = (size_t)K.fronts, kFl = (size_t)K.fronts_lists, kB = (size_t)K.blocks, kS = (size_t)K.segs;
  auto at = [](const auto& v, size_t i) -> size_t { return i < v.size() ? (size_t)v[i] : 0; };
  double* zero_block = nullptr; size_t zero_doubles = 0;
  d.n_pose = (int)g->pose_ids.size(); d.n_plane = (int)g->plane_ids.size();
  d.no_strip = g->sw.no_strip ? 1 : 0;
  d.sw = g->sw.dev_bits();
  HIP_TRY(g, step_constants(d.step_ac));
  d.pose_ld = std::max(1, (d.n_pose + 63) / 64 * 64); d.plane_ld = std::max(1, (d.n_plane + 63) / 64 * 64);
#define TRY(x) do { rc = (x); if (rc != PPS_OK) return rc; } while (0)
  const size_t state_doubles = (size_t)7 * d.pose_ld + (size_t)4 * d.plane_ld;
  TRY(dev_alloc(g, &d.pose_est, state_doubles)); d.plane_est = d.pose_est + (size_t)7 * d.pose_ld;
  TRY(dev_alloc(g, &d.pose_lin, state_doubles)); d.plane_lin = d.pose_lin + (size_t)7 * d.pose_ld;
  std::vector<int> pv(d.n_pose), lv(d.n_plane);
  for (int s = 0; s < d.n_pose; s++) pv[s] = A.node_voff[g->nodes[g->pose_ids[s]].compact];
  for (int s = 0; s < d.n_plane; s++) lv[s] = A.node_voff[g->nodes[g->plane_ids[s]].compact];
  TRY(dev_upload(g, &d.pose_voff, pv)); TRY(dev_upload(g, &d.plane_voff, lv));
  d.n_obs = (int)g->fslot_ids[F_PLANE_OBS].size(); d.n_odo = (int)g->fslot_ids[F_ODOMETRY].size();
  d.n_pp = (int)g->fslot_ids[F_POSE_PRIOR].size(); d.n_lp = (int)g->fslot_ids[F_PLANE_PRIOR].size();
  { int64_t base[4]; j_bases(g, base, nullptr); d.joff_obs = base[F_PLANE_OBS]; d.joff_odo = base[F_ODOMETRY]; d.joff_pp = base[F_POSE_PRIOR]; d.joff_lp = base[F_PLANE_PRIOR]; }
  auto idx_of = [&](int type, bool second) {
    std::vector<int> v(g->fslot_ids[type].size());
    for (size_t s = 0; s < v.size(); s++) {
      const HostFactor& f = g->factors[g->fslot_ids[type][s]];
      v[s] = g->nodes[second ? f.b : f.a].slot;
    }
    return v;
  };
  std::vector<double> tmp;
  const bool incr_pack = was_grown_only;
  d.obs_ld = (int)j_capacity(d.n_obs); d.odo_ld = (int)j_capacity(d.n_odo); d.pp_ld = (int)j_capacity(d.n_pp); d.lp_ld = (int)j_capacity(d.n_lp);
  {
    const std::vector<int>& ids = g->fslot_ids[F_PLANE_OBS];
    const size_t n = ids.size(), ld = (size_t)d.obs_ld;
    std::vector<int>& ia = g->pk_obs_a; std::vector<int>& ib = g->pk_obs_b;
    std::vector<double>& pm = g->pk_obs_m; std::vector<double>& pw = g->pk_obs_w;
    size_t s_begin = 0;
    if (incr_pack && g->pk_ld_obs == ld && g->pk_n_obs <= n && pm.size() == 4 * ld && g->pk_obs_ids.size() == g->pk_n_obs &&
        std::equal(g->pk_obs_ids.begin(), g->pk_obs_ids.end(), ids.begin())) s_begin = g->pk_n_obs;
    ia.resize(n); ib.resize(n); pm.resize(4 * ld); pw.resize(6 * ld);
    for (size_t s2 = s_begin; s2 < n; s2++) {
      const HostFactor& f = g->factors[ids[s2]];
      ia[s2] = g->nodes[f.a].slot; ib[s2] = g->nodes[f.b].slot;
      for (int k = 0; k < 4; k++) pm[(size_t)k * ld + s2] = f.meas[k];
      for (int k = 0; k < 6; k++) pw[(size_t)k * ld + s2] = f.w[k];
    }
    if (s_begin > 0 && !g->pk_meas_ok)
      for (size_t s2 = 0; s2 < s_begin; s2++) { const HostFactor& f = g->factors[ids[s2]]; for (int k = 0; k < 4; k++) pm[(size_t)k * ld + s2] = f.meas[k]; }
    g->pk_n_obs = n; g->pk_ld_obs = ld; g->pk_obs_ids.resize(s_begin); g->pk_obs_ids.insert(g->pk_obs_ids.end(), ids.begin() + (std::ptrdiff_t)s_begin, ids.end());
    const size_t same_idx = hints ? s_begin : 0, same_meas = (hints && g->pk_meas_ok) ? s_begin : 0;
    TRY(dev_upload(g, &d.obs_pose, ia, same_idx)); TRY(dev_upload(g, &d.obs_plane, ib, same_idx));
    g->slot_obs_meas = g->up_cursor;
    TRY(dev_upload_rows(g, &d.obs_meas, pm, 4, ld, n, g->up_unknown_meas, keep_meas ? std::min(n, n_obs_on_device) : kNoExact, same_meas));
    TRY(dev_upload_rows(g, &d.obs_w, pw, 6, ld, n, false, kNoExact, same_idx));
  }
  d.n_obs_fixed = g->n_obs_fixed;
  {
    const std::vector<int>& ids = g->fslot_ids[F_PLANE_OBS];
    const size_t n2 = ids.size() - (size_t)g->n_obs_fixed;
    if (n2 > 0) {
      tmp.assign(6 * n2, 0.0);
      for (size_t k = 0; k < n2; k++)
        for (int c = 0; c < 6; c++) tmp[(size_t)c * n2 + k] = g->factors[ids[g->n_obs_fixed + k]].ray[c];
      TRY(dev_upload(g, &d.obs_ray, tmp));
    }
  }
  {
    const std::vector<int>& ids = g->fslot_ids[F_ODOMETRY];
    const size_t n = ids.size(), ld = (size_t)d.odo_ld;
    std::vector<int>& ia = g->pk_odo_a; std::vector<int>& ib = g->pk_odo_b;
    std::vector<double>& pm = g->pk_odo_m; std::vector<double>& pw = g->pk_odo_w;
    size_t s_begin = 0;
    if (incr_pack && g->pk_ld_odo == ld && g->pk_n_odo <= n && pm.size() == 6 * ld && g->pk_odo_ids.size() == g->pk_n_odo &&
        std::equal(g->pk_odo_ids.begin(), g->pk_odo_ids.end(), ids.begin())) s_begin = g->pk_n_odo;
    ia.resize(n); ib.resize(n); pm.resize(6 * ld); pw.resize(21 * ld);
// ... 17 lines not shown
  pack_soa<6>(g, F_PLANE_PRIOR, nullptr, true, tmp, (size_t)d.lp_ld); TRY(dev_upload_rows(g, &d.lp_w, tmp, 6, (size_t)d.lp_ld, (size_t)d.n_lp, false));
  g->up_unknown_meas = false;
  g->pk_meas_ok = true;
  lap("4 factor packing + diff");
  TRY(dev_alloc(g, &d.J, (size_t)A.J_size)); TRY(dev_alloc(g, &d.H, (size_t)A.H_size));
  TRY(dev_alloc(g, &d.P, (size_t)std::max<int64_t>(1, A.P_size)));
  { int64_t pb[4]; p_bases(g, pb, nullptr); d.poff_obs = pb[F_PLANE_OBS]; }
  TRY(dev_alloc(g, &d.L, (size_t)A.L_size)); TRY(dev_alloc(g, &d.U, (size_t)A.U_size));
  TRY(dev_alloc(g, &g->spec_L, (size_t)A.L_size)); TRY(dev_alloc(g, &g->spec_U, (size_t)A.U_size));
  const size_t delta_doubles = (size_t)std::max(1, A.n_scalars);
  d.n_scalars = A.n_scalars;
  d.n_fronts = A.n_fronts; d.n_levels = A.n_levels; d.max_front = A.max_front; d.n_segs = A.n_segs; d.n_blocks = A.n_blocks;
  TRY(dev_upload(g, &d.f_p, A.f_p, kF)); TRY(dev_upload(g, &d.f_b, A.f_b, kF)); TRY(dev_upload(g, &d.f_poff, A.f_poff, kF)); TRY(dev_upload(g, &d.pidx, A.pidx, kF ? at(A.f_poff, kF) : 0));
  TRY(dev_upload(g, &d.f_Loff, A.f_Loff, kF)); TRY(dev_upload(g, &d.f_Uoff, A.f_Uoff, kF));
  TRY(dev_upload(g, &d.f_bidx_off, A.f_bidx_off, kF ? kF + 1 : 0)); TRY(dev_upload(g, &d.bidx, A.bidx, kF ? at(A.f_bidx_off, kF) : 0));
  TRY(dev_upload(g, &d.f_child_off, A.f_child_off, kF ? kF + 1 : 0)); TRY(dev_upload(g, &d.child, A.child, kF ? at(A.f_child_off, kF) : 0));
  TRY(dev_upload(g, &d.f_cmap_off, A.f_cmap_off, kF ? kF + 1 : 0)); TRY(dev_upload(g, &d.cmap, A.cmap));
  TRY(dev_upload(g, &d.level_fronts, A.level_fronts));
  const size_t kA = kFl ? at(A.f_asm_off, kFl) : 0;
  TRY(dev_upload(g, &d.f_asm_off, A.f_asm_off, kFl ? kFl + 1 : 0)); TRY(dev_upload(g, &d.asm_blk, A.asm_blk, kA));
  TRY(dev_upload(g, &d.asm_lrow, A.asm_lrow, kA)); TRY(dev_upload(g, &d.asm_lcol, A.asm_lcol, kA));
  TRY(dev_upload(g, &d.blk_rows, A.blk_rows, kB)); TRY(dev_upload(g, &d.blk_cols, A.blk_cols, kB));
  TRY(dev_upload(g, &d.blk_size, A.blk_size, kB)); TRY(dev_upload(g, &d.blk_nseg, A.blk_nseg, kB));
  TRY(dev_upload(g, &d.blk_hoff, A.blk_hoff, kB));
  TRY(dev_upload(g, &d.seg_blk, A.seg_blk, kS)); TRY(dev_upload(g, &d.seg_c0, A.seg_c0, kS)); TRY(dev_upload(g, &d.seg_cnt, A.seg_cnt, kS));
  TRY(dev_upload(g, &d.seg_hoff, A.seg_hoff, kS));
  TRY(dev_upload(g, &d.contrib, A.contrib, 4 * (size_t)K.contribs));
  {
    std::vector<int> mseg;
    for (int bk = 0; bk < A.n_blocks; bk++) if (A.blk_nseg[bk] > 1) mseg.push_back(bk);
    d.n_mseg = (int)mseg.size();
    TRY(dev_upload(g, &d.mseg_blk, mseg));
    std::vector<int> k2s, k2m, k2f;
    for (int sg : A.nd_segs) if (A.blk_nseg[A.seg_blk[sg]] == 1) k2s.push_back(sg);
    for (int sg = 0; sg < A.n_segs; sg++) {
      const int ns = A.blk_nseg[A.seg_blk[sg]];
      if (ns <= 1 || (sg > 0 && A.seg_blk[sg - 1] == A.seg_blk[sg])) continue;
      for (int c0 = 0; c0 < ns; c0 += 16) { k2m.push_back(sg + c0); k2m.push_back(std::min(16, ns - c0) | (ns <= 16 ? 1 << 16 : 0)); }
      if (ns > 16) k2f.push_back(sg);
    }
    d.n_k2_single = (int)k2s.size(); d.n_k2_multi = (int)k2m.size() / 2; d.n_k2_finish = (int)k2f.size();
    TRY(dev_upload(g, &d.k2_single, k2s)); TRY(dev_upload(g, &d.k2_multi, k2m)); TRY(dev_upload(g, &d.k2_finish, k2f));
  }
  TRY(dev_upload(g, &d.f_el_off, A.f_el_off, kFl ? kFl + 1 : 0)); TRY(dev_alloc(g, &d.el_tgt, (size_t)std::max<int64_t>(1, A.el_total)));
  TRY(dev_upload(g, &d.asm_el0, A.asm_el0, kA)); TRY(dev_upload(g, &d.asm_fsz, A.asm_fsz, kA));
  TRY(dev_upload(g, &d.f_ea_off, A.f_ea_off, kF ? kF + 1 : 0)); TRY(dev_alloc(g, &d.ea_tgt, (size_t)std::max<int64_t>(1, A.ea_total)));
  TRY(dev_upload(g, &d.blk_doff, A.blk_doff, kB ? kB + 1 : 0)); TRY(dev_alloc(g, &d.blk_dst, (size_t)std::max(1, A.blk_doff[A.n_blocks])));
  TRY(dev_alloc(g, &d.Hf, (size_t)A.el_total));
  if (g->use_band && !g->sw.no_spec_lin) {
    TRY(dev_alloc(g, &g->spec_J, (size_t)A.J_size)); TRY(dev_alloc(g, &g->spec_P, (size_t)std::max<int64_t>(1, A.P_size)));
    TRY(dev_alloc(g, &g->spec_H, (size_t)A.H_size)); TRY(dev_alloc(g, &g->spec_Hf, (size_t)A.el_total));
  }
  TRY(dev_upload(g, &d.grp_lvl_off, A.grp_lvl_off)); TRY(dev_upload(g, &d.glvl_front_off, A.glvl_front_off));
  {
    std::vector<int> span(8 * (size_t)std::max(1, A.n_groups), 0);
    for (int gi = 0; gi < A.n_groups; gi++) {
      const int l0 = A.grp_lvl_off[gi], nl = A.grp_lvl_off[gi + 1] - l0;
      int* r = &span[8 * (size_t)gi];
      r[0] = A.glvl_front_off[l0]; r[1] = A.glvl_front_off[l0 + nl] - r[0]; r[2] = nl;
      for (int k = 1; k <= 4; k++) r[2 + k] = A.glvl_front_off[l0 + std::min(k, nl)];
    }
    TRY(dev_upload(g, &d.grp_span, span));
  }
  TRY(dev_upload(g, &d.glvl_fronts, A.glvl_fronts));
  TRY(dev_upload(g, &d.frec, A.frec)); TRY(dev_upload(g, &d.crec, A.crec)); TRY(dev_upload(g, &d.srec, A.srec, 8 * kS));
  TRY(dev_upload(g, &d.obs_dir, A.obs_dir)); TRY(dev_upload(g, &d.nd_segs, A.nd_segs, (size_t)K.nd_segs)); d.n_nd_segs = (int)A.nd_segs.size();
  TRY(dev_upload(g, &d.cls_off, A.cls_off)); TRY(dev_upload(g, &d.cls_fronts, A.cls_fronts));
  if (g->use_dense) { TRY(dev_upload(g, &g->d_dw_asm, g->dw_asm)); TRY(dev_upload(g, &g->d_dw_pan, g->dw_pan)); TRY(dev_upload(g, &g->d_dw_trl, g->dw_trl)); }
  d.chi2_blocks = (d.n_obs + 255) / 256 + (d.n_odo + 255) / 256 + (d.n_pp + 255) / 256 + (d.n_lp + 255) / 256;
  TRY(dev_alloc(g, &d.chi2_partials, (size_t)std::max(1, d.chi2_blocks)));

  {
    const size_t n_dn = (size_t)(d.n_pose + d.n_plane + 255) / 256 + 1;
    const size_t flag_doubles = 2 * (size_t)std::max(1, A.n_fronts) + 1;
    double* zb = nullptr;
    TRY(dev_alloc(g, &zb, n_dn + 2 + 8 + 2 * delta_doubles + flag_doubles));
    zero_block = zb; zero_doubles = n_dn + 2 + 8 + 2 * delta_doubles + flag_doubles;
    d.k3_flag = reinterpret_cast<int*>(zb + n_dn + 2 + 8 + 2 * delta_doubles);
    g->k3_epoch = 0;
    d.delta = zb + n_dn + 10; g->spec_delta = d.delta + delta_doubles;
    d.dn_partials = zb;
    d.ticket = reinterpret_cast<unsigned int*>(zb + n_dn);
    g->spec_ticket = reinterpret_cast<unsigned int*>(zb + n_dn + 1);
    d.result_dev = zb + n_dn + 2; g->spec_result = zb + n_dn + 6;
    g->status_clean = true;
  }
  TRY(dev_alloc(g, &g->spec_pose, state_doubles + 1)); g->spec_plane = g->spec_pose + (size_t)7 * d.pose_ld;
  TRY(dev_alloc(g, &g->spec_chi2_partials, (size_t)std::max(1, d.chi2_blocks)));
  TRY(dev_alloc(g, &g->spec_dn_partials, (size_t)(d.n_pose + d.n_plane + 255) / 256 + 1));
  d.trace_solve = g->sw.trace >= 2 ? 1 : 0;
  if (g->sw.trace) { TRY(dev_alloc(g, &d.trace, (size_t)A.n_fronts * 8)); HIP_TRY(g, hipMemset(d.trace, 0, (size_t)A.n_fronts * 64)); }
  if (!g->use_band && !g->use_dense && A.max_front > lds_front_limit()) {
    const int fa = A.max_front + 1;
    d.gwork_stride = (int64_t)fa * (fa | 1);
    int widest = 0;
    for (int l = 0; l < A.n_levels; l++)
      if (g->level_max_front[l] > lds_front_limit()) widest = std::max(widest, A.level_off[l + 1] - A.level_off[l]);
    TRY(dev_alloc(g, &d.gwork, (size_t)d.gwork_stride * std::max(1, widest)));
  }
#undef TRY
  lap("5 index arrays + diff");
  rc = flush_uploads(g); if (rc != PPS_OK) return rc;
  rc = verify_uploads(g, "upload_all"); if (rc != PPS_OK) return rc;
  lap("6 flush");
  const bool one_launch = A.ea_total > 0 && zero_doubles < (size_t)1 << 30 && (int)A.asm_blk.size() == A.n_blocks && A.n_fronts > 0 &&
                          !g->sw.split_expand;
  if (one_launch) HIP_TRY(g, launch_expand_lists(d, A.n_fronts, (int)A.asm_blk.size(), zero_block, zero_doubles, g->stream));
  else {
    const size_t n_dst = (size_t)std::max(1, A.blk_doff[A.n_blocks]);
    if (A.ea_total > 0 && zero_doubles < (size_t)1 << 30 && n_dst < (size_t)1 << 30)
      HIP_TRY(g, launch_expand_ea(d, A.n_fronts, zero_block, zero_doubles, d.blk_dst, n_dst, g->stream));
    else {
      if (A.ea_total > 0) HIP_TRY(g, launch_expand_ea(d, A.n_fronts, nullptr, 0, nullptr, 0, g->stream));
      HIP_TRY(g, hipMemsetAsync(zero_block, 0, zero_doubles * 8, g->stream));
      HIP_TRY(g, hipMemsetAsync(d.blk_dst, 0xff, sizeof(int) * n_dst, g->stream));
    }
    HIP_TRY(g, launch_expand_el(d, (int)A.asm_blk.size(), g->stream));
  }
  g->topo_dirty = false;
  g->meas_dirty = false;
  g->grown_only_upload = true;
  g->up_an_seq = g->an_seq;
  lap("7 expand kernels + sync");
  rc = upload_state(g, false);
  lap("8 upload_state");
  g->stats.t_upload = now_s() - t0 - g->stats.t_analysis;
  return rc;
}

int prepare_solve(pps_graph* g) {
  int rc;
  if (g->n_live_nodes == 0) return fail(g, PPS_ESTATE, "empty graph");
  if (g->dev_ready) HIP_TRY(g, hipSetDevice(g->props.device));
  if (g->topo_dirty || !g->dev_ready || g->dev.n_scalars == 0) { rc = upload_all(g); if (rc != PPS_OK) return rc; }
  if (g->host_values_newer) { rc = upload_state(g); if (rc != PPS_OK) return rc; }
  if (g->meas_dirty) { rc = upload_measurements(g); if (rc != PPS_OK) return rc; }
  return PPS_OK;
}

}
```

Baseline: 16900 LM iters/s.

## Fuse K2 Hessian-block assembly as tail blocks into the linearize sweep kernels

Appends the K2 Hessian block-assembly work as extra trailing blocks to the lane-form linearize kernel and the speculative trial-linearize kernel. A done-counter is bumped by each sweep block, and the tail blocks wait on it before assembling, which removes a separate launch_hblocks / launch_hblocks_spec launch per iteration. Tail blocks spin on a device counter, so they depend on the sweep blocks being scheduled first. A done-counter is packed next to the existing ticket word, PPS_NO_K2_TAIL disables the path, and a debug API exposes the counters.

```diff
diff --git a/include/pps.h b/include/pps.h
--- a/include/pps.h
+++ b/include/pps.h
@@ -132,6 +132,8 @@
 int pps_debug_front_factor(int tiles, int strip, int p, int b, const double* A, double* L, double* U, double* not_pd);
 
 int pps_debug_exmap(int kind, int n, const double* x, const double* delta, double* out);
+
+int pps_debug_sweep_done(pps_graph* g, unsigned int out[2]);
 
 int pps_popup_planes(int device, const float* seg2d, int n, const float invK[9], const float T_wc[16],
                      float* planes_out);
diff --git a/pop_up_slam_amd/__init__.py b/pop_up_slam_amd/__init__.py
--- a/pop_up_slam_amd/__init__.py
+++ b/pop_up_slam_amd/__init__.py
@@ -97,7 +97,7 @@
     "pps_edges_host_select", "pps_popup_fill_depth", "pps_popup_plane_info", "pps_popup_mask_host",
     "pps_multi_create", "pps_multi_destroy", "pps_multi_last_error", "pps_multi_optimize", "pps_multi_rounds", "pps_multi_save_state", "pps_multi_restore_state", "pps_multi_set_profiling", "pps_multi_phase_times", "pps_popup_polygons_simple", "pps_analysis_reuse", "pps_analysis_kept",
     "pps_cov_recover", "pps_cov_marginals", "pps_cov_access", "pps_cov_joint", "pps_cov_last_times",
-    "pps_cov_block", "pps_cov_block_last",
+    "pps_cov_block", "pps_cov_block_last", "pps_debug_sweep_done",
 ]
 
 
@@ -501,6 +501,12 @@
     def set_profiling(self, level=2):
         self._ck(self.L.pps_set_profiling(self.h, int(level)))
 
+    def debug_sweep_done(self):
+        out = (C.c_uint * 2)()
+        self.L.pps_debug_sweep_done.argtypes = [C.c_void_p, C.POINTER(C.c_uint)]
+        self._ck(self.L.pps_debug_sweep_done(self.h, out))
+        return int(out[0]), int(out[1])
+
     def eval_factor(self, fid, mode=JAC_NUMERIC):
         m, c = C.c_int(), C.c_int(); self._ck(self.L.pps_factor_shape(self.h, fid, C.byref(m), C.byref(c)))
         J = np.zeros((m.value, c.value)); r = np.zeros(m.value)
diff --git a/pop_up_slam_amd/csrc/pps_api.cpp b/pop_up_slam_amd/csrc/pps_api.cpp
--- a/pop_up_slam_amd/csrc/pps_api.cpp
+++ b/pop_up_slam_amd/csrc/pps_api.cpp
@@ -16,6 +16,7 @@
   }
   s.no_spec_lin = on("PPS_NO_SPEC_LIN");
   s.no_dual = on("PPS_NO_DUAL");
+  s.no_k2_tail = on("PPS_NO_K2_TAIL");
   s.no_strip = on("PPS_NO_STRIP");
   s.no_incremental = on("PPS_NO_INCREMENTAL");
   s.no_incr_compact = on("PPS_NO_INCR_COMPACT");
@@ -497,6 +498,16 @@
   if (!A || !L || !U) return PPS_EINVAL;
   const int rc = pps::debug_front_factor(tiles, strip, p, b, A, L, U, not_pd);
   return rc == 0 ? PPS_OK : (rc < 0 ? PPS_EINVAL : PPS_EHIP);
+}
+
+int pps_debug_sweep_done(pps_graph* g, unsigned int out[2]) {
+  if (!g || !out) return PPS_EINVAL;
+  out[0] = out[1] = 0u;
+  if (!g->dev_ready || !g->dev.sweep_done) return PPS_OK;
+  HIP_TRY(g, hipStreamSynchronize(g->stream));
+  HIP_TRY(g, hipMemcpy(&out[0], g->dev.sweep_done, sizeof(unsigned int), hipMemcpyDeviceToHost));
+  if (g->spec_sweep_done) HIP_TRY(g, hipMemcpy(&out[1], g->spec_sweep_done, sizeof(unsigned int), hipMemcpyDeviceToHost));
+  return PPS_OK;
 }
 
 int pps_debug_exmap(int kind, int n, const double* x, const double* delta, double* out) {
diff --git a/pop_up_slam_amd/csrc/pps_device.h b/pop_up_slam_amd/csrc/pps_device.h
--- a/pop_up_slam_amd/csrc/pps_device.h
+++ b/pop_up_slam_amd/csrc/pps_device.h
@@ -62,6 +62,7 @@
   int chi2_blocks = 0;
   double* dn_partials = nullptr;
   unsigned int* ticket = nullptr;
+  unsigned int* sweep_done = nullptr;
   double* result_dev = nullptr;
   long long* trace = nullptr;
   int trace_solve = 0;
@@ -73,7 +74,7 @@
 };
 
 constexpr double kStatusInternal = 64.0;
-enum : unsigned { SW_K1_THREAD_FORM = 1u, SW_NO_SOLVE_FLOW = 2u, SW_NO_ROOT_FUSE = 4u, SW_DEBUG_DROP_FLAG = 8u, SW_DEBUG_DROP_XFLAG = 16u };
+enum : unsigned { SW_K1_THREAD_FORM = 1u, SW_NO_SOLVE_FLOW = 2u, SW_NO_ROOT_FUSE = 4u, SW_DEBUG_DROP_FLAG = 8u, SW_DEBUG_DROP_XFLAG = 16u, SW_NO_K2_TAIL = 32u };
 struct Switches {
   bool k1_thread_form = false;
   bool no_preassemble = false;
@@ -82,6 +83,7 @@
   bool split_expand = false;
   bool no_spec_lin = false;
   bool no_dual = false;
+  bool no_k2_tail = false;
   bool no_strip = false;
   bool no_incremental = false;
   bool no_incr_compact = false;
@@ -94,7 +96,7 @@
   int multi_split = 0;
   long long multi_thread_factors = 120000;
   unsigned dev_bits() const {
-    return (k1_thread_form ? SW_K1_THREAD_FORM : 0u) | (no_solve_flow ? SW_NO_SOLVE_FLOW : 0u) | (no_root_fuse ? SW_NO_ROOT_FUSE : 0u) |
+    return (k1_thread_form ? SW_K1_THREAD_FORM : 0u) | (no_solve_flow ? SW_NO_SOLVE_FLOW : 0u) | (no_root_fuse ? SW_NO_ROOT_FUSE : 0u) | (no_k2_tail ? SW_NO_K2_TAIL : 0u) |
            (debug_drop_flag == 1 ? SW_DEBUG_DROP_FLAG : 0u) | (debug_drop_flag == 2 ? SW_DEBUG_DROP_XFLAG : 0u);
   }
 };
@@ -126,7 +128,9 @@
 
 hipError_t step_constants(double ac[4]);
 hipError_t launch_linearize(const DevGraph& d, int mode, bool at_estimate, hipStream_t st, const LinGuard* guard = nullptr, hipEvent_t ev0 = nullptr,
-                            hipEvent_t ev1 = nullptr);
+                            hipEvent_t ev1 = nullptr,
+                            unsigned int* k2_done = nullptr);
+bool k2_tail_ok(const DevGraph& d, int mode);
 hipError_t launch_hblocks(const DevGraph& d, hipStream_t st, const LinGuard* guard = nullptr, bool products = true);
 bool k1_lane_form(const DevGraph& d, int mode);
 bool k1_products(const DevGraph& d, int mode);
@@ -156,7 +160,8 @@
                              double seq1, hipStream_t st, int n_trials = 2);
 hipError_t launch_trial_lin(const DevGraph& d, const DualAlt& alt, const SpecLin& sl, const double* base_pose, const double* base_plane, double* out_pose0,
                             double* out_plane0, double* out_pose1, double* out_plane1, double* host_result0, double seq0, double* host_result1,
-                            double seq1, hipStream_t st, hipEvent_t ev0 = nullptr, hipEvent_t ev1 = nullptr);
+                            double seq1, hipStream_t st, hipEvent_t ev0 = nullptr, hipEvent_t ev1 = nullptr,
+                            unsigned int* k2_done = nullptr, const LinGuard* k2_guard = nullptr);
 int trial_lin_waves(const DevGraph& d);
 bool trial_lin_ok(const DevGraph& d, int mode);
 hipError_t launch_hblocks_spec(const DevGraph& d, const SpecLin& sl, hipStream_t st, const LinGuard* guard = nullptr);
diff --git a/pop_up_slam_amd/csrc/pps_graph.h b/pop_up_slam_amd/csrc/pps_graph.h
--- a/pop_up_slam_amd/csrc/pps_graph.h
+++ b/pop_up_slam_amd/csrc/pps_graph.h
@@ -117,6 +117,7 @@
   double seq = 0.0;
   double *spec_pose = nullptr, *spec_plane = nullptr, *spec_chi2_partials = nullptr, *spec_dn_partials = nullptr;
   unsigned int* spec_ticket = nullptr;
+  unsigned int* spec_sweep_done = nullptr;
   double seq2 = 0.0;
   double *spec_L = nullptr, *spec_U = nullptr, *spec_delta = nullptr;
   double* spec_result = nullptr;
diff --git a/pop_up_slam_amd/csrc/pps_k1.hip b/pop_up_slam_amd/csrc/pps_k1.hip
--- a/pop_up_slam_amd/csrc/pps_k1.hip
+++ b/pop_up_slam_amd/csrc/pps_k1.hip
@@ -8,7 +8,8 @@
 
 namespace pps {
 
-hipError_t launch_linearize_lanes(const DevGraph& d, const double* pose, const double* plane, const LinGuard& gd, hipStream_t st, hipEvent_t ev0, hipEvent_t ev1);
+hipError_t launch_linearize_lanes(const DevGraph& d, const double* pose, const double* plane, const LinGuard& gd, hipStream_t st, hipEvent_t ev0, hipEvent_t ev1,
+                                  unsigned int* k2_done);
 hipError_t launch_sweep_bench_lanes(const DevGraph& d, int replicas, double* Jbig, int part, hipStream_t st);
 hipError_t launch_batch_linearize_lanes(const BatchArgs& a, const BatchGeom& g, hipStream_t st);
 
@@ -77,7 +78,8 @@
 
 bool k1_products(const DevGraph& d, int mode) { (void)mode; return !(d.sw & SW_K1_THREAD_FORM); }
 
-hipError_t launch_linearize(const DevGraph& d, int mode, bool at_estimate, hipStream_t st, const LinGuard* guard, hipEvent_t ev0, hipEvent_t ev1) {
+hipError_t launch_linearize(const DevGraph& d, int mode, bool at_estimate, hipStream_t st, const LinGuard* guard, hipEvent_t ev0, hipEvent_t ev1, unsigned int* k2_done) {
+  if (k2_done && !k2_tail_ok(d, mode)) return hipErrorInvalidValue;
   const LinGuard gd = guard ? *guard : LinGuard{};
   if (d.n_obs > d.n_obs_fixed) {
     PPS_LAUNCH(k_linearize_repop, dim3(cdiv(d.n_obs - d.n_obs_fixed, 64)), dim3(64), 0, st, d,
@@ -89,7 +91,7 @@
   if (nb == 0) return hipSuccess;
   const double* pose = at_estimate ? d.pose_est : d.pose_lin;
   const double* plane = at_estimate ? d.plane_est : d.plane_lin;
-  if (k1_lane_form(d, mode)) return launch_linearize_lanes(d, pose, plane, gd, st, ev0, ev1);
+  if (k1_lane_form(d, mode)) return launch_linearize_lanes(d, pose, plane, gd, st, ev0, ev1, k2_done);
   if (ev0) { const hipError_t e = hipEventRecord(ev0, st); if (e != hipSuccess) return e; }
   const size_t lds0 = (size_t)(kLinBlock / 64) * 64 * 31 * sizeof(double), lds1 = (size_t)(kLinBlock / 64) * 64 * 79 * sizeof(double);
   const int nb_rest = nb - nb_obs;
diff --git a/pop_up_slam_amd/csrc/pps_k1_lanes.hip b/pop_up_slam_amd/csrc/pps_k1_lanes.hip
--- a/pop_up_slam_amd/csrc/pps_k1_lanes.hip
+++ b/pop_up_slam_amd/csrc/pps_k1_lanes.hip
@@ -1,21 +1,28 @@
 #include <hip/hip_ext.h>
 
 #include "pps_k1_body.h"
+#include "pps_k2_body.h"
 
 namespace pps {
 
 __global__ __launch_bounds__(kLanesPerBlock) void k_linearize_lanes(DevGraph d, const double* __restrict__ pose,
                                                                     const double* __restrict__ plane, int nb_obs, int nb_odo,
-                                                                    int nb_pp, LinGuard gd, int apply) {
+                                                                    int nb_pp, LinGuard gd, int apply, K2Tail tail) {
   if (!lin_guard(gd, pose, plane)) return;
+  if (tail.done && (int)blockIdx.x >= tail.first) { body_k2_tail(d, tail, LinGuard{}, blockIdx.x); return; }
   body_linearize_lanes(d, pose, plane, nb_obs, nb_odo, nb_pp, blockIdx.x, apply != 0);
+  if (tail.done) tail_post(tail);
 }
 
 
-hipError_t launch_linearize_lanes(const DevGraph& d, const double* pose, const double* plane, const LinGuard& gd, hipStream_t st, hipEvent_t ev0, hipEvent_t ev1) {
+hipError_t launch_linearize_lanes(const DevGraph& d, const double* pose, const double* plane, const LinGuard& gd, hipStream_t st, hipEvent_t ev0, hipEvent_t ev1,
+                                  unsigned int* k2_done) {
+  static_assert(kLanesPerBlock == 64 * kK2TailWaves, "one block size for the sweep and its K2 blocks");
   const int lb_obs = cdiv(d.n_obs_fixed, kObsPerBlock), lb_odo = cdiv(d.n_odo, kFactorsPerBlock), lb_pp = cdiv(d.n_pp, kFactorsPerBlock),
             lb_lp = cdiv(d.n_lp, kFactorsPerBlock);
-  PPS_LAUNCH_EV(ev0, ev1, k_linearize_lanes, dim3(lb_obs + lb_odo + lb_pp + lb_lp), dim3(kLanesPerBlock), 0, st, d, pose, plane, lb_obs, lb_odo, lb_pp, gd, 0);
+  const int lb_all = lb_obs + lb_odo + lb_pp + lb_lp;
+  const K2Tail tail{k2_done, lb_all, k2_done ? k2_tail_blocks(d) : 0, lb_all};
+  PPS_LAUNCH_EV(ev0, ev1, k_linearize_lanes, dim3(lb_all + tail.nb), dim3(kLanesPerBlock), 0, st, d, pose, plane, lb_obs, lb_odo, lb_pp, gd, 0, tail);
   return hipGetLastError();
 }
 
diff --git a/pop_up_slam_amd/csrc/pps_k2.hip b/pop_up_slam_amd/csrc/pps_k2.hip
--- a/pop_up_slam_amd/csrc/pps_k2.hip
+++ b/pop_up_slam_amd/csrc/pps_k2.hip
@@ -1,142 +1,9 @@
 #include <cstdlib>
 
-#include "pps_kcommon.h"
-#include "pps_symbolic.h"
+#include "pps_k2_body.h"
 
 namespace pps {
 
-constexpr int kK2Waves = 16;
-
-__device__ __forceinline__ double wave_segment_sum(const DevGraph& d, int rec, int4 mine, int lane, int* __restrict__ plist) {
-  const int rows = __builtin_amdgcn_readlane(rec, 0), cols = __builtin_amdgcn_readlane(rec, 1), size = __builtin_amdgcn_readlane(rec, 2);
-  const int cnt = __builtin_amdgcn_readlane(rec, 4);
-  const int rc = rows * cols;
-  const bool act = lane < size;
-  const bool is_g = lane >= rc;
-  const int cdiv_ = cols > 0 ? cols : 1;
-  const int i = is_g ? lane - rc : lane / cdiv_;
-  const int j = is_g ? 0 : lane - (lane / cdiv_) * cdiv_;
-  const bool isp = lane < cnt && mine.w >= kProductFlag;
-  const unsigned long long pmask = __ballot(isp);
-  unsigned long long jmask = __ballot(lane < cnt && !isp);
-  const double* __restrict__ J = d.J;
-  const double* __restrict__ P = d.P;
-  double acc = 0.0;
-  const int np = __builtin_popcountll(pmask);
-  const int S = size <= 12 ? 5 : (size <= 21 ? 3 : (size <= 32 ? 2 : 1));
-  const int sl = lane / (size > 0 ? size : 1), en = lane - sl * size;
-  const bool live = sl < S && size > 0;
-  const int enc = live ? en : 0;
-  double v0[16];
-  if (np > 0) {
-    const int rank = __builtin_popcountll(pmask & ((1ull << lane) - 1ull));
-    if (isp) plist[rank] = mine.y;
-    __builtin_amdgcn_wave_barrier();
-#pragma unroll
-    for (int u = 0; u < 16; u++) { const int k = sl + S * u; v0[u] = P[plist[k < np ? k : np - 1] + enc]; }
-  }
-  while (jmask) {
-    const int c0 = __builtin_ctzll(jmask);
-    jmask &= jmask - 1;
-    const bool two = jmask != 0;
-    const int c1 = two ? __builtin_ctzll(jmask) : c0;
-    jmask &= jmask - 1;
-    double a[2][6], bb[2][6];
-#pragma unroll
-    for (int u = 0; u < 2; u++) {
-      const int cc = u ? c1 : c0;
-      const int jv = __builtin_amdgcn_readlane(mine.x, cc), ju = __builtin_amdgcn_readlane(mine.y, cc);
-      const int ro = __builtin_amdgcn_readlane(mine.z, cc), mm = __builtin_amdgcn_readlane(mine.w, cc);
-      const double* pa = J + jv + i;
-      const double* pb = is_g ? J + ro : J + ju + j;
-      const int sb = is_g ? 1 : cols;
-#pragma unroll
-      for (int k = 0; k < 6; k++) {
-        const bool ok = act && k < mm && (u == 0 || two);
-        a[u][k] = ok ? pa[k * rows] : 0.0;
-        bb[u][k] = ok ? pb[k * sb] : 0.0;
-      }
-    }
-#pragma unroll
-    for (int u = 0; u < 2; u++)
-#pragma unroll
-      for (int k = 0; k < 6; k++) acc = PPS_MAC(acc, a[u][k], bb[u][k]);
-  }
-  if (is_g) acc = -acc;
-  if (!act) acc = 0.0;
-  if (np > 0) {
-    double pacc = 0.0;
-#pragma unroll
-    for (int u = 0; u < 16; u++) pacc += (live && sl + S * u < np) ? v0[u] : 0.0;
-    for (int k0 = 16 * S; k0 < np; k0 += 16 * S) {
-      double v[16];
-#pragma unroll
-      for (int u = 0; u < 16; u++) { const int k = k0 + sl + S * u; v[u] = P[plist[k < np ? k : np - 1] + enc]; }
-#pragma unroll
-      for (int u = 0; u < 16; u++) pacc += (live && k0 + sl + S * u < np) ? v[u] : 0.0;
-    }
-    __builtin_amdgcn_wave_barrier();
-    double tot = pacc;
-    for (int sg = 1; sg < S; sg++) tot += __shfl(pacc, lane + sg * size, 64);
-    acc += act ? tot : 0.0;
-  }
-  return acc;
-}
-
-__device__ __forceinline__ void seg_header(const DevGraph& d, int seg, int lane, int& rec, int4& mine) {
-  rec = d.srec[(size_t)seg * 8 + (lane & 7)];
-  const int c0 = __builtin_amdgcn_readlane(rec, 3), cnt = __builtin_amdgcn_readlane(rec, 4);
-  mine = make_int4(0, 0, 0, 0);
-  if (lane < cnt) mine = reinterpret_cast<const int4*>(d.contrib)[c0 + lane];
-  if (!d.P && mine.w >= kProductFlag) { mine.w -= kProductFlag; mine.y = mine.x; }
-}
-
-__device__ __forceinline__ void body_hblocks2(const DevGraph& d, int bx) {
-  __shared__ double part[kK2Waves][64];
-  __shared__ int plist_lds[kK2Waves][64];
-  const int wave = uni(threadIdx.x >> 6), lane = threadIdx.x & 63;
-  int* const plist = plist_lds[wave];
-  const int nbs = (d.n_k2_single + kK2Waves - 1) / kK2Waves;
-  if (bx < nbs) {
-    const int slot = bx * kK2Waves + wave;
-    if (slot >= d.n_k2_single) return;
-    int rec; int4 mine;
-    seg_header(d, uni(d.k2_single[slot]), lane, rec, mine);
-    const int size = __builtin_amdgcn_readlane(rec, 2), hoff = __builtin_amdgcn_readlane(rec, 5), doff = __builtin_amdgcn_readlane(rec, 6);
-    const int dst = lane < size ? d.blk_dst[doff + lane] : -1;
-    const double acc = wave_segment_sum(d, rec, mine, lane, plist);
-    if (lane >= size) return;
-    d.H[hoff + lane] = acc;
-    if (dst >= 0) d.Hf[dst] = acc;
-    return;
-  }
-  const int b = bx - nbs;
-  if (b >= d.n_k2_multi) return;
-  const int seg0 = uni(d.k2_multi[2 * b]), info = uni(d.k2_multi[2 * b + 1]);
-  const int nsc = info & 0xffff;
-  const bool fin = (info >> 16) != 0;
-  int rec0; int4 mine0;
-  seg_header(d, seg0, lane, rec0, mine0);
-  const int size = __builtin_amdgcn_readlane(rec0, 2), hoff = __builtin_amdgcn_readlane(rec0, 5), doff = __builtin_amdgcn_readlane(rec0, 6);
-  const int dst = (fin && wave == 0 && lane < size) ? d.blk_dst[doff + lane] : -1;
-  double acc = 0.0;
-  for (int sgi = wave; sgi < nsc; sgi += kK2Waves) {
-    int rec; int4 mine;
-    if (sgi == 0) { rec = rec0; mine = mine0; } else seg_header(d, seg0 + sgi, lane, rec, mine);
-    acc += wave_segment_sum(d, rec, mine, lane, plist);
-  }
-  part[wave][lane] = acc;
-  __syncthreads();
-  if (wave != 0 || lane >= size) return;
-  const int nw = nsc < kK2Waves ? nsc : kK2Waves;
-  double q[4] = {0.0, 0.0, 0.0, 0.0};
-#pragma unroll
-  for (int w = 0; w < 4; w++)
-    for (int v = w; v < nw; v += 4) q[w] += part[v][lane];
-  const double tot = (q[0] + q[1]) + (q[2] + q[3]);
-  d.H[hoff + lane] = tot;
-  if (dst >= 0) d.Hf[dst] = tot;
-}
 
 constexpr int kK2Chunk = 16;
 __device__ __forceinline__ void body_hfinish(const DevGraph& d, int bx) {
diff --git a/pop_up_slam_amd/csrc/pps_k2_body.h b/pop_up_slam_amd/csrc/pps_k2_body.h
--- /dev/null
+++ b/pop_up_slam_amd/csrc/pps_k2_body.h
@@ -0,0 +1,186 @@
+#pragma once
+#include "pps_kcommon.h"
+#include "pps_regtile.h"
+#include "pps_symbolic.h"
+
+namespace pps {
+
+constexpr int kK2Waves = 16;
+constexpr int kK2TailWaves = 4;
+
+__device__ __forceinline__ double wave_segment_sum(const DevGraph& d, int rec, int4 mine, int lane, int* __restrict__ plist) {
+  const int rows = __builtin_amdgcn_readlane(rec, 0), cols = __builtin_amdgcn_readlane(rec, 1), size = __builtin_amdgcn_readlane(rec, 2);
+  const int cnt = __builtin_amdgcn_readlane(rec, 4);
+  const int rc = rows * cols;
+  const bool act = lane < size;
+  const bool is_g = lane >= rc;
+  const int cdiv_ = cols > 0 ? cols : 1;
+  const int i = is_g ? lane - rc : lane / cdiv_;
+  const int j = is_g ? 0 : lane - (lane / cdiv_) * cdiv_;
+  const bool isp = lane < cnt && mine.w >= kProductFlag;
+  const unsigned long long pmask = __ballot(isp);
+  unsigned long long jmask = __ballot(lane < cnt && !isp);
+  const double* __restrict__ J = d.J;
+  const double* __restrict__ P = d.P;
+  double acc = 0.0;
+  const int np = __builtin_popcountll(pmask);
+  const int S = size <= 12 ? 5 : (size <= 21 ? 3 : (size <= 32 ? 2 : 1));
+  const int sl = lane / (size > 0 ? size : 1), en = lane - sl * size;
+  const bool live = sl < S && size > 0;
+  const int enc = live ? en : 0;
+  double v0[16];
+  if (np > 0) {
+    const int rank = __builtin_popcountll(pmask & ((1ull << lane) - 1ull));
+    if (isp) plist[rank] = mine.y;
+    __builtin_amdgcn_wave_barrier();
+#pragma unroll
+    for (int u = 0; u < 16; u++) { const int k = sl + S * u; v0[u] = P[plist[k < np ? k : np - 1] + enc]; }
+  }
+  while (jmask) {
+    const int c0 = __builtin_ctzll(jmask);
+    jmask &= jmask - 1;
+    const bool two = jmask != 0;
+    const int c1 = two ? __builtin_ctzll(jmask) : c0;
+    jmask &= jmask - 1;
+    double a[2][6], bb[2][6];
+#pragma unroll
+    for (int u = 0; u < 2; u++) {
+      const int cc = u ? c1 : c0;
+      const int jv = __builtin_amdgcn_readlane(mine.x, cc), ju = __builtin_amdgcn_readlane(mine.y, cc);
+      const int ro = __builtin_amdgcn_readlane(mine.z, cc), mm = __builtin_amdgcn_readlane(mine.w, cc);
+      const double* pa = J + jv + i;
+      const double* pb = is_g ? J + ro : J + ju + j;
+      const int sb = is_g ? 1 : cols;
+#pragma unroll
+      for (int k = 0; k < 6; k++) {
+        const bool ok = act && k < mm && (u == 0 || two);
+        a[u][k] = ok ? pa[k * rows] : 0.0;
+        bb[u][k] = ok ? pb[k * sb] : 0.0;
+      }
+    }
+#pragma unroll
+    for (int u = 0; u < 2; u++)
+#pragma unroll
+      for (int k = 0; k < 6; k++) acc = PPS_MAC(acc, a[u][k], bb[u][k]);
+  }
+  if (is_g) acc = -acc;
+  if (!act) acc = 0.0;
+  if (np > 0) {
+    double pacc = 0.0;
+#pragma unroll
+    for (int u = 0; u < 16; u++) pacc += (live && sl + S * u < np) ? v0[u] : 0.0;
+    for (int k0 = 16 * S; k0 < np; k0 += 16 * S) {
+      double v[16];
+#pragma unroll
+      for (int u = 0; u < 16; u++) { const int k = k0 + sl + S * u; v[u] = P[plist[k < np ? k : np - 1] + enc]; }
+#pragma unroll
+      for (int u = 0; u < 16; u++) pacc += (live && k0 + sl + S * u < np) ? v[u] : 0.0;
+    }
+    __builtin_amdgcn_wave_barrier();
+    double tot = pacc;
+    for (int sg = 1; sg < S; sg++) tot += __shfl(pacc, lane + sg * size, 64);
+    acc += act ? tot : 0.0;
+  }
+  return acc;
+}
+
+__device__ __forceinline__ void seg_header(const DevGraph& d, int seg, int lane, int& rec, int4& mine) {
+  rec = d.srec[(size_t)seg * 8 + (lane & 7)];
+  const int c0 = __builtin_amdgcn_readlane(rec, 3), cnt = __builtin_amdgcn_readlane(rec, 4);
+  mine = make_int4(0, 0, 0, 0);
+  if (lane < cnt) mine = reinterpret_cast<const int4*>(d.contrib)[c0 + lane];
+  if (!d.P && mine.w >= kProductFlag) { mine.w -= kProductFlag; mine.y = mine.x; }
+}
+
+template <int NW = kK2Waves>
+__device__ __forceinline__ void body_hblocks2(const DevGraph& d, int bx) {
+  static_assert(NW == 16 || NW == 4, "the partial sums of a chunk are interleaved by four");
+  __shared__ double part[NW][64];
+  __shared__ int plist_lds[NW][64];
+  const int wave = uni(threadIdx.x >> 6), lane = threadIdx.x & 63;
+  int* const plist = plist_lds[wave];
+  const int nbs = (d.n_k2_single + NW - 1) / NW;
+  if (bx < nbs) {
+    const int slot = bx * NW + wave;
+    if (slot >= d.n_k2_single) return;
+    int rec; int4 mine;
+    seg_header(d, uni(d.k2_single[slot]), lane, rec, mine);
+    const int size = __builtin_amdgcn_readlane(rec, 2), hoff = __builtin_amdgcn_readlane(rec, 5), doff = __builtin_amdgcn_readlane(rec, 6);
+    const int dst = lane < size ? d.blk_dst[doff + lane] : -1;
+    const double acc = wave_segment_sum(d, rec, mine, lane, plist);
+    if (lane >= size) return;
+    d.H[hoff + lane] = acc;
+    if (dst >= 0) d.Hf[dst] = acc;
+    return;
+  }
+  const int b = bx - nbs;
+  if (b >= d.n_k2_multi) return;
+  const int seg0 = uni(d.k2_multi[2 * b]), info = uni(d.k2_multi[2 * b + 1]);
+  const int nsc = info & 0xffff;
+  const bool fin = (info >> 16) != 0;
+  int rec0; int4 mine0;
+  seg_header(d, seg0, lane, rec0, mine0);
+  const int size = __builtin_amdgcn_readlane(rec0, 2), hoff = __builtin_amdgcn_readlane(rec0, 5), doff = __builtin_amdgcn_readlane(rec0, 6);
+  const int dst = (fin && wave == 0 && lane < size) ? d.blk_dst[doff + lane] : -1;
+  double acc = 0.0;
+  for (int sgi = wave; sgi < nsc; sgi += NW) {
+    int rec; int4 mine;
+    if (sgi == 0) { rec = rec0; mine = mine0; } else seg_header(d, seg0 + sgi, lane, rec, mine);
+    acc += wave_segment_sum(d, rec, mine, lane, plist);
+  }
+  part[wave][lane] = acc;
+  __syncthreads();
+  if (wave != 0 || lane >= size) return;
+  const int nw = nsc < NW ? nsc : NW;
+  double q[4] = {0.0, 0.0, 0.0, 0.0};
+#pragma unroll
+  for (int w = 0; w < 4; w++)
+    for (int v = w; v < nw; v += 4) q[w] += part[v][lane];
+  const double tot = (q[0] + q[1]) + (q[2] + q[3]);
+  d.H[hoff + lane] = tot;
+  if (dst >= 0) d.Hf[dst] = tot;
+}
+
+constexpr unsigned kTailTicket = 1u << 16;
+struct K2Tail {
+  unsigned int* done;
+  int first, nb;
+  int posts;
+};
+
+__device__ __forceinline__ void tail_post(const K2Tail& t) {
+  asm volatile("s_waitcnt vmcnt(0)" ::: "memory");
+  __syncthreads();
+  if (threadIdx.x == 0) {
+    __builtin_amdgcn_fence(__ATOMIC_RELEASE, "agent");
+    __hip_atomic_fetch_add(t.done, 1u, __ATOMIC_RELAXED, __HIP_MEMORY_SCOPE_AGENT);
+  }
+}
+__device__ __forceinline__ void tail_post_thread(unsigned int* done) {
+  __builtin_amdgcn_fence(__ATOMIC_RELEASE, "agent");
+  __hip_atomic_fetch_add(done, 1u, __ATOMIC_RELAXED, __HIP_MEMORY_SCOPE_AGENT);
+}
+__device__ __forceinline__ void tail_wait(const DevGraph& d, const K2Tail& t) {
+  if (threadIdx.x == 0) {
+    int spin = 0;
+    while ((__hip_atomic_load(t.done, __ATOMIC_RELAXED, __HIP_MEMORY_SCOPE_AGENT) & (kTailTicket - 1u)) < (unsigned)t.posts) {
+      if (++spin >= (1 << 21)) { raise_status(&d.result_dev[2], kStatusInternal); break; }
+      __builtin_amdgcn_s_sleep(2);
+    }
+  }
+  __syncthreads();
+  __builtin_amdgcn_fence(__ATOMIC_ACQUIRE, "agent");
+}
+__device__ __forceinline__ void body_k2_tail(const DevGraph& d, const K2Tail& t, const LinGuard& gd, int bx) {
+  tail_wait(d, t);
+  if (lin_guard(gd)) body_hblocks2<kK2TailWaves>(d, bx - t.first);
+  asm volatile("s_waitcnt vmcnt(0)" ::: "memory");
+  __syncthreads();
+  if (threadIdx.x == 0) {
+    const unsigned before = __hip_atomic_fetch_add(t.done, kTailTicket, __ATOMIC_RELAXED, __HIP_MEMORY_SCOPE_AGENT);
+    if ((before >> 16) == (unsigned)(t.nb - 1)) __hip_atomic_store(t.done, 0u, __ATOMIC_RELAXED, __HIP_MEMORY_SCOPE_AGENT);
+  }
+}
+inline int k2_tail_blocks(const DevGraph& d) { return (d.n_k2_single + kK2TailWaves - 1) / kK2TailWaves + d.n_k2_multi; }
+
+}
diff --git a/pop_up_slam_amd/csrc/pps_k4.hip b/pop_up_slam_amd/csrc/pps_k4.hip
--- a/pop_up_slam_amd/csrc/pps_k4.hip
+++ b/pop_up_slam_amd/csrc/pps_k4.hip
@@ -6,6 +6,7 @@
 #include "pps_geom.h"
 #include "pps_kcommon.h"
 #include "pps_k1_body.h"
+#include "pps_k2_body.h"
 
 namespace pps {
 
@@ -72,7 +73,7 @@
 
 constexpr int kChiBlock = 256;
 
-__device__ __forceinline__ void chi2_finish(const DevGraph& d, int nb, int n_dn, double* __restrict__ out, double seq) {
+__device__ __forceinline__ void chi2_finish(const DevGraph& d, int nb, int n_dn, double* __restrict__ out, double seq, unsigned int* post = nullptr) {
   double cs = 0.0, dn = 0.0;
   for (int i = threadIdx.x; i < nb; i += kChiBlock) cs += __hip_atomic_load(&d.chi2_partials[i], __ATOMIC_RELAXED, __HIP_MEMORY_SCOPE_AGENT);
   for (int i = threadIdx.x; i < n_dn; i += kChiBlock) dn += __hip_atomic_load(&d.dn_partials[i], __ATOMIC_RELAXED, __HIP_MEMORY_SCOPE_AGENT);
@@ -88,13 +89,14 @@
     d.result_dev[0] = a; d.result_dev[1] = b2; d.result_dev[2] = 0.0;
     out[0] = a; out[1] = b2; out[2] = npd;
     __hip_atomic_store(&out[3], seq, __ATOMIC_RELEASE, __HIP_MEMORY_SCOPE_SYSTEM);
+    if (post) tail_post_thread(post);
   }
 }
 
 template <bool TICKET = true, bool APPLY = false>
 __device__ __forceinline__ void body_chi2(const DevGraph& d, const double* __restrict__ pose,
                                           const double* __restrict__ plane, int nb_obs, int nb_odo, int nb_pp,
-                                          int n_dn, double* __restrict__ out, double seq, int bx, int nb, int total_blocks = 0) {
+                                          int n_dn, double* __restrict__ out, double seq, int bx, int nb, int total_blocks = 0, unsigned int* post = nullptr) {
   __shared__ double red[kChiBlock / 64];
   int b = bx;
   double s = 0.0;
@@ -174,7 +176,7 @@
   if (!last) return;
   if (threadIdx.x == 0) __builtin_amdgcn_fence(__ATOMIC_ACQUIRE, "agent");
   __syncthreads();
-  chi2_finish(d, nb, n_dn, out, seq);
+  chi2_finish(d, nb, n_dn, out, seq, post);
   if (threadIdx.x == 0) *d.ticket = 0u;
 }
 
@@ -260,9 +262,15 @@
 __global__ __launch_bounds__(kChiBlock) void k_trial_lin(DevGraph d, DualAlt alt, SpecLin sl, const double* __restrict__ base_pose, const double* __restrict__ base_plane,
                                                          double* __restrict__ out_pose, double* __restrict__ out_plane, double* __restrict__ out_pose1,
                                                          double* __restrict__ out_plane1, int nb_ret, int nb_obs, int nb_odo, int nb_pp, int nb_chi,
-                                                         double* __restrict__ out, double seq, double* __restrict__ out1, double seq1, int lb_obs, int lb_odo, int lb_pp, int apply) {
-  static_assert(kChiBlock == kLanesPerBlock, "one block size for the trial blocks and the lane-form sweep");
+                                                         double* __restrict__ out, double seq, double* __restrict__ out1, double seq1, int lb_obs, int lb_odo, int lb_pp, int apply,
+                                                         K2Tail tail, LinGuard gd) {
+  static_assert(kChiBlock == kLanesPerBlock && kChiBlock == 64 * kK2TailWaves, "one block size for the trial blocks, the lane-form sweep and the K2 blocks");
   const int total = nb_ret + nb_chi;
+  if (tail.done && (int)blockIdx.x >= tail.first) {
+    d.J = sl.J; d.P = sl.P; d.H = sl.H; d.Hf = sl.Hf;
+    body_k2_tail(d, tail, gd, blockIdx.x);
+    return;
+  }
   const bool sweep = (int)blockIdx.x >= 2 * total;
   const int y = sweep ? sl.which : ((int)blockIdx.x >= total ? 1 : 0);
   const int bx0 = sweep ? (int)blockIdx.x - 2 * total : (int)blockIdx.x - y * total;
@@ -273,10 +281,11 @@
   if (sweep) {
     d.J = sl.J; d.P = sl.P; d.H = sl.H; d.Hf = sl.Hf;
     body_linearize_lanes(d, base_pose, base_plane, lb_obs, lb_odo, lb_pp, bx0, apply != 0);
+    if (tail.done) tail_post(tail);
     return;
   }
   if (bx0 >= nb_ret) {
-    body_chi2<true, true>(d, base_pose, base_plane, nb_obs, nb_odo, nb_pp, nb_ret, out, seq, bx0 - nb_ret, nb_chi, total);
+    body_chi2<true, true>(d, base_pose, base_plane, nb_obs, nb_odo, nb_pp, nb_ret, out, seq, bx0 - nb_ret, nb_chi, total, tail.done);
     return;
   }
   __shared__ double red[4];
@@ -291,7 +300,7 @@
   if (!last) return;
   if (threadIdx.x == 0) __builtin_amdgcn_fence(__ATOMIC_ACQUIRE, "agent");
   __syncthreads();
-  chi2_finish(d, nb_chi, nb_ret, out, seq);
+  chi2_finish(d, nb_chi, nb_ret, out, seq, tail.done);
   if (threadIdx.x == 0) *d.ticket = 0u;
 }
 
@@ -301,10 +310,17 @@
   return (2 * nb + lb) * (kChiBlock / 64);
 }
 bool trial_lin_ok(const DevGraph& d, int mode) { return k1_lane_form(d, mode) && d.n_obs == d.n_obs_fixed && d.P != nullptr; }
+bool k2_tail_ok(const DevGraph& d, int mode) {
+  if (d.sw & SW_NO_K2_TAIL) return false;
+  if (!k1_lane_form(d, mode) || !k1_products(d, mode) || d.n_obs != d.n_obs_fixed || d.P == nullptr || d.n_k2_finish > 0) return false;
+  const int nb = k2_tail_blocks(d);
+  const int lb = cdiv(d.n_obs_fixed, kObsPerBlock) + cdiv(d.n_odo, kFactorsPerBlock) + cdiv(d.n_pp, kFactorsPerBlock) + cdiv(d.n_lp, kFactorsPerBlock);
+  return nb > 0 && nb < 60000 && lb > 0 && lb < 60000;
+}
 
 hipError_t launch_trial_lin(const DevGraph& d, const DualAlt& alt, const SpecLin& sl, const double* base_pose, const double* base_plane, double* out_pose0,
                             double* out_plane0, double* out_pose1, double* out_plane1, double* host_result0, double seq0, double* host_result1,
-                            double seq1, hipStream_t st, hipEvent_t ev0, hipEvent_t ev1) {
+                            double seq1, hipStream_t st, hipEvent_t ev0, hipEvent_t ev1, unsigned int* k2_done, const LinGuard* k2_guard) {
   const int n = d.n_pose + d.n_plane;
   const int nb_obs = cdiv(d.n_obs, kChiBlock), nb_odo = cdiv(d.n_odo, kChiBlock), nb_pp = cdiv(d.n_pp, kChiBlock), nb_lp = cdiv(d.n_lp, kChiBlock);
   const int nb = nb_obs + nb_odo + nb_pp + nb_lp;
@@ -313,8 +329,11 @@
   const int lb_obs = cdiv(d.n_obs_fixed, kObsPerBlock), lb_odo = cdiv(d.n_odo, kFactorsPerBlock), lb_pp = cdiv(d.n_pp, kFactorsPerBlock),
             lb_lp = cdiv(d.n_lp, kFactorsPerBlock);
   const int lb_all = lb_obs + lb_odo + lb_pp + lb_lp;
-  PPS_LAUNCH_EV(ev0, ev1, k_trial_lin, dim3(2 * (nb_ret + nb) + lb_all), dim3(kChiBlock), 0, st, d, alt, sl, base_pose, base_plane, out_pose0,
-                out_plane0, out_pose1, out_plane1, nb_ret, nb_obs, nb_odo, nb_pp, nb, host_result0, seq0, host_result1, seq1, lb_obs, lb_odo, lb_pp, 1);
+  const int first = 2 * (nb_ret + nb) + lb_all;
+  const K2Tail tail{k2_done, first, k2_done ? k2_tail_blocks(d) : 0, lb_all + 2};
+  PPS_LAUNCH_EV(ev0, ev1, k_trial_lin, dim3(first + tail.nb), dim3(kChiBlock), 0, st, d, alt, sl, base_pose, base_plane, out_pose0,
+                out_plane0, out_pose1, out_plane1, nb_ret, nb_obs, nb_odo, nb_pp, nb, host_result0, seq0, host_result1, seq1, lb_obs, lb_odo, lb_pp, 1,
+                tail, k2_guard ? *k2_guard : LinGuard{});
   return hipGetLastError();
 }
 
diff --git a/pop_up_slam_amd/csrc/pps_solve.cpp b/pop_up_slam_amd/csrc/pps_solve.cpp
--- a/pop_up_slam_amd/csrc/pps_solve.cpp
+++ b/pop_up_slam_amd/csrc/pps_solve.cpp
@@ -19,17 +19,18 @@
 };
 
 int do_linearize(pps_graph* g, const LinGuard* guard = nullptr) {
+  unsigned int* const k2_done = g->profiling < 2 && g->dev.sweep_done && k2_tail_ok(g->dev, g->props.jacobian_mode) ? g->dev.sweep_done : nullptr;
   if (g->profiling == 1) {
     if (g->k1_used + 2 > (int)g->k1_events.size()) {
       for (int k = 0; k < 2; k++) { hipEvent_t e; HIP_TRY(g, hipEventCreate(&e)); g->k1_events.push_back(e); }
     }
     g->k1_skip.resize(g->k1_events.size() / 2, 0);
     g->k1_skip[g->k1_used / 2] = 0;
-    HIP_TRY(g, launch_linearize(g->dev, g->props.jacobian_mode, false, g->stream, guard, g->k1_events[g->k1_used], g->k1_events[g->k1_used + 1]));
+    HIP_TRY(g, launch_linearize(g->dev, g->props.jacobian_mode, false, g->stream, guard, g->k1_events[g->k1_used], g->k1_events[g->k1_used + 1], k2_done));
     g->k1_used += 2;
   } else
-  { PhaseTimer t(g, &g->stats.t_linearize); HIP_TRY(g, launch_linearize(g->dev, g->props.jacobian_mode, false, g->stream, guard)); }
-  { PhaseTimer t(g, &g->stats.t_assemble); HIP_TRY(g, launch_hblocks(g->dev, g->stream, guard, k1_products(g->dev, g->props.jacobian_mode))); }
+  { PhaseTimer t(g, &g->stats.t_linearize); HIP_TRY(g, launch_linearize(g->dev, g->props.jacobian_mode, false, g->stream, guard, nullptr, nullptr, k2_done)); }
+  if (!k2_done) { PhaseTimer t(g, &g->stats.t_assemble); HIP_TRY(g, launch_hblocks(g->dev, g->stream, guard, k1_products(g->dev, g->props.jacobian_mode))); }
   if (!guard) g->stats.n_linearize++;
   return PPS_OK;
 }
@@ -314,6 +315,7 @@
   bool use_alt = !adaptive;
   bool have_next = true;
   const bool fuse_lin = !g->sw.no_spec_lin && g->spec_J != nullptr && trial_lin_ok(d, prop.jacobian_mode) && trial_lin_waves(d) <= 3072;
+  unsigned int* const k2_done = fuse_lin && g->spec_sweep_done && k2_tail_ok(d, prop.jacobian_mode) ? g->spec_sweep_done : nullptr;
   int fused_pair = -1;
   int pred = 0, pred_launched = 0;
   bool error_known = false;
@@ -329,9 +331,10 @@
       g->k1_skip[fused_pair] = 1;
       e0 = g->k1_events[g->k1_used]; e1 = g->k1_events[g->k1_used + 1]; g->k1_used += 2;
     }
-    HIP_TRY(g, launch_trial_lin(d, alt, sl, d.pose_lin, d.plane_lin, t_pose[0], t_plane[0], t_pose[1], t_plane[1], slot[0], s0, slot[1], s1, g->stream, e0, e1));
     const LinGuard gd{{d.result_dev, g->spec_result}, {nullptr, nullptr}, {nullptr, nullptr}, lm.error, error_known ? 1 : 0, use_alt ? 0 : 1, pred_launched};
-    HIP_TRY(g, launch_hblocks_spec(d, sl, g->stream, &gd));
+    HIP_TRY(g, launch_trial_lin(d, alt, sl, d.pose_lin, d.plane_lin, t_pose[0], t_plane[0], t_pose[1], t_plane[1], slot[0], s0, slot[1], s1, g->stream, e0, e1,
+                                k2_done, &gd));
+    if (!k2_done) HIP_TRY(g, launch_hblocks_spec(d, sl, g->stream, &gd));
     return PPS_OK;
   };
   auto enqueue_dual = [&](double lam) -> int {
diff --git a/pop_up_slam_amd/csrc/pps_upload.cpp b/pop_up_slam_amd/csrc/pps_upload.cpp
--- a/pop_up_slam_amd/csrc/pps_upload.cpp
+++ b/pop_up_slam_amd/csrc/pps_upload.cpp
@@ -488,7 +488,7 @@
   lap("1c opening stream sync");
   free_device(g);
   g->spec_L = g->spec_U = g->spec_delta = nullptr; g->spec_result = nullptr;
-  g->spec_pose = g->spec_plane = g->spec_chi2_partials = g->spec_dn_partials = nullptr; g->spec_ticket = nullptr;
+  g->spec_pose = g->spec_plane = g->spec_chi2_partials = g->spec_dn_partials = nullptr; g->spec_ticket = nullptr; g->spec_sweep_done = nullptr;
   g->spec_J = g->spec_P = g->spec_H = g->spec_Hf = nullptr;
   g->d_item_frame = g->d_item_plane = g->d_item_slot = g->d_frame_pose_slot = g->d_frame_seg_off = nullptr; g->d_fr_seg = nullptr;
   g->frames_dirty = true;
@@ -672,6 +672,7 @@
     d.dn_partials = zb;
     d.ticket = reinterpret_cast<unsigned int*>(zb + n_dn);
     g->spec_ticket = reinterpret_cast<unsigned int*>(zb + n_dn + 1);
+    d.sweep_done = d.ticket + 1; g->spec_sweep_done = g->spec_ticket + 1;
     d.result_dev = zb + n_dn + 2; g->spec_result = zb + n_dn + 6;
     g->status_clean = true;
   }
```

Result: slower. 9305 LM iters/s (-44.9%).
